# jaak-s/BayesianDataFusion.jl

Measured on AMD Instinct MI355X. Metric: Gibbs sweeps/sec (both entities) + test RMSE, MovieLens-1M D=32, higher is better.
Workload: dtype f64; 1 GPU; BPMF MovieLens-1M 6040x3952, 500209 training ratings (500000 held out), D=32, alpha=1.5, step = rows of both entities + hyperpriors + test prediction update (one native call); BEFORE the --warmup steps the engine's set-up runs 60 ms of full iterations whose results are discarded (device_warmup_ms); num_latent=32, burnin=5, psamples=1985, parallelism=1 GPU

## Files before the change

### bayesiandatafusion.jl_amd/_lib.py

```python
import ctypes as C
import os

_HERE = os.path.dirname(os.path.abspath(__file__))
LIB_PATH = os.environ.get("BDF_LIB_PATH") or os.path.join(_HERE, "csrc", "libbdf_hip.so")

BDF_MAX_MODES = 4
BDF_MAX_TERMS = 4
BDF_MAX_D = 64

P_ROW, P_BETA_E1, P_BETA_E2, P_NW_NORMAL, P_GAMMA_N, P_GAMMA_U, P_NW_MEAN, P_BETA_REL1, P_BETA_REL2 = 1, 2, 3, 4, 5, 6, 7, 8, 9
P_HMC_MOMENTUM, P_HMC_ACCEPT = 10, 11
P_PROBIT = 12
P_CENSORED = 13
P_INTERVAL = 14
P_ORDINAL = 15
P_ROBUST_N, P_ROBUST_U = 16, 17
P_PG = 18
P_NOISE_N, P_NOISE_U = 19, 20
P_SPIKE_N, P_SPIKE_U, P_SPIKE = 21, 22, 23


class ArgumentError(ValueError):
    """The reference's ArgumentError."""

# ... 93 lines not shown
    "bdf_ctx_time_next_hyper": (C.c_int, [C.c_void_p, C.c_void_p, C.c_void_p]),
    "bdf_ctx_set_item_size": (C.c_int, [C.c_void_p, C.c_int]),
    "bdf_dev_alloc": (C.c_int, [C.c_void_p, C.c_size_t, C.POINTER(C.c_void_p)]),
    "bdf_dev_free": (C.c_int, [C.c_void_p, C.c_void_p]),
    "bdf_h2d": (C.c_int, [C.c_void_p, C.c_void_p, C.c_void_p, C.c_size_t]),
    "bdf_d2h": (C.c_int, [C.c_void_p, C.c_void_p, C.c_void_p, C.c_size_t]),
    "bdf_index_build": (C.c_int, [C.c_int, c_i64p, C.c_int64, C.c_void_p, C.c_int, C.POINTER(c_i64p), C.POINTER(c_i64p)]),
    "bdf_relation_create": (C.c_int, [C.c_void_p, C.c_int, c_i64p, C.c_int64, C.c_void_p, C.c_int, c_dp, C.POINTER(C.c_void_p)]),
    "bdf_relation_destroy": (C.c_int, [C.c_void_p]),
    "bdf_relation_index": (C.c_int, [C.c_void_p, C.c_int, C.POINTER(c_i64p), C.POINTER(c_i64p)]),
    "bdf_relation_value_mean": (C.c_int, [C.c_void_p, c_dp]),
    "bdf_relation_order": (C.c_int, [C.c_void_p, C.c_int, c_i32p]),
    "bdf_sample_rows": (C.c_int, [C.c_void_p, C.c_int, C.c_int64, C.c_int, C.POINTER(Term), C.c_void_p, C.c_int, C.c_void_p,
                                  C.c_uint32, C.c_int, C.c_int, C.c_void_p, C.c_void_p]),
    "bdf_prior_pack_doubles": (C.c_int, [C.c_int]),
    "bdf_sample_block": (C.c_int, [C.c_void_p, C.c_int, C.c_int64, C.c_int64, C.c_void_p, C.c_void_p, C.c_void_p, C.c_double, C.c_void_p,
                                   C.c_void_p, C.c_uint32, C.c_void_p]),
    "bdf_row_system": (C.c_int, [C.c_void_p, C.c_int, C.c_int64, C.c_int, C.POINTER(Term), C.c_void_p, C.c_int, C.c_void_p,
                                 C.c_void_p, C.c_void_p]),
    "bdf_normals": (C.c_int, [C.c_void_p, C.c_uint32, C.c_uint32, C.c_int64, C.c_int64, C.c_int, C.c_void_p]),
    "bdf_philox": (C.c_int, [C.c_void_p, C.c_uint32, C.c_uint32, C.c_uint64, C.c_uint32, C.POINTER(C.c_uint32)]),
    "bdf_sample_rows_spike": (C.c_int, [C.c_void_p, C.c_int, C.c_int64, C.c_int, C.POINTER(Term), C.c_void_p, C.c_void_p, C.c_uint32, C.c_int,
                                        C.c_int, C.c_void_p]),
    "bdf_spike_hyper": (C.c_int, [C.c_void_p, C.c_int, C.c_int64, C.c_void_p, C.c_double, C.c_double, C.c_double, C.c_double, C.c_uint32,
                                  C.c_void_p]),
    "bdf_spike_accumulate": (C.c_int, [C.c_void_p, C.c_int, C.c_int64, C.c_void_p, C.c_void_p, C.c_void_p, C.c_void_p]),
    "bdf_hyper_sums": (C.c_int, [C.c_void_p, C.c_int, C.c_int64, C.c_void_p, C.c_void_p, C.c_void_p, C.c_void_p]),
    "bdf_hyper_sums_ranks": (C.c_int, [C.c_void_p, C.c_void_p, C.c_int, C.c_int64, C.c_int, C.c_void_p, C.c_void_p, C.c_void_p, C.c_void_p]),
    "bdf_hyper_sample": (C.c_int, [C.c_void_p, C.c_int, C.c_int64, C.c_void_p, C.c_void_p, C.c_void_p, C.c_double, C.c_void_p,
                                   C.c_double, C.c_uint32, C.c_void_p, C.c_void_p, C.c_void_p, C.c_void_p, C.c_void_p]),
    "bdf_hyper_draws": (C.c_int, [C.c_void_p, C.c_int, C.c_int64, C.c_double, C.c_uint32, C.c_void_p]),
    "bdf_pairs_sort": (C.c_int, [C.c_void_p, C.c_int]),
    "bdf_pairs_order": (C.c_int, [C.c_void_p, c_i64p]),
    "bdf_pairs_set_baseline": (C.c_int, [C.c_void_p, C.c_void_p]),
    "bdf_pairs_set_link": (C.c_int, [C.c_void_p, C.c_int]),
    "bdf_pairs_set_logistic_link": (C.c_int, [C.c_void_p]),
    "bdf_pairs_set_count_link": (C.c_int, [C.c_void_p, C.c_double]),
    "bdf_probit_draw": (C.c_int, [C.c_void_p, C.c_void_p, C.c_int, C.POINTER(C.c_void_p), C.c_double, C.c_uint32, C.c_void_p, C.c_void_p]),
    "bdf_censored_draw": (C.c_int, [C.c_void_p, C.c_void_p, C.c_void_p, C.c_int, C.POINTER(C.c_void_p), C.c_double, C.c_double, C.c_void_p,
                                    C.c_uint32, C.c_void_p, C.c_void_p]),
    "bdf_interval_draw": (C.c_int, [C.c_void_p, C.c_void_p, C.c_void_p, C.c_int, C.POINTER(C.c_void_p), C.c_double, C.c_double, C.c_void_p,
                                    C.c_uint32, C.c_void_p, C.c_void_p]),
    "bdf_robust_draw": (C.c_int, [C.c_void_p, C.c_void_p, C.c_int, C.POINTER(C.c_void_p), C.c_double, C.c_double, C.c_void_p, C.c_double,
                                  C.c_uint32, C.c_void_p, C.c_void_p]),
    "bdf_pg_draw": (C.c_int, [C.c_void_p, C.c_void_p, C.c_int, C.POINTER(C.c_void_p), C.c_double, C.c_int, C.c_double, C.c_uint32,
                              C.c_void_p, C.c_void_p]),
    "bdf_entity_noise_draw": (C.c_int, [C.c_void_p, C.c_void_p, C.c_int, C.c_void_p, C.c_int, C.POINTER(C.c_void_p), C.c_double, C.c_double,
                                        C.c_void_p, C.c_double, C.c_double, C.c_uint32, C.c_void_p, C.c_void_p, C.c_void_p]),
    "bdf_pairs_set_precision_scale": (C.c_int, [C.c_void_p, C.c_void_p, C.c_int]),
    "bdf_pairs_weighted_sse": (C.c_int, [C.c_void_p, C.c_void_p, C.c_int, C.POINTER(C.c_void_p), C.c_double, C.c_void_p, C.c_void_p]),
    "bdf_background_prior": (C.c_int, [C.c_void_p, C.c_int, C.c_int64, C.c_int, C.POINTER(BackgroundTerm), C.c_void_p, C.c_int, C.c_void_p,
                                       C.c_void_p, C.c_void_p, C.c_void_p, C.c_void_p]),
    "bdf_background_sse": (C.c_int, [C.c_void_p, C.c_void_p, C.c_int, C.POINTER(C.c_void_p), C.c_double, C.c_void_p, C.c_double, C.c_double,
                                     C.c_void_p, C.c_void_p, C.c_void_p, C.c_void_p, C.c_int64, C.c_int64, C.c_void_p]),
    "bdf_scores_create": (C.c_int, [C.c_void_p, C.c_int64, C.c_int64, C.c_int, C.c_int, C.c_void_p, C.POINTER(C.c_void_p)]),
    "bdf_scores_destroy": (C.c_int, [C.c_void_p]),
    "bdf_scores_push": (C.c_int, [C.c_void_p, C.c_void_p, C.c_void_p]),
    "bdf_scores_flush": (C.c_int, [C.c_void_p]),
    "bdf_scores_topk": (C.c_int, [C.c_void_p, C.c_void_p, C.c_int, C.c_double, C.c_void_p, C.c_void_p]),
    "bdf_scores_metrics": (C.c_int, [C.c_void_p, C.c_void_p, C.c_int, C.c_void_p, C.c_double, C.c_void_p]),
    "bdf_scores_copy": (C.c_int, [C.c_void_p, C.c_void_p, C.c_int64, C.c_int64, C.c_int]),
    "bdf_scores_set_draws": (C.c_int, [C.c_void_p, C.c_double]),
    "bdf_ordinal_create": (C.c_int, [C.c_void_p, C.c_int, C.c_double, C.c_int64, C.POINTER(C.c_void_p)]),
    "bdf_ordinal_destroy": (C.c_int, [C.c_void_p]),
    "bdf_ordinal_set_adapt": (C.c_int, [C.c_void_p, C.c_int64]),
    "bdf_ordinal_step": (C.c_int, [C.c_void_p, C.c_void_p, C.c_void_p, C.c_void_p, C.c_int, C.POINTER(C.c_void_p), C.c_double, C.c_double,
                                   C.c_void_p, C.c_uint32, C.c_int, C.c_void_p]),
    "bdf_ordinal_bounds": (C.c_int, [C.c_void_p, C.c_void_p, C.c_void_p, C.c_int64, C.c_void_p]),
    "bdf_ordinal_read": (C.c_int, [C.c_void_p, c_dp, c_dp, c_i64p, c_i64p, c_dp, c_dp, C.c_int64]),
    "bdf_ordinal_proposal": (C.c_int, [C.c_void_p, c_dp, c_dp, C.POINTER(C.c_int), c_dp]),
    "bdf_feat_linear": (C.c_int, [C.c_void_p, C.c_void_p, C.c_void_p, C.c_double, C.c_void_p]),
    "bdf_predict_sse": (C.c_int, [C.c_void_p, C.c_void_p, C.c_int, C.POINTER(C.c_void_p), C.c_double, C.c_void_p, C.c_void_p]),
    "bdf_sample_alpha": (C.c_int, [C.c_void_p, C.c_double, C.c_double, C.c_int64, C.c_void_p, C.c_uint32, C.c_void_p]),
    "bdf_sample_beta_rel": (C.c_int, [C.c_void_p, C.c_void_p, C.c_void_p, C.c_int, C.POINTER(C.c_void_p), C.c_double, C.c_double,
                                      C.c_double, C.c_uint32, C.c_void_p, C.c_void_p, C.c_void_p]),
    "bdf_sample_beta_rel_ranks": (C.c_int, [C.c_void_p, C.c_void_p, C.c_void_p, C.c_void_p, C.c_int64, C.c_int, C.POINTER(C.c_void_p),
                                            C.c_double, C.c_double, C.c_double, C.c_uint32, C.c_void_p, C.c_void_p, C.c_void_p]),
    "bdf_sum_ranks": (C.c_int, [C.c_void_p, C.c_void_p, C.c_void_p, C.c_int64]),
    "bdf_gibbs_recorded": (C.c_int, [C.c_void_p, C.c_int, C.POINTER(C.c_int), C.POINTER(C.c_int)]),
    "bdf_gibbs_set_recorded": (C.c_int, [C.c_void_p, C.c_int, C.c_int, C.c_int]),
    "bdf_ctx_set_small_rows": (C.c_int, [C.c_void_p, C.c_int, C.c_int64]),
    "bdf_ctx_set_lowrank": (C.c_int, [C.c_void_p, C.c_int, C.c_int64]),
    "bdf_ctx_set_col_rows": (C.c_int, [C.c_void_p, C.c_int]),
    "bdf_ctx_rows_dispatch": (C.c_int, [C.c_void_p, C.c_uint32, C.POINTER(C.c_int64)]),
    "bdf_pairs_create": (C.c_int, [C.c_void_p, C.c_int, C.c_int64, C.c_void_p, C.c_int, c_dp, C.POINTER(C.c_void_p)]),
    "bdf_pairs_destroy": (C.c_int, [C.c_void_p]),
    "bdf_predict": (C.c_int, [C.c_void_p, C.c_void_p, C.c_int, C.POINTER(C.c_void_p), C.c_double, C.c_void_p]),
    "bdf_predict_all": (C.c_int, [C.c_void_p, C.c_int, C.POINTER(C.c_int64), C.c_int, C.POINTER(C.c_void_p), C.c_double, C.c_void_p]),
    "bdf_predict_update": (C.c_int, [C.c_void_p, C.c_void_p, C.c_int, C.POINTER(C.c_void_p), C.c_double, C.c_int, C.c_double,
                                     C.c_double, C.c_double, C.c_void_p]),
    "bdf_pairs_state": (C.c_int, [C.c_void_p, C.POINTER(C.c_void_p), C.POINTER(C.c_void_p), c_i64p]),
    "bdf_pairs_lpd_update": (C.c_int, [C.c_void_p, C.c_void_p, C.c_void_p, C.c_int, C.POINTER(C.c_void_p), C.c_double, C.c_double, C.c_void_p,
                                       C.c_int, C.c_void_p]),
    "bdf_pairs_lpd": (C.c_int, [C.c_void_p, C.c_void_p, C.c_void_p]),
    "bdf_pairs_waic_update": (C.c_int, [C.c_void_p, C.c_void_p, C.c_void_p, C.c_int, C.POINTER(C.c_void_p), C.c_double, C.c_double, C.c_void_p,
                                        C.c_int, C.c_void_p]),
    "bdf_pairs_waic": (C.c_int, [C.c_void_p, C.c_void_p, C.c_void_p, C.c_void_p]),
    "bdf_newrows_quad": (C.c_int, [C.c_void_p, C.c_int, C.c_int64, C.c_void_p, C.c_void_p, C.c_void_p]),
    "bdf_newrows_update": (C.c_int, [C.c_void_p, C.c_void_p, C.c_int, C.c_void_p, C.c_void_p, C.c_void_p, C.c_double, C.c_double, C.c_void_p,
                                     C.c_int, C.c_double, C.c_double, C.c_double, C.c_int, C.c_void_p]),
    "bdf_newrows_result": (C.c_int, [C.c_void_p, C.c_void_p, C.c_void_p]),
    "bdf_newrows_state": (C.c_int, [C.c_void_p, C.POINTER(C.c_void_p), c_dp]),
    "bdf_feat_create_dense": (C.c_int, [C.c_void_p, C.c_int64, C.c_int64, c_dp, C.POINTER(C.c_void_p)]),
    "bdf_feat_create_csr": (C.c_int, [C.c_void_p, C.c_int64, C.c_int64, C.c_int64, c_i32p, c_i32p, c_dp, C.POINTER(C.c_void_p)]),
    "bdf_feat_create_bin": (C.c_int, [C.c_void_p, C.c_int64, C.c_int64, C.c_int64, c_i32p, c_i32p, C.POINTER(C.c_void_p)]),
    "bdf_feat_destroy": (C.c_int, [C.c_void_p]),
    "bdf_feat_set_row_ids": (C.c_int, [C.c_void_p, c_i32p]),
    "bdf_feat_size": (C.c_int, [C.c_void_p, c_i64p, c_i64p, c_i64p]),
    "bdf_feat_mul": (C.c_int, [C.c_void_p, C.c_void_p, C.c_void_p, C.c_int, C.c_void_p, C.c_int]),
    "bdf_feat_AtA_mul": (C.c_int, [C.c_void_p, C.c_void_p, C.c_void_p, C.c_int, C.c_double, C.c_void_p]),
    "bdf_uhat": (C.c_int, [C.c_void_p, C.c_void_p, C.c_int, C.c_void_p, C.c_void_p, C.c_void_p, C.c_void_p]),
    "bdf_hyper_feature_terms": (C.c_int, [C.c_void_p, C.c_int, C.c_int64, C.c_void_p, C.c_void_p, C.c_void_p, C.c_void_p]),
    "bdf_sample_beta": (C.c_int, [C.c_void_p, C.c_void_p, C.c_int, C.c_void_p, C.c_void_p, C.c_void_p, C.c_void_p, C.c_int,
                                  C.c_double, C.c_int, C.c_int, C.c_double, C.c_double, C.c_uint32, C.c_void_p, C.c_void_p,
                                  C.c_void_p]),
    "bdf_sample_beta_ranks": (C.c_int, [C.c_void_p, C.c_void_p, C.c_void_p, C.c_int, C.c_void_p, C.c_void_p, C.c_void_p, C.c_void_p, C.c_int,
                                        C.c_double, C.c_int, C.c_int, C.c_double, C.c_double, C.c_uint32, C.c_void_p, C.c_void_p,
                                        C.c_void_p]),
    "bdf_allgather_block": (C.c_int, [C.c_void_p, C.c_void_p, C.c_void_p, C.c_size_t]),
    "bdf_ctx_create_side": (C.c_int, [C.c_void_p, C.POINTER(C.c_void_p), C.c_int, C.c_int, C.POINTER(C.c_void_p)]),
    "bdf_ctx_create_rows": (C.c_int, [C.c_int, C.c_uint64, C.c_int, C.POINTER(C.c_void_p)]),
    "bdf_ctx_stream": (C.c_int, [C.c_void_p, C.POINTER(C.c_void_p)]),
    "bdf_layout_build": (C.c_int, [C.c_int64, c_i64p, C.c_int, C.c_int, c_i32p, c_i64p]),
    "bdf_relation_create_sharded": (C.c_int, [C.c_void_p, C.c_int, c_i64p, C.c_int64, C.c_void_p, C.c_int, c_dp, C.POINTER(c_i32p),
                                              c_i64p, C.c_int, C.c_int, C.c_int, C.POINTER(C.c_void_p)]),
    "bdf_comm_unique_id": (C.c_int, [C.c_void_p]),
    "bdf_comm_create": (C.c_int, [C.c_void_p, C.c_int, C.c_int, C.c_char_p, C.POINTER(C.c_void_p)]),
    "bdf_comm_create_host": (C.c_int, [C.c_void_p, C.c_int, C.c_int, EXCHANGE_FN, C.c_void_p, C.POINTER(C.c_void_p)]),
    "bdf_comm_enable_peer": (C.c_int, [C.c_void_p, EXCHANGE_FN, C.c_void_p, C.c_size_t]),
    "bdf_comm_disable_peer": (C.c_int, [C.c_void_p]),
    "bdf_comm_peer_selftest": (C.c_int, [C.c_void_p, C.c_void_p, C.c_void_p, C.c_size_t]),
    "bdf_comm_peer_stats": (C.c_int, [C.c_void_p, C.POINTER(C.c_int64), C.POINTER(C.c_int64)]),
    "bdf_comm_destroy": (C.c_int, [C.c_void_p]),
    "bdf_comm_size": (C.c_int, [C.c_void_p, C.POINTER(C.c_int), C.POINTER(C.c_int)]),
    "bdf_allgather_rows": (C.c_int, [C.c_void_p, C.c_void_p, C.c_int, C.c_int64, C.c_void_p, C.c_int, C.c_int]),
    "bdf_allgather_join": (C.c_int, [C.c_void_p, C.c_void_p]),
    "bdf_gibbs_create": (C.c_int, [C.c_void_p, C.c_int, C.c_int, C.POINTER(GibbsEntity), C.POINTER(C.c_void_p)]),
    "bdf_gibbs_destroy": (C.c_int, [C.c_void_p]),
    "bdf_gibbs_contexts": (C.c_int, [C.c_void_p, C.POINTER(C.c_void_p), C.POINTER(C.c_void_p)]),
    "bdf_gibbs_set_test": (C.c_int, [C.c_void_p, C.c_void_p, C.POINTER(C.c_int32), C.c_double, C.c_double, C.c_double, C.c_double,
                                     C.c_void_p]),
    "bdf_gibbs_set_comm": (C.c_int, [C.c_void_p, C.c_void_p]),
    "bdf_gibbs_set_relations": (C.c_int, [C.c_void_p, C.c_int, C.c_void_p]),
    "bdf_gibbs_sweep": (C.c_int, [C.c_void_p, C.c_uint32, C.c_int]),
    "bdf_gibbs_current": (C.c_int, [C.c_void_p, C.c_int, C.POINTER(C.c_int)]),
    "bdf_gibbs_time_rows": (C.c_int, [C.c_void_p, C.c_int, C.c_void_p, C.c_void_p]),
    "bdf_gibbs_span_rows": (C.c_int, [C.c_void_p, C.c_int, C.c_void_p]),
    "bdf_ctx_span_next_rows": (C.c_int, [C.c_void_p, C.c_void_p]),
    "bdf_gibbs_sync": (C.c_int, [C.c_void_p]),
    "bdf_gibbs_rows_only": (C.c_int, [C.c_void_p, C.c_int, C.c_uint32]),
    "bdf_gibbs_warm_device": (C.c_int, [C.c_void_p, C.c_double]),
    "bdf_synth_ratings": (C.c_int, [C.c_uint64, C.c_int64, C.c_int64, C.c_int64, C.c_int64, C.c_double, C.c_double, c_i32p, c_i32p,
                                    c_dp, C.c_void_p]),
    "bdf_vb_create": (C.c_int, [C.c_void_p, C.c_int, c_i64p, C.c_int64, C.c_void_p, C.c_int, c_dp, C.c_double, c_dp, c_dp,
                                C.POINTER(C.c_void_p)]),
    "bdf_vb_destroy": (C.c_int, [C.c_void_p]),
    "bdf_vb_set_test": (C.c_int, [C.c_void_p, C.c_void_p, C.c_double, C.c_double]),
    "bdf_vb_iterate": (C.c_int, [C.c_void_p, C.c_int]),
    "bdf_vb_stats": (C.c_int, [C.c_void_p, c_dp]),
    "bdf_vb_model": (C.c_int, [C.c_void_p, C.c_int, c_dp, c_dp, c_dp]),
    "bdf_hmc_create": (C.c_int, [C.c_void_p, C.c_int, c_i64p, C.c_int64, C.c_void_p, C.c_int, c_dp, C.c_double,
                                 C.POINTER(C.c_void_p)]),
    "bdf_hmc_destroy": (C.c_int, [C.c_void_p]),
    "bdf_hmc_set_test": (C.c_int, [C.c_void_p, C.c_void_p, C.c_double, C.c_double]),
    "bdf_hmc_set_params": (C.c_int, [C.c_void_p, C.c_int, C.c_int, C.c_int, C.c_double, C.c_int]),
    "bdf_hmc_iterate": (C.c_int, [C.c_void_p, C.c_int]),
# ... 53 lines not shown
```

### bayesiandatafusion.jl_amd/csrc/bdf_api.hip

```cpp
#include <chrono>
#include "rows.h"
#include <cstdlib>
#include <cstring>
#include <algorithm>
#include <cmath>
#include <numeric>
#include <atomic>

static thread_local char g_err[512] = "";

void bdf_set_error(const char *fmt, ...)
{
    va_list ap;
    va_start(ap, fmt);
    vsnprintf(g_err, sizeof(g_err), fmt, ap);
    va_end(ap);
}

extern "C" const char *bdf_last_error(void) { return g_err; }
extern "C" int bdf_version(void) { return 100; }

extern "C" int bdf_ctx_create(int device, void *stream, uint64_t seed, bdf_ctx **out)
{
    BDF_REQUIRE(out != nullptr, BDF_ERR_ARG, "bdf_ctx_create: out is NULL");
    int ndev = 0;
    if (hipGetDeviceCount(&ndev) != hipSuccess || ndev <= 0) {
        bdf_set_error("bdf_ctx_create: no HIP device visible (this library has no CPU path)");
        return BDF_ERR_NOGPU;
    }
    BDF_REQUIRE(device >= 0 && device < ndev, BDF_ERR_ARG, "bdf_ctx_create: device %d out of range (0..%d)", device, ndev - 1);
    BDF_HIP(hipSetDevice(device));
    hipDeviceProp_t prop;
    BDF_HIP(hipGetDeviceProperties(&prop, device));
    if (strncmp(prop.gcnArchName, "gfx950", 6) != 0) {
        bdf_set_error("bdf_ctx_create: device %d is %s; this library is built for gfx950 only", device, prop.gcnArchName);
        return BDF_ERR_NOGPU;
    }
    bdf_ctx *c = new bdf_ctx();
    c->sweep_dev = nullptr; c->flag_dev = nullptr; c->flag_host = nullptr; c->scratch = nullptr; c->scratch2 = nullptr; c->cg_status = nullptr; c->cg_part = nullptr;
    c->hyper_fuse = false; c->hyper_partial = nullptr; c->hyper_nblocks = 0; c->hyper_sumU = c->hyper_UUt = nullptr;
    c->hyper_chain = false; c->hyper_count = nullptr; c->hyper_chain_draws = nullptr;
    c->own_stream = false; c->stream = nullptr; c->rows = nullptr;
    struct Guard { bdf_ctx *c; ~Guard() { if (c) bdf_ctx_destroy(c); } } guard{c};
    c->device = device;
    c->n_cus = prop.multiProcessorCount;
    c->seed = seed;
    c->own_stream = false;
    c->stream = (hipStream_t)stream;
    BDF_HIP(hipMalloc((void **)&c->sweep_dev, sizeof(uint32_t)));
    BDF_HIP(hipHostMalloc((void **)&c->flag_host, 16 * sizeof(int), hipHostMallocMapped | hipHostMallocCoherent));
    memset(c->flag_host, 0, 16 * sizeof(int));
    BDF_HIP(hipHostGetDevicePointer((void **)&c->flag_dev, c->flag_host, 0));
    BDF_HIP(hipMemsetAsync(c->sweep_dev, 0, sizeof(uint32_t), c->stream));
    c->time_start = c->time_stop = nullptr;
    c->time_h_start = c->time_h_stop = nullptr;
    c->sweep_host = 0;
    c->rows_span = nullptr;
    c->rows_ready = nullptr; c->rows_ready_want = 0; c->hyper_ready = nullptr; c->hyper_ready_value = 0;
    c->rows_done = nullptr; c->rows_done_added = -1; c->hyper_wait = nullptr; c->hyper_wait_target = 0;
    c->warnings = 0;
    c->reserve_cus = 0;
    c->on_reserved = 0;
    c->skip_flag = nullptr;
    c->cg_status = nullptr; c->cg_part = nullptr;
    c->hyper_fuse = false; c->hyper_partial = nullptr; c->hyper_nblocks = 0; c->hyper_sumU = c->hyper_UUt = nullptr;
    c->hyper_chain = false; c->hyper_count = nullptr; c->hyper_chain_draws = nullptr;
    c->cg_gen = 0;
    c->cg_bar = nullptr;
    c->rows = bdf_rows_state_create();
    c->norm_part = nullptr;
    c->newrows_W = nullptr;
    c->scratch = nullptr;
    c->scratch2 = nullptr;
    c->scratch2_bytes = 0;
    c->scratch_bytes = 0;
    c->item_size = 192;
    c->piece_size = 128;
    c->item_auto = true;
    c->small_max = getenv("BDF_K1_SMALL") ? atoi(getenv("BDF_K1_SMALL")) : 48;
    c->small_min_rows = getenv("BDF_K1_SMALL_MIN_ROWS") ? atoll(getenv("BDF_K1_SMALL_MIN_ROWS")) : 8192;
    c->lr_max = getenv("BDF_LOWRANK") ? atoi(getenv("BDF_LOWRANK")) : -1;
    c->lr_min_rows = getenv("BDF_LOWRANK_MIN_ROWS") ? atoll(getenv("BDF_LOWRANK_MIN_ROWS")) : 8192;
    c->col_piece = getenv("BDF_K1_COL") ? atoi(getenv("BDF_K1_COL")) : 128;
    if (c->col_piece == 1) c->col_piece = 128;
    if (c->col_piece != 0) c->col_piece = std::min(4096, std::max(8, c->col_piece));
    c->col_explicit = false;
    c->lr_T = nullptr; c->lr_vt = nullptr; c->lr_vt_bytes = 0; c->lr_mrows = nullptr; c->lr_mrows_bytes = 0;
    {
        const char *force = getenv("BDF_GATHER");
        c->gather_mode = force && !strcmp(force, "general") ? 1 : (force && !strcmp(force, "wide") ? 2 : 0);
    }
    guard.c = nullptr;
    *out = c;
    return BDF_OK;
}

extern "C" int bdf_ctx_destroy(bdf_ctx *ctx)
{
    if (!ctx) return BDF_OK;
    hipSetDevice(ctx->device);
    hipStreamSynchronize(ctx->stream);
    bdf_rows_state_destroy(ctx);
    if (ctx->scratch) hipFree(ctx->scratch);
    if (ctx->sweep_dev) hipFree(ctx->sweep_dev);
    if (ctx->flag_host) hipHostFree(ctx->flag_host);
    if (ctx->scratch2) hipFree(ctx->scratch2);
    if (ctx->cg_status) hipHostFree((void *)ctx->cg_status);
    if (ctx->cg_part) hipFree(ctx->cg_part);
    if (ctx->cg_bar) hipFree(ctx->cg_bar);
    if (ctx->hyper_count) hipFree(ctx->hyper_count);
    if (ctx->lr_T) hipFree(ctx->lr_T);
    if (ctx->lr_vt) hipFree(ctx->lr_vt);
    if (ctx->lr_mrows) hipFree(ctx->lr_mrows);
    if (ctx->norm_part) hipFree(ctx->norm_part);
    if (ctx->newrows_W) hipFree(ctx->newrows_W);
    if (ctx->own_stream) hipStreamDestroy(ctx->stream);
    delete ctx;
    return BDF_OK;
}

int bdf_scratch(bdf_ctx *ctx, size_t bytes, void **out)
{
    if (bytes > ctx->scratch_bytes) {
        BDF_HIP(hipStreamSynchronize(ctx->stream));
        if (ctx->scratch) BDF_HIP(hipFree(ctx->scratch));
        size_t nb = std::max(bytes, ctx->scratch_bytes * 2);
        nb = (nb + 255) & ~(size_t)255;
        BDF_HIP(hipMalloc(&ctx->scratch, nb));
        ctx->scratch_bytes = nb;
    }
    *out = ctx->scratch;
    return BDF_OK;
}

int bdf_scratch2(bdf_ctx *ctx, size_t bytes, void **out)
{
    if (bytes > ctx->scratch2_bytes) {
        BDF_HIP(hipStreamSynchronize(ctx->stream));
        if (ctx->scratch2) BDF_HIP(hipFree(ctx->scratch2));
        size_t nb = std::max(bytes, ctx->scratch2_bytes * 2);
        nb = (nb + 255) & ~(size_t)255;
        BDF_HIP(hipMalloc(&ctx->scratch2, nb));
        ctx->scratch2_bytes = nb;
    }
    *out = ctx->scratch2;
    return BDF_OK;
}

__global__ void k_set_u32(uint32_t *p, uint32_t v) { *p = v; }
__global__ void k_inc_u32(uint32_t *p) { *p = *p + 1; }

extern "C" int bdf_ctx_set_sweep(bdf_ctx *ctx, uint32_t sweep)
{
    BDF_REQUIRE(ctx, BDF_ERR_ARG, "bdf_ctx_set_sweep: ctx is NULL");
    ctx->sweep_host = sweep;
    return BDF_OK;
}

extern "C" int bdf_ctx_advance_sweep(bdf_ctx *ctx)
{
    BDF_REQUIRE(ctx, BDF_ERR_ARG, "bdf_ctx_advance_sweep: ctx is NULL");
    ctx->sweep_host++;
    return BDF_OK;
}

extern "C" int bdf_ctx_set_item_size(bdf_ctx *ctx, int observations)
{
    BDF_REQUIRE(ctx && (observations == 0 || (observations >= 8 && observations <= (1 << 20))), BDF_ERR_ARG, "bdf_ctx_set_item_size: 0 (automatic) or 8..2^20 observations");
    if (observations == 0) {
        ctx->item_size = 192; ctx->piece_size = 128; ctx->item_auto = true;
        return BDF_OK;
    }
    ctx->item_size = observations;
    ctx->piece_size = std::max(8, observations * 2 / 3);
    ctx->item_auto = false;
    return BDF_OK;
}

extern "C" int bdf_ctx_set_gather(bdf_ctx *ctx, int mode)
{
    BDF_REQUIRE(ctx && mode >= 0 && mode <= 2, BDF_ERR_ARG, "bdf_ctx_set_gather: mode must be 0 (auto), 1 (general) or 2 (64-bit offsets)");
    ctx->gather_mode = mode;
    return BDF_OK;
}

extern "C" int bdf_ctx_set_small_rows(bdf_ctx *ctx, int max_observations, int64_t min_rows)
{
    BDF_REQUIRE(ctx && max_observations >= 0 && min_rows >= 0, BDF_ERR_ARG, "bdf_ctx_set_small_rows: bad argument");
    ctx->small_max = max_observations;
    ctx->small_min_rows = min_rows;
    return BDF_OK;
}

extern "C" int bdf_ctx_set_lowrank(bdf_ctx *ctx, int max_observations, int64_t min_rows)
{
    BDF_REQUIRE(ctx && max_observations >= -1 && max_observations <= 32 && min_rows >= 0, BDF_ERR_ARG,
                "bdf_ctx_set_lowrank: max_observations must be -1 (default), 0 (off) or 1..32");
    ctx->lr_max = max_observations;
    ctx->lr_min_rows = min_rows;
    return BDF_OK;
}

extern "C" int bdf_ctx_span_next_rows(bdf_ctx *ctx, void *slot_dev)
{
    BDF_REQUIRE(ctx, BDF_ERR_ARG, "bdf_ctx_span_next_rows: NULL context");
    ctx->rows_span = (unsigned long long *)slot_dev;
    return BDF_OK;
}

extern "C" int bdf_ctx_rows_dispatch(const bdf_ctx *ctx, uint32_t entity_tag, int64_t out[6])
{
    BDF_REQUIRE(ctx && out, BDF_ERR_ARG, "bdf_ctx_rows_dispatch: NULL argument");
    const std::array<int64_t, 7> *r = bdf_rows_dispatch_counts(ctx, entity_tag);
    BDF_REQUIRE(r, BDF_ERR_ARG, "bdf_ctx_rows_dispatch: no row launch under entity_tag %u on this context", entity_tag);
    for (int k = 0; k < 6; k++) out[k] = (*r)[(size_t)k + 1];
    return BDF_OK;
}

extern "C" int bdf_ctx_set_col_rows(bdf_ctx *ctx, int max_piece)
{
    BDF_REQUIRE(ctx && (max_piece == 0 || max_piece == -1 || (max_piece >= 8 && max_piece <= 4096)), BDF_ERR_ARG,
                "bdf_ctx_set_col_rows: -1 (default), 0 (off) or 8..4096 observations per piece");
    if (max_piece == -1) {
        ctx->col_piece = getenv("BDF_K1_COL") ? atoi(getenv("BDF_K1_COL")) : 128;
        if (ctx->col_piece == 1) ctx->col_piece = 128;
        if (ctx->col_piece != 0) ctx->col_piece = std::min(4096, std::max(8, ctx->col_piece));
        ctx->col_explicit = false;
        return BDF_OK;
    }
    ctx->col_piece = max_piece;
    ctx->col_explicit = true;
    return BDF_OK;
}

extern "C" int bdf_ctx_set_piece_size(bdf_ctx *ctx, int observations)
{
    BDF_REQUIRE(ctx && observations >= 8 && observations <= ctx->item_size, BDF_ERR_ARG,
                "bdf_ctx_set_piece_size: 8..item size (%d) observations", ctx ? ctx->item_size : 0);
    ctx->piece_size = observations;
    ctx->item_auto = false;
    return BDF_OK;
}

extern "C" int bdf_ctx_sync(bdf_ctx *ctx)
{
    BDF_REQUIRE(ctx, BDF_ERR_ARG, "bdf_ctx_sync: ctx is NULL");
    hipError_t st = hipErrorNotReady;
    const auto t_spin = std::chrono::steady_clock::now();
    while ((st = hipStreamQuery(ctx->stream)) == hipErrorNotReady &&
           std::chrono::duration<double, std::micro>(std::chrono::steady_clock::now() - t_spin).count() < 300.0) { }
    if (st == hipErrorNotReady) st = hipStreamSynchronize(ctx->stream);
    BDF_HIP(st);
    int flag = __atomic_load_n(ctx->flag_host, __ATOMIC_ACQUIRE);
    if (flag) {
        __atomic_store_n(ctx->flag_host, 0, __ATOMIC_RELEASE);
        ctx->warnings |= (uint32_t)flag & BDF_WARN_CG_MAXITER;
        flag &= ~(int)BDF_WARN_CG_MAXITER;
    }
    if (flag) {
        if (flag & 16) {
            bdf_set_error("row sampler: a split row's pieces did not all arrive in time (flag %d)", flag);
            return BDF_ERR_HIP;
        }
        if (flag & 32) {
            bdf_set_error("macau_hmc: an energy of the Hamiltonian was not finite (flag %d)", flag);
            return BDF_ERR_NOTPD;
        }
        bdf_set_error("a matrix that must be positive definite was not (flag %d: %s%s%s%s)", flag, flag & 1 ? "row system " : "",
                      flag & 2 ? "hyperprior " : "", flag & 4 ? "noise precision " : "", flag & 8 ? "FF + lambda I" : "");
        return BDF_ERR_NOTPD;
    }
    return BDF_OK;
}

extern "C" int bdf_ctx_warnings(bdf_ctx *ctx, uint32_t *bits_out)
{
    BDF_REQUIRE(ctx && bits_out, BDF_ERR_ARG, "bdf_ctx_warnings: NULL argument");
    *bits_out = ctx->warnings;
    ctx->warnings = 0;
    return BDF_OK;
}

extern "C" int bdf_event_create(void **ev)
{
    BDF_REQUIRE(ev, BDF_ERR_ARG, "bdf_event_create: NULL argument");
    hipEvent_t e;
    BDF_HIP(hipEventCreate(&e));
    *ev = (void *)e;
    return BDF_OK;
}

extern "C" int bdf_event_destroy(void *ev)
{
    if (ev) BDF_HIP(hipEventDestroy((hipEvent_t)ev));
    return BDF_OK;
}

extern "C" int bdf_event_elapsed_us(void *start, void *stop, double *us)
{
    BDF_REQUIRE(start && stop && us, BDF_ERR_ARG, "bdf_event_elapsed_us: NULL argument");
    BDF_HIP(hipEventSynchronize((hipEvent_t)stop));
    float ms = 0.f;
    BDF_HIP(hipEventElapsedTime(&ms, (hipEvent_t)start, (hipEvent_t)stop));
    *us = 1e3 * (double)ms;
    return BDF_OK;
}

extern "C" int bdf_ctx_time_next_rows(bdf_ctx *ctx, void *start, void *stop)
{
    BDF_REQUIRE(ctx, BDF_ERR_ARG, "bdf_ctx_time_next_rows: ctx is NULL");
    ctx->time_start = (hipEvent_t)start;
    ctx->time_stop = (hipEvent_t)stop;
    return BDF_OK;
}
// ... 536 lines not shown
```

### bayesiandatafusion.jl_amd/csrc/bdf_common.h

```cpp
#pragma once
#include <map>
#include <array>
#include <algorithm>
#include <numeric>
#include <hip/hip_runtime.h>
#include <hip/hip_ext.h>
#include <cstdint>
#include <cstdio>
#include <cstdarg>
#include <cstring>
#include <vector>
#include "../../include/bdf.h"

void bdf_set_error(const char *fmt, ...);

#define BDF_HIP(expr)                                                                      \
    do {                                                                                   \
        hipError_t e__ = (expr);                                                           \
        if (e__ != hipSuccess) {                                                           \
            bdf_set_error("%s failed: %s (%s:%d)", #expr, hipGetErrorString(e__), __FILE__, __LINE__); \
            return BDF_ERR_HIP;                                                            \
        }                                                                                  \
    } while (0)

#define BDF_REQUIRE(cond, code, ...)                                                       \
    do {                                                                                   \
        if (!(cond)) { bdf_set_error(__VA_ARGS__); return (code); }                        \
    } while (0)

template <typename T>
int bdf_upload(T **dst, const std::vector<T> &src)
{
    BDF_HIP(hipMalloc((void **)dst, std::max<size_t>(src.size() * sizeof(T), 16)));
    if (!src.empty()) BDF_HIP(hipMemcpy(*dst, src.data(), src.size() * sizeof(T), hipMemcpyHostToDevice));
    return BDF_OK;
}

template <typename Degree>
std::vector<int32_t> rows_by_degree(int64_t N, Degree degree)
{
    std::vector<int32_t> ord((size_t)N);
    std::iota(ord.begin(), ord.end(), 0);
    std::stable_sort(ord.begin(), ord.end(), [&](int32_t x, int32_t y) { return degree(x) > degree(y); });
    return ord;
}

struct bdf_rows_state;
struct bdf_ctx {
    int device;
    int n_cus;
    hipStream_t stream;
    bool own_stream;
    uint64_t seed;
    uint32_t *sweep_dev;
    uint32_t sweep_host;
    void *scratch;
    size_t scratch_bytes;
    void *scratch2;
    size_t scratch2_bytes;
    int small_max;
    int64_t small_min_rows;
    int lr_max;
    int64_t lr_min_rows;
    int col_piece;
    bool col_explicit;
    double *lr_T;
    double *lr_mrows;
    size_t lr_mrows_bytes;
    double *lr_vt;
    size_t lr_vt_bytes;
    int *flag_dev;
    int *flag_host;
    uint32_t warnings;
    int item_size;
    int piece_size;
    bool item_auto;
    int gather_mode;
    hipEvent_t time_start, time_stop;
    unsigned long long *rows_span;
    const uint32_t *rows_ready;
    uint32_t rows_ready_want;
    uint32_t *rows_done;
    int64_t rows_done_added;
    const uint32_t *hyper_wait;
    uint32_t hyper_wait_target;
    uint32_t *hyper_ready;
    uint32_t hyper_ready_value;
    hipEvent_t time_h_start, time_h_stop;
    int reserve_cus;
    int on_reserved;
    const int *skip_flag;
    volatile uint64_t *cg_status;
    bool hyper_fuse;
    const double *hyper_partial; int hyper_nblocks; double *hyper_sumU, *hyper_UUt;
    bool hyper_chain;
    int hyper_chain_D; int64_t hyper_chain_N, hyper_chain_rpb; const double *hyper_chain_sample, *hyper_chain_uhat;
    unsigned *hyper_count;
    double *hyper_chain_draws;
    double *cg_part;
    uint32_t cg_gen;
    unsigned *cg_bar;
    bdf_rows_state *rows;
    double *norm_part;
    double *newrows_W;
};

int bdf_scratch(bdf_ctx *ctx, size_t bytes, void **out);
int bdf_scratch2(bdf_ctx *ctx, size_t bytes, void **out);
int bdf_sum_ranks_into(bdf_ctx *ctx, bdf_comm *comm, double *x, int64_t n, double *gather);
int bdf_sample_beta_rel_impl(bdf_ctx *ctx, bdf_comm *comm, const bdf_feat *fc, const bdf_pairs *train, int64_t first_obs, int D,
                             const double *const *factors, double mean_value, double alpha, const double *alpha_dev, double lambda_beta,
                             uint32_t rel_tag, double *beta_out, double *linear_out, double *rhs_out);
#define BDF_DRAWS_BATCH 8
int bdf_hyper_draws_batch(bdf_ctx *ctx, int D, int n, const int64_t *N, const double *nu, const uint32_t *entity_tag, double *const *draws_out);

struct bdf_mode_index {
    std::vector<int64_t> rowptr;
    std::vector<int64_t> rowids;
    std::vector<int32_t> order;
    int64_t *rowptr_dev;
    int32_t *colidx_dev;
    double  *vals_dev;
    int32_t *perm_dev;
    uint32_t *packed_dev;
    int32_t *order_dev;
    std::vector<int32_t> own_orig;
    std::vector<int32_t> own_pos;
    std::vector<int64_t> own_q;
    std::vector<int64_t> chunk_begin;
    int64_t own_nnz;
};

struct bdf_rel {
    bdf_ctx *ctx;
    uint64_t serial;
    int n_modes;
    int64_t dims[BDF_MAX_MODES];
    int64_t nnz;
    double value_mean;
    bdf_mode_index idx[BDF_MAX_MODES];
    int sharded;
    int rank, world, chunks;
    int64_t nint[BDF_MAX_MODES];
    int n_codes;
    double *table_dev;
};

struct bdf_pairs {
// ... 224 lines not shown
```

### bayesiandatafusion.jl_amd/csrc/bdf_gibbs.hip

```cpp
#include "bdf_common.h"
#include <algorithm>
#include <chrono>
#include <cmath>
#include <cstdio>
#include <cstdlib>
#include <map>
#include <mutex>
#include <tuple>

struct bdf_gibbs {
    bdf_ctx *rows, *hyper, *pred;
    bdf_ctx *gate = nullptr;
    int D;
    struct Ent {
        bdf_gibbs_entity d;
        int cur;
        hipEvent_t ev_rows = nullptr, ev_hyper = nullptr;
        hipEvent_t ev_beta = nullptr;
        bool beta_recorded = false;
        bool hyper_recorded = false;
        uint32_t epoch = 0;
        uint32_t *done_dev = nullptr;
        uint32_t done_target = 0;
        hipEvent_t t_start = nullptr, t_stop = nullptr;
        unsigned long long *span = nullptr;
    };
    std::vector<Ent> ent;
    bdf_pairs *test;
    int32_t test_entity[BDF_MAX_MODES];
    double test_mean, clamp_lo, clamp_hi, class_cut;
    double *stats_dev;
    hipEvent_t ev_pred[3] = {nullptr, nullptr, nullptr};
    uint64_t pred_at[3] = {0, 0, 0};
    uint64_t n_pred;
    uint64_t n_iter = 0;
    bdf_comm *comm;
    std::vector<bdf_gibbs_relation> rels;
    double *rel_sse = nullptr;
    uint32_t *ready_dev;
    bool polling;
    bool debug;
    double host_wait_us, host_enqueue_us;
    uint64_t n_sweeps;
};

namespace {

__global__ void k_spin(long long ticks)
{
    const long long t0 = wall_clock64();
    while (wall_clock64() - t0 < ticks) __builtin_amdgcn_s_sleep(8);
}

__global__ void k_wait_flag(const uint32_t *flag, long long max_ticks, uint32_t *timed_out)
{
    const long long t0 = wall_clock64();
    while (__hip_atomic_load(flag, __ATOMIC_RELAXED, __HIP_MEMORY_SCOPE_AGENT) == 0) {
        __builtin_amdgcn_s_sleep(8);
        if (wall_clock64() - t0 > max_ticks) { *timed_out = 1; break; }
    }
}
__global__ void k_set_flag(uint32_t *flag) { __hip_atomic_store(flag, 1u, __ATOMIC_RELEASE, __HIP_MEMORY_SCOPE_AGENT); }

__global__ __launch_bounds__(64) void k_rows_gate(const uint32_t *done, uint32_t target, int *flag)
{
    int spins = 0;
    for (;;) {
        uint32_t v = __hip_atomic_load(done + BDF_DONE_STRIDE * threadIdx.x, __ATOMIC_RELAXED, __HIP_MEMORY_SCOPE_AGENT);
#pragma unroll
        for (int off = 32; off >= 1; off >>= 1) v += __shfl_xor(v, off);
        if ((int32_t)(v - target) >= 0) break;
        __builtin_amdgcn_s_sleep(8);
        if (++spins > (1 << 22)) { if (threadIdx.x == 0) atomicOr_system(flag, 16); break; }
    }
}

int streams_concurrent(hipStream_t a, hipStream_t b, bool *yes)
{
    uint32_t *d;
    BDF_HIP(hipMalloc((void **)&d, 2 * sizeof(uint32_t)));
    struct Free { uint32_t *p; ~Free() { (void)hipFree(p); } } guard{d};
    BDF_HIP(hipMemsetAsync(d, 0, 2 * sizeof(uint32_t), a));
    BDF_HIP(hipStreamSynchronize(a)); BDF_HIP(hipStreamSynchronize(b));
    hipLaunchKernelGGL(k_wait_flag, dim3(1), dim3(1), 0, a, (const uint32_t *)d, 2000000LL, d + 1);
    hipLaunchKernelGGL(k_set_flag, dim3(1), dim3(1), 0, b, d);
    BDF_HIP(hipStreamSynchronize(a)); BDF_HIP(hipStreamSynchronize(b));
    uint32_t h[2] = {0, 0};
    BDF_HIP(hipMemcpy(h, d, sizeof(h), hipMemcpyDeviceToHost));
    *yes = h[1] == 0;
    return BDF_OK;
}

int streams_overlap(hipStream_t a, hipStream_t b, bool *yes)
{
    hipEvent_t e0, e1, e2;
    BDF_HIP(hipEventCreate(&e0)); BDF_HIP(hipEventCreate(&e1)); BDF_HIP(hipEventCreate(&e2));
    BDF_HIP(hipStreamSynchronize(a)); BDF_HIP(hipStreamSynchronize(b));
    float best = 1e9f;
    for (int rep = 0; rep < 3; rep++) {
        BDF_HIP(hipEventRecord(e0, a));
        BDF_HIP(hipStreamWaitEvent(b, e0, 0));
        hipLaunchKernelGGL(k_spin, dim3(1), dim3(64), 0, a, 6000LL);
        hipLaunchKernelGGL(k_spin, dim3(1), dim3(64), 0, b, 6000LL);
        BDF_HIP(hipEventRecord(e1, b));
        BDF_HIP(hipStreamWaitEvent(a, e1, 0));
        BDF_HIP(hipEventRecord(e2, a));
        BDF_HIP(hipEventSynchronize(e2));
        float ms = 0.f;
        BDF_HIP(hipEventElapsedTime(&ms, e0, e2));
        best = std::min(best, ms);
    }
    (void)hipEventDestroy(e0); (void)hipEventDestroy(e1); (void)hipEventDestroy(e2);
    *yes = best < 0.100f;
    return BDF_OK;
}

int pooled_stream(int device, int reserve, bool reserved, int slot, hipStream_t *out)
{
    static std::mutex mu;
    static std::map<std::tuple<int, int, int, int>, hipStream_t> pool;
    std::lock_guard<std::mutex> lock(mu);
    const auto key = std::make_tuple(device, reserve, reserved ? 1 : 0, slot);
    auto it = pool.find(key);
    if (it != pool.end()) { *out = it->second; return BDF_OK; }
    hipStream_t st;
    if (reserve <= 0) {
        BDF_HIP(hipStreamCreateWithFlags(&st, hipStreamNonBlocking));
    } else {
        hipDeviceProp_t prop;
        BDF_HIP(hipGetDeviceProperties(&prop, device));
        const int ncu = prop.multiProcessorCount, words = (ncu + 31) / 32;
        std::vector<uint32_t> mask((size_t)words, 0u);
        for (int i = 0; i < ncu; i++)
            if ((i < reserve) == reserved) mask[(size_t)(i / 32)] |= 1u << (i % 32);
        BDF_HIP(hipExtStreamCreateWithCUMask(&st, (uint32_t)words, mask.data()));
    }
    pool[key] = st;
    *out = st;
    return BDF_OK;
}

int make_side_ctx(bdf_ctx *main, const std::vector<bdf_ctx *> &apart, bool reserved, bdf_ctx **out)
{
    bdf_ctx *fallback = nullptr;
    for (int attempt = 0; attempt < 8; attempt++) {
        hipStream_t st;
        int rc = pooled_stream(main->device, main->reserve_cus, reserved, attempt + 1, &st);
        if (rc) return rc;
        if (st == main->stream) continue;
        bool taken = false;
        for (bdf_ctx *o : apart) taken = taken || o->stream == st;
        if (taken) continue;
        bdf_ctx *c;
        rc = bdf_ctx_create(main->device, (void *)st, main->seed, &c);
        if (rc) return rc;
        c->reserve_cus = main->reserve_cus;
        c->on_reserved = (reserved && main->reserve_cus > 0) ? 1 : 0;
        bool ok = true;
        if ((rc = streams_overlap(st, main->stream, &ok))) return rc;
// ... 11 lines not shown
}

}

extern "C" int bdf_ctx_create_rows(int device, uint64_t seed, int reserve_cus, bdf_ctx **out)
{
    BDF_REQUIRE(out && reserve_cus >= 0 && reserve_cus % 8 == 0 && reserve_cus <= 64, BDF_ERR_ARG,
                "bdf_ctx_create_rows: reserve_cus must be 0, 8, 16, ... 64 (whole CUs per XCD)");
    int ndev = 0;
    if (hipGetDeviceCount(&ndev) != hipSuccess || ndev <= 0) {
        bdf_set_error("bdf_ctx_create_rows: no HIP device visible (this library has no CPU path)");
        return BDF_ERR_NOGPU;
    }
    BDF_REQUIRE(device >= 0 && device < ndev, BDF_ERR_ARG, "bdf_ctx_create_rows: device %d out of range", device);
    BDF_HIP(hipSetDevice(device));
    hipStream_t st;
    int rc = pooled_stream(device, reserve_cus, false, 0, &st);
    if (rc) return rc;
    bdf_ctx *c;
    if ((rc = bdf_ctx_create(device, (void *)st, seed, &c))) return rc;
    c->reserve_cus = reserve_cus;
    *out = c;
    return BDF_OK;
}

extern "C" int bdf_ctx_create_side(bdf_ctx *main_ctx, bdf_ctx *const *apart, int n_apart, int reserved, bdf_ctx **out)
{
    BDF_REQUIRE(main_ctx && out && n_apart >= 0 && (n_apart == 0 || apart), BDF_ERR_ARG, "bdf_ctx_create_side: bad argument");
    std::vector<bdf_ctx *> ap(apart, apart + n_apart);
    return make_side_ctx(main_ctx, ap, reserved != 0, out);
}

extern "C" int bdf_gibbs_create(bdf_ctx *rows_ctx, int D, int n_entities, const bdf_gibbs_entity *ents, bdf_gibbs **out)
{
    BDF_REQUIRE(rows_ctx && ents && out, BDF_ERR_ARG, "bdf_gibbs_create: NULL argument");
    BDF_REQUIRE(D >= 1 && D <= BDF_MAX_D, BDF_ERR_ARG, "bdf_gibbs_create: num_latent=%d must be in 1..%d", D, BDF_MAX_D);
    BDF_REQUIRE(n_entities >= 1 && n_entities <= 64, BDF_ERR_ARG, "bdf_gibbs_create: 1..64 entities");
    for (int j = 0; j < n_entities; j++) {
        const bdf_gibbs_entity &e = ents[j];
        BDF_REQUIRE(e.n_terms >= 1 && e.n_terms <= BDF_MAX_TERMS, BDF_ERR_ARG, "bdf_gibbs_create: entity %d takes part in %d relations (1..%d)", j, e.n_terms, BDF_MAX_TERMS);
        BDF_REQUIRE(e.sample[0] && e.sample[1] && e.sample[2] && e.mu && e.Lambda && e.mu0 && e.WI && e.sumU && e.UUt && e.prior_pack && e.draws,
                    BDF_ERR_ARG, "bdf_gibbs_create: entity %d has a NULL buffer", j);
        BDF_REQUIRE(!e.feat || (e.beta && e.uhat && e.mu_matrix && e.Tinv && e.lambda_beta), BDF_ERR_ARG,
                    "bdf_gibbs_create: entity %d has side information but a NULL beta / uhat / mu_matrix / Tinv / lambda_beta", j);
        BDF_REQUIRE(!e.spike || (e.spike_state && !e.feat && !e.bg_Lambda), BDF_ERR_ARG,
                    "bdf_gibbs_create: entity %d has the spike-and-slab prior: spike_state must be set, side information and a background are not taken", j);
        BDF_REQUIRE(!e.feat || e.feat->m == e.N, BDF_ERR_ARG, "bdf_gibbs_create: entity %d has %lld rows but its feature matrix %lld", j,
                    (long long)e.N, e.feat ? (long long)e.feat->m : 0LL);
        for (int t = 0; t < e.n_terms; t++) {
            BDF_REQUIRE(e.terms[t].rel, BDF_ERR_ARG, "bdf_gibbs_create: entity %d term %d has no relation", j, t);
            for (int k = 0; k < e.terms[t].rel->n_modes; k++)
                BDF_REQUIRE(e.terms[t].entity_of_mode[k] >= 0 && e.terms[t].entity_of_mode[k] < n_entities, BDF_ERR_ARG,
                            "bdf_gibbs_create: entity %d term %d mode %d names entity %d", j, t, k, e.terms[t].entity_of_mode[k]);
        }
    }
    BDF_HIP(hipSetDevice(rows_ctx->device));
    bdf_gibbs *g = new bdf_gibbs();
    g->rows = rows_ctx; g->hyper = g->pred = nullptr; g->D = D; g->test = nullptr; g->stats_dev = nullptr;
    g->n_pred = 0; g->comm = nullptr; g->ready_dev = nullptr; g->polling = false;
    g->debug = false; g->host_wait_us = g->host_enqueue_us = 0.0; g->n_sweeps = 0;
    int rc;
    if ((rc = make_side_ctx(rows_ctx, {}, true, &g->hyper)) || (rc = make_side_ctx(rows_ctx, {g->hyper}, false, &g->pred))) { bdf_gibbs_destroy(g); return rc; }
    g->ready_dev = nullptr;
    g->polling = rows_ctx->reserve_cus > 0 && g->hyper->on_reserved && !getenv("BDF_NO_POLL");
    if (g->polling) {
        bool conc = false;
        if ((rc = streams_concurrent(rows_ctx->stream, g->hyper->stream, &conc))) { bdf_gibbs_destroy(g); return rc; }
        g->polling = conc;
    }
    if (g->polling && (rc = make_side_ctx(rows_ctx, {g->hyper, g->pred}, true, &g->gate))) { bdf_gibbs_destroy(g); return rc; }
    if (g->polling && !g->gate) g->polling = false;
    g->debug = getenv("BDF_DEBUG") != nullptr;
    if (g->debug)
        fprintf(stderr, "[bdf_gibbs] reserve_cus=%d hyperprior stream on reserved CUs=%d polling=%d\n", rows_ctx->reserve_cus,
                g->hyper->on_reserved, (int)g->polling);
    struct Guard { bdf_gibbs *g; ~Guard() { if (g) bdf_gibbs_destroy(g); } } guard{g};
    BDF_HIP(hipMalloc((void **)&g->ready_dev, (size_t)n_entities * sizeof(uint32_t)));
    BDF_HIP(hipMemsetAsync(g->ready_dev, 0, (size_t)n_entities * sizeof(uint32_t), rows_ctx->stream));
    BDF_HIP(hipStreamSynchronize(rows_ctx->stream));
    g->ent.resize((size_t)n_entities);
    for (int j = 0; j < n_entities; j++) {
        auto &E = g->ent[(size_t)j];
        E.d = ents[j]; E.cur = 0;
        BDF_HIP(hipEventCreate(&E.ev_rows));
        BDF_HIP(hipEventCreate(&E.ev_hyper));
        if (E.d.feat) BDF_HIP(hipEventCreateWithFlags(&E.ev_beta, hipEventDisableTiming));
    }
    for (int k = 0; k < 3; k++) BDF_HIP(hipEventCreateWithFlags(&g->ev_pred[k], hipEventDisableTiming));
    if (g->polling) {
        const size_t bytes = (size_t)BDF_DONE_SHARDS * BDF_DONE_STRIDE * sizeof(uint32_t);
        for (int j = 0; j < n_entities; j++) {
            BDF_HIP(hipMalloc((void **)&g->ent[(size_t)j].done_dev, bytes));
            BDF_HIP(hipMemsetAsync(g->ent[(size_t)j].done_dev, 0, bytes, rows_ctx->stream));
        }
        BDF_HIP(hipStreamSynchronize(rows_ctx->stream));
    }
    guard.g = nullptr;
    *out = g;
    return BDF_OK;
}

extern "C" int bdf_gibbs_destroy(bdf_gibbs *g)
{
    if (!g) return BDF_OK;
    if (g->rows) (void)hipStreamSynchronize(g->rows->stream);
    if (g->debug && g->n_sweeps)
        fprintf(stderr, "[bdf_gibbs] %llu sweeps: host enqueue %.1f us per sweep, host wait for the device %.1f us per sweep\n",
                (unsigned long long)g->n_sweeps, g->host_enqueue_us / (double)g->n_sweeps, g->host_wait_us / (double)g->n_sweeps);
    for (auto &E : g->ent) {
        if (E.ev_rows) (void)hipEventDestroy(E.ev_rows);
        if (E.ev_hyper) (void)hipEventDestroy(E.ev_hyper);
        if (E.ev_beta) (void)hipEventDestroy(E.ev_beta);
        if (E.done_dev) (void)hipFree(E.done_dev);
    }
    for (int k = 0; k < 3; k++)
        if (g->ev_pred[k]) (void)hipEventDestroy(g->ev_pred[k]);
    if (g->ready_dev) (void)hipFree(g->ready_dev);
    if (g->rel_sse) (void)hipFree(g->rel_sse);
    if (g->gate) { (void)hipStreamSynchronize(g->gate->stream); bdf_ctx_destroy(g->gate); }
    if (g->pred) bdf_ctx_destroy(g->pred);
    if (g->hyper) bdf_ctx_destroy(g->hyper);
    delete g;
    return BDF_OK;
}

extern "C" int bdf_gibbs_contexts(bdf_gibbs *g, bdf_ctx **hyper, bdf_ctx **pred)
{
    BDF_REQUIRE(g, BDF_ERR_ARG, "bdf_gibbs_contexts: NULL argument");
    if (hyper) *hyper = g->hyper;
    if (pred) *pred = g->pred;
    return BDF_OK;
}

extern "C" int bdf_ctx_stream(const bdf_ctx *ctx, void **stream)
{
    BDF_REQUIRE(ctx && stream, BDF_ERR_ARG, "bdf_ctx_stream: NULL argument");
    *stream = (void *)ctx->stream;
    return BDF_OK;
}

extern "C" int bdf_gibbs_set_test(bdf_gibbs *g, bdf_pairs *pairs, const int32_t *entity_of_mode, double mean_value,
                                  double clamp_lo, double clamp_hi, double class_cut, double *stats_dev)
{
    BDF_REQUIRE(g && pairs && entity_of_mode && stats_dev, BDF_ERR_ARG, "bdf_gibbs_set_test: NULL argument");
    for (int k = 0; k < pairs->n_modes; k++) {
        BDF_REQUIRE(entity_of_mode[k] >= 0 && entity_of_mode[k] < (int)g->ent.size(), BDF_ERR_ARG, "bdf_gibbs_set_test: mode %d names entity %d", k, entity_of_mode[k]);
        g->test_entity[k] = entity_of_mode[k];
    }
    g->test = pairs; g->test_mean = mean_value; g->clamp_lo = clamp_lo; g->clamp_hi = clamp_hi; g->class_cut = class_cut;
    g->stats_dev = stats_dev;
    return BDF_OK;
}

extern "C" int bdf_gibbs_set_relations(bdf_gibbs *g, int n_relations, const bdf_gibbs_relation *rels)
{
    BDF_REQUIRE(g && n_relations >= 0 && (n_relations == 0 || rels), BDF_ERR_ARG, "bdf_gibbs_set_relations: bad argument");
    for (int k = 0; k < n_relations; k++) {
        const bdf_gibbs_relation &r = rels[k];
        BDF_REQUIRE(r.rel && (r.alpha_dev || r.probit), BDF_ERR_ARG, "bdf_gibbs_set_relations: relation %d has no handle or no alpha_dev", k);
        BDF_REQUIRE(!(r.alpha_sample || r.feat) || r.train, BDF_ERR_ARG, "bdf_gibbs_set_relations: relation %d needs its observations as pairs (train)", k);
        BDF_REQUIRE(!r.feat || (r.beta && r.linear), BDF_ERR_ARG, "bdf_gibbs_set_relations: relation %d has features but no beta / linear buffer", k);
        BDF_REQUIRE(!r.feat_test || r.test_baseline, BDF_ERR_ARG, "bdf_gibbs_set_relations: relation %d has test features but no baseline buffer", k);
        BDF_REQUIRE(!r.probit || (!r.feat && !r.alpha_sample), BDF_ERR_ARG, "bdf_gibbs_set_relations: relation %d: the probit model takes neither relation features nor a sampled alpha", k);
        BDF_REQUIRE(!r.probit || (r.train && r.linear), BDF_ERR_ARG, "bdf_gibbs_set_relations: relation %d: the probit model needs its observations as pairs (train) and a linear buffer", k);
        BDF_REQUIRE(!r.censor || (!r.probit && !r.feat), BDF_ERR_ARG, "bdf_gibbs_set_relations: relation %d: the censored model takes neither the probit model nor relation features", k);
        BDF_REQUIRE(!r.censor || (r.train && r.linear), BDF_ERR_ARG, "bdf_gibbs_set_relations: relation %d: the censored model needs its observations as pairs (train) and a linear buffer", k);
// ... 105 lines not shown
    int n_bg = 0;
    for (int t = 0; t < e.n_terms; t++) {
        terms[t].rel = e.terms[t].rel; terms[t].mode = e.terms[t].mode; terms[t]._pad = 0;
        terms[t].alpha = e.terms[t].alpha; terms[t].mean_value = e.terms[t].mean_value; terms[t].linear_values = nullptr;
        terms[t].alpha_dev = nullptr; terms[t].obs_precision = nullptr;
        if (const bdf_gibbs_relation *gr = relation_of(g, e.terms[t].rel)) {
            terms[t].alpha_dev = gr->probit ? nullptr : gr->alpha_dev;
            terms[t].linear_values = (gr->feat || draws_latent(*gr)) ? gr->linear : nullptr;
            if (gr->probit) terms[t].alpha = 1.0;
            terms[t].obs_precision = gr->obs_precision;
            if (gr->bg_weight > 0.0) {
                if (gr->obs_precision) terms[t].linear_values = gr->linear;
                else terms[t].alpha_dev = e.bg_alpha_rows + n_bg;
                n_bg++;
            }
        }
        for (int k = 0; k < BDF_MAX_MODES; k++) terms[t].factors[k] = nullptr;
        current_factors(g, e.terms[t].entity_of_mode, e.terms[t].rel->n_modes, terms[t].factors);
    }
}

int update_relations(bdf_gibbs *g)
{
    bdf_ctx *R = g->rows;
    const int D = g->D;
    int rc;
    for (const auto &r : g->rels) {
        if (!has_model(r)) continue;
        const double *fac[BDF_MAX_MODES];
        current_factors(g, r.entity_of_mode, r.rel->n_modes, fac);
        if (r.robust_nu > 0.0 && (rc = bdf_robust_draw(R, r.train, D, fac, r.mean_value, 0.0, r.alpha_dev, r.robust_nu, r.rel_tag, r.obs_precision,
                                                      r.alpha_sample ? g->rel_sse + 1 : nullptr)))
            return rc;
        if (r.noise_mode != 0 && (rc = bdf_entity_noise_draw(R, r.rel, r.noise_mode - 1, r.train, D, fac, r.mean_value, 0.0, r.alpha_dev, r.noise_shape,
                                                             r.noise_rate, r.rel_tag, r.noise_tau, r.obs_precision, r.alpha_sample ? g->rel_sse + 1 : nullptr)))
            return rc;
        if (r.alpha_sample) {
            int64_t n = r.nnz;
            if (r.bg_weight > 0.0) {
                const size_t pk = (size_t)D + (size_t)D * D;
                for (int m = 0; m < 2; m++)
                    if ((rc = bdf_hyper_sums(R, D, g->ent[(size_t)r.entity_of_mode[m]].d.N, fac[m], nullptr, r.bg_sums + m * pk, r.bg_sums + m * pk + D))) return rc;
                rc = bdf_background_sse(R, r.train, D, fac, r.mean_value, r.bg_weights, r.bg_value, r.bg_weight, r.bg_sums, r.bg_sums + D, r.bg_sums + pk,
                                        r.bg_sums + pk + D, r.rel->dims[0], r.rel->dims[1], g->rel_sse + 1);
                n = r.rel->dims[0] * r.rel->dims[1];
            } else if (r.obs_precision) rc = (r.robust_nu > 0.0 || r.noise_mode != 0) ? BDF_OK : bdf_pairs_weighted_sse(R, r.train, D, fac, r.mean_value, r.obs_precision, g->rel_sse + 1);
            else rc = bdf_predict_sse(R, r.train, D, fac, r.mean_value, nullptr, g->rel_sse);
            if (rc) return rc;
            if (g->comm && (rc = bdf_sum_ranks(R, g->comm, g->rel_sse + 1, 1))) return rc;
            if ((rc = bdf_sample_alpha(R, r.alpha_lambda0, r.alpha_nu0, n, g->rel_sse + 1, r.rel_tag, r.alpha_dev))) return rc;
        }
        if (r.probit && (rc = bdf_probit_draw(R, r.train, D, fac, r.mean_value, r.rel_tag, r.linear + r.first_obs, nullptr))) return rc;
        if (r.pg_model && (rc = bdf_pg_draw(R, r.train, D, fac, r.mean_value, r.pg_model, r.pg_r, r.rel_tag, r.obs_precision, r.linear + r.first_obs)))
            return rc;
        if (r.censor && (rc = bdf_censored_draw(R, r.train, r.censor, D, fac, r.mean_value, 0.0, r.alpha_dev, r.rel_tag, r.linear + r.first_obs, nullptr)))
            return rc;
        if (r.ordinal && (rc = bdf_ordinal_step(R, r.ordinal, r.train, r.ordinal_codes, D, fac, r.mean_value, 0.0, r.alpha_dev, r.rel_tag, -1,
                                                const_cast<double *>(r.interval))))
            return rc;
        if (r.interval && (rc = bdf_interval_draw(R, r.train, r.interval, D, fac, r.mean_value, 0.0, r.alpha_dev, r.rel_tag, r.linear + r.first_obs, nullptr)))
            return rc;
        if (r.feat) {
            if ((rc = bdf_sample_beta_rel_impl(R, g->comm, r.feat, r.train, r.first_obs, D, fac, r.mean_value, 1.0, r.alpha_dev, r.lambda_beta,
                                               r.rel_tag, r.beta, r.linear + r.first_obs, nullptr)))
                return rc;
            if (g->comm) {
                if ((rc = bdf_allgather_block(R, g->comm, r.linear, sizeof(double) * (size_t)r.obs_block)) || (rc = bdf_allgather_join(R, g->comm))) return rc;
            }
            if (r.feat_test) {
                for (int k = 0; k < 3; k++)
                    if (g->n_pred > (uint64_t)k) BDF_HIP(hipStreamWaitEvent(R->stream, g->ev_pred[(g->n_pred - 1 - (uint64_t)k) % 3], 0));
                if ((rc = bdf_feat_linear(R, r.feat_test, r.beta, r.mean_value, r.test_baseline))) return rc;
            }
        }
    }
    return BDF_OK;
}
}

extern "C" int bdf_gibbs_set_comm(bdf_gibbs *g, bdf_comm *comm)
{
    BDF_REQUIRE(g, BDF_ERR_ARG, "bdf_gibbs_set_comm: NULL argument");
    g->comm = comm;
    return BDF_OK;
}

namespace {
double hyper_nu(const bdf_gibbs_entity &e) { return e.nu0 + ((e.feat && e.full_lambda_u) ? (double)e.feat->n : 0.0); }
}

extern "C" int bdf_gibbs_rows_only(bdf_gibbs *g, int entity, uint32_t sweep)
{
    BDF_REQUIRE(g && entity >= 0 && entity < (int)g->ent.size(), BDF_ERR_ARG, "bdf_gibbs_rows_only: bad argument");
    bdf_ctx *R = g->rows;
    auto &E = g->ent[(size_t)entity];
    const bdf_gibbs_entity &e = E.d;
    R->sweep_host = sweep;
    int rc;
    bdf_term terms[BDF_MAX_TERMS];
    fill_terms(g, e, terms);
    const int nxt = (E.cur + 1) % 3;
    if (e.spike) {
        if ((rc = bdf_sample_rows_spike(R, g->D, e.N, e.n_terms, terms, e.spike_state, e.sample[E.cur], e.tag, 0, 1, e.sample[nxt]))) return rc;
        E.cur = nxt;
        return BDF_OK;
    }
    const double *mu, *Lambda, *pack;
    if ((rc = row_prior(g, E, &mu, &Lambda, &pack))) return rc;
    const int nch = e.terms[0].rel->chunks;
    for (int c = 0; c < nch; c++)
        if ((rc = bdf_sample_rows(R, g->D, e.N, e.n_terms, terms, mu, e.feat ? 1 : 0, Lambda, e.tag, c, nch, e.sample[nxt], pack))) return rc;
    E.cur = nxt;
    return BDF_OK;
}

extern "C" int bdf_gibbs_warm_device(bdf_gibbs *g, double milliseconds)
{
    BDF_REQUIRE(g && milliseconds >= 0.0 && milliseconds <= 10000.0, BDF_ERR_ARG, "bdf_gibbs_warm_device: bad argument");
    if (milliseconds <= 0.0) return BDF_OK;
    bdf_ctx *R = g->rows;
    const int D = g->D, n = (int)g->ent.size();
    int rc;
    if ((rc = bdf_gibbs_sync(g))) return rc;
    struct Piece { void *p; size_t bytes; bool sample; int ent; };
    std::vector<Piece> pieces;
    std::vector<char> flags;
    const size_t DD = (size_t)D * D * sizeof(double), Dv = (size_t)D * sizeof(double);
    for (int j = 0; j < n; j++) {
        auto &E = g->ent[(size_t)j];
        const bdf_gibbs_entity &e = E.d;
        pieces.push_back({e.sample[E.cur], (size_t)e.N * Dv, true, j});
        pieces.push_back({e.mu, Dv, false, j}); pieces.push_back({e.Lambda, DD, false, j});
        pieces.push_back({e.sumU, Dv, false, j}); pieces.push_back({e.UUt, DD, false, j});
        if (e.params) pieces.push_back({e.params, Dv + DD, false, j});
        pieces.push_back({e.prior_pack, (size_t)bdf_prior_pack_doubles(D) * sizeof(double), false, j});
        pieces.push_back({e.draws, DD + Dv, false, j});
        if (e.spike) pieces.push_back({e.spike_state, 4 * Dv, false, j});
        if (e.feat) {
            pieces.push_back({e.beta, (size_t)e.feat->n * Dv, false, j});
            pieces.push_back({e.uhat, (size_t)e.N * Dv, false, j});
            pieces.push_back({e.mu_matrix, (size_t)e.N * Dv, false, j});
            pieces.push_back({e.Tinv, DD, false, j});
            pieces.push_back({e.lambda_beta, sizeof(double), false, j});
            if (e.cg_iters) pieces.push_back({e.cg_iters, (size_t)D * sizeof(int32_t), false, j});
        }
        flags.push_back(E.hyper_recorded ? 1 : 0); flags.push_back(E.beta_recorded ? 1 : 0);
    }
    if (g->stats_dev) pieces.push_back({g->stats_dev, 4 * sizeof(double), false, 0});
    for (const auto &r : g->rels) {
        if (r.alpha_dev) pieces.push_back({r.alpha_dev, sizeof(double), false, 0});
        if (r.feat) {
            int world = 1, rk = 0;
            if (g->comm) (void)bdf_comm_size(g->comm, &rk, &world);
            pieces.push_back({r.beta, (size_t)r.feat->n * sizeof(double), false, 0});
            pieces.push_back({r.linear, (size_t)r.obs_block * (size_t)world * sizeof(double), false, 0});
            if (r.feat_test) pieces.push_back({r.test_baseline, (size_t)r.feat_test->m * sizeof(double), false, 0});
        }
        if (draws_latent(r)) pieces.push_back({r.linear + r.first_obs, (size_t)r.train->n * sizeof(double), false, 0});
        if (r.robust_nu > 0.0 || r.pg_model || r.noise_mode != 0) pieces.push_back({r.obs_precision, (size_t)r.train->n * sizeof(double), false, 0});
        if (r.noise_mode != 0) pieces.push_back({r.noise_tau, (size_t)r.rel->dims[r.noise_mode - 1] * sizeof(double), false, 0});
        if (r.ordinal) {
            pieces.push_back({r.ordinal->state_dev, r.ordinal->state_doubles * sizeof(double), false, 0});
            pieces.push_back({const_cast<double *>(r.interval), (size_t)r.train->n * 2 * sizeof(double), false, 0});
        }
    }
    size_t total = 0;
    for (auto &pc : pieces) total += (pc.bytes + 255) & ~(size_t)255;
    char *snap = nullptr;
    BDF_HIP(hipMalloc((void **)&snap, std::max<size_t>(total, 256)));
    struct Free { char *p; ~Free() { if (p) (void)hipFree(p); } } guard{snap};
    size_t off = 0;
    for (auto &pc : pieces) {
        BDF_HIP(hipMemcpyAsync(snap + off, pc.p, pc.bytes, hipMemcpyDeviceToDevice, R->stream));
        off += (pc.bytes + 255) & ~(size_t)255;
    }
    BDF_HIP(hipStreamSynchronize(R->stream));
    const uint32_t keep = R->sweep_host;
    int64_t fixed = 0;
    const auto t0 = std::chrono::steady_clock::now();
    int64_t k = 0;
    rc = BDF_OK;
    while (!rc) {
        for (int b = 0; b < 8 && !rc; b++, k++) rc = bdf_gibbs_sweep(g, 0xfffe0000u + (uint32_t)(k & 0xffff), g->test ? 3 : -1);
        if (rc) break;
        if (g->comm && fixed == 0) {
            if ((rc = bdf_gibbs_sync(g))) break;
            const double per_iter = std::chrono::duration<double, std::milli>(std::chrono::steady_clock::now() - t0).count() / 8.0;
            const double mine = std::max(8.0, std::min(20000.0, milliseconds / std::max(per_iter, 1e-3)));
            int rank = 0, world = 1;
            if ((rc = bdf_comm_size(g->comm, &rank, &world))) break;
            void *sv;
            if ((rc = bdf_scratch(R, ((size_t)world + 1) * sizeof(double), &sv))) break;
            double *cnt = (double *)sv;
            BDF_HIP(hipMemcpyAsync(cnt, &mine, sizeof(double), hipMemcpyHostToDevice, R->stream));
            if ((rc = bdf_sum_ranks_into(R, g->comm, cnt, 1, cnt + 1))) break;
            double sum = 0.0;
            BDF_HIP(hipMemcpyAsync(&sum, cnt, sizeof(double), hipMemcpyDeviceToHost, R->stream));
            BDF_HIP(hipStreamSynchronize(R->stream));
            fixed = std::max<int64_t>(8, (int64_t)(sum / (double)world + 0.5));
        }
        if (fixed ? k >= fixed : std::chrono::duration<double, std::milli>(std::chrono::steady_clock::now() - t0).count() >= milliseconds) break;
    }
    const int rc_sync = bdf_gibbs_sync(g);
    if (!rc) rc = rc_sync;
    off = 0;
    for (auto &pc : pieces) {
        void *dst = pc.sample ? (void *)g->ent[(size_t)pc.ent].d.sample[g->ent[(size_t)pc.ent].cur] : pc.p;
        BDF_HIP(hipMemcpyAsync(dst, snap + off, pc.bytes, hipMemcpyDeviceToDevice, R->stream));
        off += (pc.bytes + 255) & ~(size_t)255;
    }
    for (int j = 0; j < n; j++) {
        g->ent[(size_t)j].hyper_recorded = flags[(size_t)2 * j] != 0;
        g->ent[(size_t)j].beta_recorded = flags[(size_t)2 * j + 1] != 0;
    }
    BDF_HIP(hipStreamSynchronize(R->stream));
    R->sweep_host = g->hyper->sweep_host = g->pred->sweep_host = keep;
    return rc;
}

extern "C" int bdf_gibbs_recorded(const bdf_gibbs *g, int entity, int *hyper, int *beta)
{
    BDF_REQUIRE(g && entity >= 0 && entity < (int)g->ent.size() && hyper && beta, BDF_ERR_ARG, "bdf_gibbs_recorded: bad argument");
    *hyper = g->ent[(size_t)entity].hyper_recorded ? 1 : 0;
    *beta = g->ent[(size_t)entity].beta_recorded ? 1 : 0;
    return BDF_OK;
}

extern "C" int bdf_gibbs_set_recorded(bdf_gibbs *g, int entity, int hyper, int beta)
{
    BDF_REQUIRE(g && entity >= 0 && entity < (int)g->ent.size(), BDF_ERR_ARG, "bdf_gibbs_set_recorded: bad argument");
    g->ent[(size_t)entity].hyper_recorded = hyper != 0;
    g->ent[(size_t)entity].beta_recorded = beta != 0;
    return BDF_OK;
}

extern "C" int bdf_gibbs_time_rows(bdf_gibbs *g, int entity, void *start, void *stop)
{
    BDF_REQUIRE(g && entity >= 0 && entity < (int)g->ent.size(), BDF_ERR_ARG, "bdf_gibbs_time_rows: bad entity");
    g->ent[(size_t)entity].t_start = (hipEvent_t)start;
    g->ent[(size_t)entity].t_stop = (hipEvent_t)stop;
    return BDF_OK;
}

extern "C" int bdf_gibbs_span_rows(bdf_gibbs *g, int entity, void *slot_dev)
{
    BDF_REQUIRE(g && entity >= 0 && entity < (int)g->ent.size(), BDF_ERR_ARG, "bdf_gibbs_span_rows: bad entity");
    g->ent[(size_t)entity].span = (unsigned long long *)slot_dev;
    return BDF_OK;
}

extern "C" int bdf_gibbs_current(const bdf_gibbs *g, int entity, int *buffer)
{
    BDF_REQUIRE(g && buffer && entity >= 0 && entity < (int)g->ent.size(), BDF_ERR_ARG, "bdf_gibbs_current: bad argument");
    *buffer = g->ent[(size_t)entity].cur;
    return BDF_OK;
}

extern "C" int bdf_gibbs_sweep(bdf_gibbs *g, uint32_t sweep, int predict_phase)
{
    BDF_REQUIRE(g, BDF_ERR_ARG, "bdf_gibbs_sweep: NULL argument");
    bdf_ctx *R = g->rows, *H = g->hyper, *P = g->pred;
    const int D = g->D, n = (int)g->ent.size();
    int rc;
    R->sweep_host = H->sweep_host = P->sweep_host = sweep;
    constexpr uint64_t pred_lag = 3;
    const auto t_in = std::chrono::steady_clock::now();
    for (uint64_t back = 1; back <= std::min<uint64_t>(g->n_pred, 3); back++) {
        const uint64_t k = (g->n_pred - back) % 3;
        if (g->pred_at[k] + pred_lag <= g->n_iter) {
            hipError_t st = hipErrorNotReady;
            const auto t_spin = std::chrono::steady_clock::now();
            while ((st = hipEventQuery(g->ev_pred[k])) == hipErrorNotReady &&
                   std::chrono::duration<double, std::micro>(std::chrono::steady_clock::now() - t_spin).count() < 400.0) { }
            if (st == hipErrorNotReady) st = hipEventSynchronize(g->ev_pred[k]);
            BDF_HIP(st);
            break;
        }
    }
    const auto t_go = std::chrono::steady_clock::now();
    bool draws_in_chain = !g->comm;
    for (int j = 0; j < n; j++) draws_in_chain = draws_in_chain && g->ent[(size_t)j].d.N <= 16384;
    if (!draws_in_chain && n <= BDF_DRAWS_BATCH) {
        int64_t Ns[BDF_DRAWS_BATCH]; double nus[BDF_DRAWS_BATCH]; uint32_t tags[BDF_DRAWS_BATCH]; double *outs[BDF_DRAWS_BATCH];
        int nb = 0;
        for (int j = 0; j < n; j++) {
            const bdf_gibbs_entity &e = g->ent[(size_t)j].d;
            if (e.spike) continue;
            Ns[nb] = e.n_real; nus[nb] = hyper_nu(e); tags[nb] = e.tag; outs[nb] = e.draws; nb++;
        }
        if (nb > 0 && (rc = bdf_hyper_draws_batch(H, D, nb, Ns, nus, tags, outs))) return rc;
    }
    if (!g->rels.empty() && (rc = update_relations(g))) return rc;
    for (int j = 0; j < n; j++) {
        auto &E = g->ent[(size_t)j];
        const bdf_gibbs_entity &e = E.d;
        static const bool poll_with_comm = getenv("BDF_POLL_WITH_COMM") != nullptr;
        bool bg = false;
        for (int t = 0; t < e.n_terms; t++) bg = bg || background_of(g, e, t) != nullptr;
        const bool poll = g->polling && (!g->comm || poll_with_comm) && E.hyper_recorded && !e.feat && !bg && !e.spike;
        if (E.hyper_recorded && !poll) BDF_HIP(hipStreamWaitEvent(R->stream, E.ev_hyper, 0));
        if (e.feat && (rc = bdf_uhat(R, e.feat, D, e.beta, e.mu, e.uhat, e.mu_matrix))) return rc;
        if (!draws_in_chain && n > BDF_DRAWS_BATCH && !e.spike && (rc = bdf_hyper_draws(H, D, e.n_real, hyper_nu(e), e.tag, e.draws))) return rc;
        const double *mu_rows = nullptr, *Lambda_rows = nullptr, *pack_rows = nullptr;
        if (!e.spike && (rc = row_prior(g, E, &mu_rows, &Lambda_rows, &pack_rows))) return rc;
        bdf_term terms[BDF_MAX_TERMS];
        fill_terms(g, e, terms);
        const int nxt = (E.cur + 1) % 3;
        hipEvent_t done = E.t_stop ? E.t_stop : E.ev_rows;
        const int nch = e.terms[0].rel->chunks;
        const bool counter = E.done_dev && draws_in_chain && g->polling && !g->comm && !e.feat && !bg && !e.spike && nch == 1 && !E.t_stop;
        const bool pred_waits = j == n - 1 && g->test && predict_phase >= 0;
        bool by_counter = false;
        for (int c = 0; c < nch; c++) {
            R->time_start = (c == 0) ? E.t_start : nullptr;
            R->rows_span = E.span;
            R->time_stop = (c == nch - 1 && !g->comm && !counter) ? done : nullptr;
            if (poll) { R->rows_ready = g->ready_dev + j; R->rows_ready_want = E.epoch; }
            if (counter) R->rows_done = E.done_dev;
            if ((rc = e.spike ? bdf_sample_rows_spike(R, D, e.N, e.n_terms, terms, e.spike_state, e.sample[E.cur], e.tag, c, nch, e.sample[nxt])
                              : bdf_sample_rows(R, D, e.N, e.n_terms, terms, mu_rows, e.feat ? 1 : 0, Lambda_rows, e.tag, c, nch, e.sample[nxt], pack_rows)))
                return rc;
            if (counter && R->rows_done_added >= 0) { by_counter = true; E.done_target += (uint32_t)R->rows_done_added; }
            if (g->comm && (rc = bdf_allgather_rows(R, g->comm, D, e.N, e.sample[nxt], c, nch))) return rc;
        }
        if (g->comm) {
            if ((rc = bdf_allgather_join(R, g->comm))) return rc;
            BDF_HIP(hipEventRecord(done, R->stream));
        } else if (counter && !by_counter) {
            BDF_HIP(hipEventRecord(done, R->stream));
        }
        E.t_start = E.t_stop = nullptr;
        E.span = nullptr;
        E.cur = nxt;
        if (by_counter) { H->hyper_wait = E.done_dev; H->hyper_wait_target = E.done_target; }
        else BDF_HIP(hipStreamWaitEvent(H->stream, done, 0));
        if (e.spike) {
            if ((rc = bdf_spike_hyper(H, D, e.n_real, e.sample[E.cur], e.spike_a, e.spike_b, e.spike_shape, e.spike_rate, e.tag, e.spike_state)))
                return rc;
            BDF_HIP(hipEventRecord(E.ev_hyper, H->stream));
            E.hyper_recorded = true;
            if (pred_waits) BDF_HIP(hipStreamWaitEvent(P->stream, done, 0));
            continue;
        }
        H->hyper_fuse = true;
        const double *Tinv = e.WI;
        if (e.feat && e.full_lambda_u) {
            if (E.beta_recorded) BDF_HIP(hipStreamWaitEvent(H->stream, E.ev_beta, 0));
            if ((rc = bdf_hyper_feature_terms(H, D, e.feat->n, e.beta, e.WI, e.lambda_beta, e.Tinv))) return rc;
            Tinv = e.Tinv;
        }
        if ((rc = g->comm ? bdf_hyper_sums_ranks(H, g->comm, D, e.N, nch, e.sample[E.cur], e.feat ? e.uhat : nullptr, e.sumU, e.UUt)
                          : bdf_hyper_sums(H, D, e.N, e.sample[E.cur], e.feat ? e.uhat : nullptr, e.sumU, e.UUt)))
            return rc;
        H->hyper_chain_draws = draws_in_chain ? e.draws : nullptr;
        H->time_h_stop = E.ev_hyper;
        H->hyper_ready = g->ready_dev + j;
        H->hyper_ready_value = ++E.epoch;
        if ((rc = bdf_hyper_sample(H, D, e.n_real, e.sumU, e.UUt, e.mu0, e.b0, Tinv, hyper_nu(e), e.tag, e.mu, e.Lambda, e.params, e.prior_pack, e.draws)))
            return rc;
        E.hyper_recorded = true;
        if (pred_waits && by_counter) {
            hipExtLaunchKernelGGL(k_rows_gate, dim3(1), dim3(64), 0, g->gate->stream, nullptr, E.ev_rows, 0, (const uint32_t *)E.done_dev,
                                  E.done_target, H->flag_dev);
            BDF_HIP(hipGetLastError());
            BDF_HIP(hipStreamWaitEvent(P->stream, E.ev_rows, 0));
        } else if (pred_waits) BDF_HIP(hipStreamWaitEvent(P->stream, done, 0));
    }
    for (int j = 0; j < n; j++) {
        auto &E = g->ent[(size_t)j];
        const bdf_gibbs_entity &e = E.d;
        if (!e.feat) continue;
        BDF_HIP(hipStreamWaitEvent(R->stream, E.ev_hyper, 0));
        if ((rc = bdf_sample_beta_ranks(R, g->comm, e.feat, D, e.sample[E.cur], e.mu, e.Lambda, e.lambda_beta, e.use_ff, e.tol, 0,
                                        e.sample_lambda_beta, e.lb_nu, e.lb_mu, e.tag, e.beta, nullptr, e.cg_iters)))
            return rc;
        BDF_HIP(hipEventRecord(E.ev_beta, R->stream));
        E.beta_recorded = true;
    }
    if (g->test && predict_phase >= 0) {
        const double *fac[BDF_MAX_MODES];
        current_factors(g, g->test_entity, g->test->n_modes, fac);
        if ((rc = predict_phase == 3 ? bdf_predict_sse(P, g->test, D, fac, g->test_mean, nullptr, g->stats_dev)
                                     : bdf_predict_update(P, g->test, D, fac, g->test_mean, predict_phase, g->clamp_lo, g->clamp_hi, g->class_cut, g->stats_dev)))
            return rc;
        BDF_HIP(hipEventRecord(g->ev_pred[g->n_pred % 3], P->stream));
        g->pred_at[g->n_pred % 3] = g->n_iter;
        g->n_pred++;
    }
    g->n_iter++;
    if (g->debug) {
        g->host_wait_us += std::chrono::duration<double, std::micro>(t_go - t_in).count();
        g->host_enqueue_us += std::chrono::duration<double, std::micro>(std::chrono::steady_clock::now() - t_go).count();
        g->n_sweeps++;
    }
    return BDF_OK;
}

extern "C" int bdf_gibbs_sync(bdf_gibbs *g)
{
    BDF_REQUIRE(g, BDF_ERR_ARG, "bdf_gibbs_sync: NULL argument");
    int rc;
// ... 4 lines not shown
```

### bayesiandatafusion.jl_amd/csrc/dpp_rows32.h

```cpp
#pragma once
#include "dpp_rows16.h"

namespace {

template <int S, int I>
__device__ __forceinline__ int sys_off(int j)
{
    constexpr int IB = I / 16, ii = I % 16;
    if constexpr (IB >= S) {
        constexpr int blk = IB * (IB + 1) / 2 + S;
        return (blk * 4 + (ii >> 2)) * 64 + 16 * (ii & 3) + j;
    } else {
        return (1 * 4 + (j >> 2)) * 64 + 16 * (j & 3) + ii;
    }
}

template <int DR, int I>
__device__ __forceinline__ void col_rank1(double (&A0)[33], double (&A1)[33], double v0, double v1)
{
    if constexpr (I < 16) {
        if constexpr (I == 0) fm1<0>(A0[0], v0, v0); else fm1_run<I>(A0[I], v0, v0);
        if constexpr (16 + I < DR) {
            fm1_run<I>(A0[16 + I], v1, v0);
            fm1_run<I>(A1[16 + I], v1, v1);
        }
        col_rank1<DR, I + 1>(A0, A1, v0, v1);
    }
}
template <int B0, int K0, int N, int I = 0>
__device__ __forceinline__ void col_star(double (&A)[33], double s, double m)
{
    if constexpr (I < N) {
        fm1_run<K0 + I>(A[B0 + I], s, m);
        col_star<B0, K0, N, I + 1>(A, s, m);
    }
}
__device__ __forceinline__ double col_own_y(double v0, double v1, uint64_t hmask)
{
    int lo, hi;
    asm("s_mov_b64 vcc, %6\n\t"
        "v_cndmask_b32_dpp %0, %2, %4, vcc row_ror:8 row_mask:0xf bank_mask:0xf\n\t"
        "v_cndmask_b32_dpp %1, %3, %5, vcc row_ror:8 row_mask:0xf bank_mask:0xf"
        : "=&v"(lo), "=v"(hi) : "v"(__double2loint(v0)), "v"(__double2hiint(v0)), "v"(__double2loint(v1)), "v"(__double2hiint(v1)), "s"(hmask) : "vcc");
    return __hiloint2double(hi, lo);
}
template <int DR>
__device__ __forceinline__ void col_rank1u(double (&A0)[33], double (&A1)[33], double v0, double v1, bool h, uint64_t hmask)
{
    fm1<0>(A0[0], v0, v0);
    col_star<1, 1, 7>(A0, v0, v0);
    col_star<0, 0, 8>(A1, v0, v1);
    col_star<16, 0, (DR - 16 < 8 ? DR - 16 : 8)>(A1, v1, v1);
    const double x = h ? v0 : v1;
    col_star<8, 8, 8>(A0, v0, x);
    if constexpr (DR > 24) {
        const double y = col_own_y(v0, v1, hmask);
        col_star<24, 8, DR - 24>(A1, v1, y);
    }
}
template <int DR, int S, int K, int I, bool FIRST>
__device__ __forceinline__ void fin_elim(double (&A0)[33], double (&A1)[33], double nm0, double nm1)
{
    if constexpr (I <= 32) {
        if constexpr (S == 0) {
            if constexpr (DR > 16) {
                if constexpr (FIRST) fm1<K>(A1[I], A0[I], nm1); else fm1_run<K>(A1[I], A0[I], nm1);
                fm1_self_run<K>(A0[I], nm0);
            } else {
                if constexpr (FIRST) fm1_self<K>(A0[I], nm0); else fm1_self_run<K>(A0[I], nm0);
            }
        } else {
            if constexpr (FIRST) fm1_self<K>(A1[I], nm1); else fm1_self_run<K>(A1[I], nm1);
        }
        fin_elim<DR, S, K, (I + 1 < DR || I == 32) ? I + 1 : 32, false>(A0, A1, nm0, nm1);
    }
}

template <int DR, int k>
__device__ __forceinline__ void fin_factor(double (&A0)[33], double (&A1)[33], double &d0, double &d1, int j)
{
    if constexpr (k < DR) {
        constexpr int S = k / 16, K = k % 16;
        const double dk = row_bcast_f64<K>(S ? A1[k] : A0[k]);
        const double rinv = fast_rcp(dk);
        double nm0 = 0.0, nm1;
        if constexpr (S == 0) {
            d0 = (j == K) ? dk : d0;
            nm0 = (j > K) ? -(A0[k] * rinv) : 0.0;
            nm1 = -(A1[k] * rinv);
        } else {
            d1 = (j == K) ? dk : d1;
            nm1 = (j > K) ? -(A1[k] * rinv) : 0.0;
        }
        fin_elim<DR, S, K, (k + 1 < DR) ? k + 1 : 32, true>(A0, A1, nm0, nm1);
        fin_factor<DR, k + 1>(A0, A1, d0, d1, j);
    }
}

template <int C>
__device__ __forceinline__ void fin_backward(const double (&A0)[33], const double (&A1)[33], double &y0, double &y1, double rd0,
                                             double rd1, int j)
{
    if constexpr (C >= 1) {
        constexpr int S = C / 16, K = C % 16;
        if constexpr (S == 1) {
            fm1<K>(y0, y1, -(A0[C] * rd0));
            if constexpr (K > 0) fm1_self_run<K>(y1, (j < K) ? -(A1[C] * rd1) : 0.0);
        } else {
            fm1_self<K>(y0, (j < K) ? -(A0[C] * rd0) : 0.0);
        }
        fin_backward<C - 1>(A0, A1, y0, y1, rd0, rd1, j);
    }
}

}
```

### bayesiandatafusion.jl_amd/csrc/k_rows_col.hip

```cpp
#include "rows.h"
#include "dpp_rows32.h"
#include <algorithm>

#ifndef BDF_COL_WAVES
#define BDF_COL_WAVES 2
#endif
#define COL_VGPR_HALF 104
#define COL_PSZ 672
#define COL_NE 42
#define COL_TL 304

#ifdef BDF_K1_STAMPS
#define CSTAMP_DECL unsigned long long st_t = __builtin_amdgcn_s_memtime(), st_acc = 0, st_mid = 0, st_prior = 0, st_fin = 0, st_rng = 0, st_lay = 0, st_steps = 0, st_rounds = 0, st_parts = 0, st_fins = 0, st_folds = 0; const unsigned long long st_begin = st_t
#define CSTAMP(x) do { const unsigned long long now_ = __builtin_amdgcn_s_memtime(); x += now_ - st_t; st_t = now_; } while (0)
#else
#define CSTAMP_DECL do { } while (0)
#define CSTAMP(x) do { } while (0)
#endif

namespace {

struct ColCoef { static __device__ __forceinline__ double c(double x) { asm volatile("" : "+s"(x)); return x; } };

template <int DR, int K>
__device__ __forceinline__ void col_obs(double (&A0)[33], double (&A1)[33], double v0, double v1, double r, bool h, uint64_t hmask)
{
    col_rank1u<DR>(A0, A1, v0, v1, h, hmask);
    fm1_run<K>(A0[32], r, v0);
    fm1_run<K>(A1[32], r, v1);
}

__device__ __forceinline__ double col_ld(__amdgpu_buffer_rsrc_t rs, uint32_t off)
{
    typedef unsigned u2v __attribute__((ext_vector_type(2)));
    const u2v x = __builtin_amdgcn_raw_buffer_load_b64(rs, (int)off, 0, 0);
    return __hiloint2double((int)x.y, (int)x.x);
}

template <bool FULL, int K0>
__device__ __forceinline__ void col_gather4(double (&b)[4][2], __amdgpu_buffer_rsrc_t rs, uint32_t idw, uint32_t rowb, uint32_t eo, bool ok1)
{
#pragma unroll
    for (int q = 0; q < 4; q++) {
        uint32_t id;
        if (q == 0) id = row_bcast_u32<K0>(idw); else if (q == 1) id = row_bcast_u32<K0 + 1>(idw);
        else if (q == 2) id = row_bcast_u32<K0 + 2>(idw); else id = row_bcast_u32<K0 + 3>(idw);
        if constexpr (FULL) {
            const uint32_t base = id + eo;
            b[q][1] = col_ld(rs, base);
            b[q][0] = col_ld(rs, base + 128u);
        } else {
            const uint32_t base = id + eo;
            b[q][0] = col_ld(rs, base);
            b[q][1] = col_ld(rs, ok1 ? base - 128u : 0xffffffffu);
        }
    }
}
template <int DR, int K0>
__device__ __forceinline__ void col_compute4(double (&A0)[33], double (&A1)[33], const double (&b)[4][2], double r, bool h, uint64_t hmask)
{
    col_obs<DR, K0>(A0, A1, b[0][0], b[0][1], r, h, hmask);
    col_obs<DR, K0 + 1>(A0, A1, b[1][0], b[1][1], r, h, hmask);
    col_obs<DR, K0 + 2>(A0, A1, b[2][0], b[2][1], r, h, hmask);
    col_obs<DR, K0 + 3>(A0, A1, b[3][0], b[3][1], r, h, hmask);
}

__device__ __forceinline__ double &col_entry(double (&A0)[33], double (&A1)[33], int e)
{
    return e < 16 ? A0[e] : e == 16 ? A0[32] : e < 25 ? A1[e - 17] : A1[e - 9];
}
template <int X>
__device__ __forceinline__ void col_fold(double (&A0)[33], double (&A1)[33], double m)
{
#pragma unroll
    for (int e = 0; e < COL_NE; e++) { double &d = col_entry(A0, A1, e); d = fma(__shfl_xor(d, X), m, d); }
}

template <int E0, int E1, bool ADD>
__device__ __forceinline__ void col_slot_load(double (&A0)[33], double (&A1)[33], const double *src, double m)
{
#pragma unroll
    for (int e = E0; e < E1; e++) {
        const double v = src[e * 16];
        double &d = col_entry(A0, A1, e);
        if (ADD) d = fma(v, m, d); else d = v * m;
    }
}

__device__ __forceinline__ void col_prior_dma(const double *image, unsigned lds_dst, int lane)
{
    const void *sbase = (const void *)(((uint64_t)(uint32_t)__builtin_amdgcn_readfirstlane((int)((uint64_t)image >> 32)) << 32) |
                                       (uint32_t)__builtin_amdgcn_readfirstlane((int)(uint32_t)(uint64_t)image));
#pragma unroll
    for (int k = 0; k < 6; k++) {
        const unsigned voff = (unsigned)k * 1024u + (unsigned)lane * 16u;
        unsigned keep;
        asm volatile("s_mov_b32 %0, m0\n\ts_mov_b32 m0, %2\n\ts_nop 0\n\tglobal_load_lds_dwordx4 %1, %3 sc1\n\ts_mov_b32 m0, %0"
                     : "=&s"(keep) : "v"(voff), "s"(lds_dst + (unsigned)k * 1024u), "s"(sbase) : "memory");
    }
}
template <int S, int I, int DR>
__device__ __forceinline__ void col_prior_lds(double (&A)[33], const double *img, double alpha, int j)
{
    if constexpr (I < DR) {
        A[I] = fma(alpha, A[I], img[sys_off<S, I>(j)]);
        col_prior_lds<S, I + 1, DR>(A, img, alpha, j);
    }
}

template <int DR, bool FULL>
__global__ __launch_bounds__(64, BDF_COL_WAVES) __attribute__((amdgpu_num_vgpr(COL_VGPR_HALF))) void k_rows_col(SampleArgs a_in, ColPlanDev p_in, uint32_t fac_bytes)
{
    __shared__ __attribute__((aligned(16))) double lds[4 * COL_TL + 768];
    const int w = blockIdx.x;
    if (w >= p_in.n_waves) return;
    const int r_end = p_in.wave_round[w + 1];
    if (a_in.span && threadIdx.x == 0) atomicMin(a_in.span + 2 * (w & 63), (unsigned long long)__builtin_amdgcn_s_memrealtime());
    CSTAMP_DECL;
#pragma nounroll
    for (int rd = p_in.wave_round[w]; rd < r_end; rd++) {
    int zero = 0, lane = threadIdx.x;
    asm volatile("" : "+s"(zero), "+v"(lane));
    const SampleArgs &a = (&a_in)[zero];
    const ColPlanDev &p = (&p_in)[zero];
    const int j = lane & 15, g = lane >> 4;
    const bool hh = (j & 8) != 0;
    const uint64_t hmask = 0xff00ff00ff00ff00ull;
    const TermDev &T = a.t[0];
    const int D = FULL ? 32 : a.D;
    const int ec0 = D - 1 - j, ec1 = D - 17 - j;
    const int n0 = ec0, n1 = ec1 >= 0 ? ec1 : 0;
    const bool ok1 = ec1 >= 0;
    const uint32_t rowb = (uint32_t)D * 8u;
    const uint32_t eo = FULL ? (uint32_t)ec1 * 8u : (uint32_t)ec0 * 8u;
    const __amdgpu_buffer_rsrc_t rs = __builtin_amdgcn_make_buffer_rsrc((void *)T.fac[0], 0, (int)fac_bytes, 0x00020000);
    const bool coded = T.packed != nullptr;
    const double mean = T.mean;
    {
        const ColJob jb = p.jobs[(int64_t)rd * 4 + g];
        const bool live = jb.row >= 0;
        const int n = live ? jb.count : 0;
        const unsigned lds_img = (unsigned)__builtin_amdgcn_readfirstlane((int)(unsigned)(size_t)(__attribute__((address_space(3))) double *)(lds + 4 * COL_TL));
        bool have_prior = true;
        if (a.ready) have_prior = __builtin_amdgcn_readfirstlane((int)((int32_t)(__hip_atomic_load(a.ready, __ATOMIC_RELAXED, __HIP_MEMORY_SCOPE_AGENT) - a.ready_want) >= 0)) != 0;
        if (have_prior) col_prior_dma(a.prior_c, lds_img, lane);
        double A0[33], A1[33];
#pragma unroll
        for (int i = 0; i < 33; i++) { A0[i] = 0.0; A1[i] = 0.0; }
        int nmax = n;
        nmax = max(nmax, __shfl_xor(nmax, 16));
        nmax = max(nmax, __shfl_xor(nmax, 32));
        nmax = __builtin_amdgcn_readfirstlane(nmax);
        if (nmax > 0) {
            const uint32_t *packed = coded ? T.packed + jb.q_begin : nullptr;
            const int32_t *colidx = T.colidx + jb.q_begin;
            const double *vals = T.vals + jb.q_begin;
            const double *table = T.table;
#define COL_CHUNK(c0, IDW, R)                                                                     \
            {                                                                                     \
                const int o_ = (c0) + j;                                                          \
                IDW = 0xffffffu; R = 0.0;                                                         \
                if (o_ < n) {                                                                     \
                    if (coded) { const uint32_t pw_ = packed[o_]; IDW = pw_; R = table[pw_ >> 24] - mean; } \
                    else { IDW = (uint32_t)colidx[o_]; R = vals[o_] - mean; }                     \
                }                                                                                 \
                IDW = __umul24(IDW, rowb);       \
            }
            uint32_t idw_c, idw_n;
            double r_c, r_n;
            COL_CHUNK(0, idw_c, r_c)
            double ba[4][2], bb[4][2];
            col_gather4<FULL, 0>(ba, rs, idw_c, rowb, eo, ok1);
            for (int c0 = 0;; c0 += 16) {
                COL_CHUNK(c0 + 16, idw_n, r_n)
                col_gather4<FULL, 4>(bb, rs, idw_c, rowb, eo, ok1);
                __builtin_amdgcn_sched_barrier(0);
                col_compute4<DR, 0>(A0, A1, ba, r_c, hh, hmask);
                if (c0 + 4 >= nmax) break;
                col_gather4<FULL, 8>(ba, rs, idw_c, rowb, eo, ok1);
                __builtin_amdgcn_sched_barrier(0);
                col_compute4<DR, 4>(A0, A1, bb, r_c, hh, hmask);
                if (c0 + 8 >= nmax) break;
                col_gather4<FULL, 12>(bb, rs, idw_c, rowb, eo, ok1);
                __builtin_amdgcn_sched_barrier(0);
                col_compute4<DR, 8>(A0, A1, ba, r_c, hh, hmask);
                if (c0 + 12 >= nmax) break;
                col_gather4<FULL, 0>(ba, rs, idw_n, rowb, eo, ok1);
                __builtin_amdgcn_sched_barrier(0);
                col_compute4<DR, 12>(A0, A1, bb, r_c, hh, hmask);
                if (c0 + 16 >= nmax) break;
                idw_c = idw_n; r_c = r_n;
            }
#undef COL_CHUNK
        }
#ifdef BDF_K1_STAMPS
        asm volatile("s_nop 0" :: "v"(A0[0]), "v"(A0[32]), "v"(A1[31]));
        st_steps += (unsigned long long)nmax; st_rounds++;
#endif
        CSTAMP(st_acc);
        const unsigned fl = (unsigned)jb.flags;
        if (__builtin_amdgcn_readfirstlane((int)(__ballot((fl & COLF_PAIR) != 0) != 0ull))) {
#ifdef BDF_K1_STAMPS
            st_folds++;
#endif
            col_fold<16>(A0, A1, (fl & COLF_PAIR) ? 1.0 : 0.0);
            if (__builtin_amdgcn_readfirstlane((int)(__ballot((fl & COLF_QUAD) != 0) != 0ull)))
                col_fold<32>(A0, A1, (fl & COLF_QUAD) ? 1.0 : 0.0);
        }
        if (__builtin_amdgcn_readfirstlane((int)(fl & COLF_MULTI))) {
            const int srow = __builtin_amdgcn_readfirstlane(jb.srow);
            double *dst = p.partials + (int64_t)__builtin_amdgcn_readfirstlane(jb.slot) * COL_PSZ + j;
            if (g == 0) {
#pragma unroll
                for (int e = 0; e < COL_NE; e++) __hip_atomic_store(dst + e * 16, col_entry(A0, A1, e), __ATOMIC_RELAXED, __HIP_MEMORY_SCOPE_AGENT);
            }
            const ColSplit sr = p.rows[srow];
            asm volatile("s_waitcnt vmcnt(0)" ::: "memory");
            int old = 0;
            if (lane == 0) old = __hip_atomic_fetch_add(p.arrived + srow, 1, __ATOMIC_RELAXED, __HIP_MEMORY_SCOPE_AGENT);
            old = __builtin_amdgcn_readfirstlane(old);
#ifdef BDF_K1_STAMPS
            st_parts++;
            if (old == sr.n_slots - 1) st_fins++;
#endif
            if (old != sr.n_slots - 1) { CSTAMP(st_mid); continue; }
            __builtin_amdgcn_fence(__ATOMIC_ACQUIRE, "agent");
            asm volatile("s_waitcnt vmcnt(0)" ::: "memory");
            if (lane == 0) p.arrived[srow] = 0;
            const double *src = p.partials + (int64_t)sr.slot_begin * COL_PSZ + j;
            col_slot_load<0, COL_NE, false>(A0, A1, src + (int64_t)(g < sr.n_slots ? g : 0) * COL_PSZ, g < sr.n_slots ? 1.0 : 0.0);
            for (int s0 = 4; s0 < sr.n_slots; s0 += 4) {
                const bool on = s0 + g < sr.n_slots;
                const double *sp = src + (int64_t)(on ? s0 + g : 0) * COL_PSZ;
                const double m = on ? 1.0 : 0.0;
                col_slot_load<0, 14, true>(A0, A1, sp, m);
                asm volatile("" ::: "memory");
                col_slot_load<14, 28, true>(A0, A1, sp, m);
                asm volatile("" ::: "memory");
                col_slot_load<28, COL_NE, true>(A0, A1, sp, m);
                asm volatile("" ::: "memory");
            }
            col_fold<16>(A0, A1, 1.0);
            col_fold<32>(A0, A1, 1.0);
        }
        CSTAMP(st_mid);
        double z0 = 0.0, z1 = 0.0;
        {
            double ze = 0.0, zo = 0.0;
            if (live && 2 * j < D) bdf_normal_pair<ColCoef>(a.seed, a.sweep, BDF_P_ROW, a.entity_tag, (uint64_t)(uint32_t)jb.orig, (uint32_t)j, ze, zo);
            const int base = lane & 48;
            const double ze0 = __shfl(ze, base + (n0 >> 1)), zo0 = __shfl(zo, base + (n0 >> 1));
            const double ze1 = __shfl(ze, base + (n1 >> 1)), zo1 = __shfl(zo, base + (n1 >> 1));
            z0 = (n0 & 1) ? zo0 : ze0;
            z1 = ok1 ? ((n1 & 1) ? zo1 : ze1) : 0.0;
        }
        asm volatile("" : "+v"(z0), "+v"(z1) :: "memory");
        CSTAMP(st_rng);
        {
            double *tl = lds + g * COL_TL;
            const int jl = j & 7;
            if (!hh) {
#pragma unroll
                for (int i = 0; i < 8; i++) tl[jl * 9 + i] = A0[8 + i];
#pragma unroll
                for (int i = 0; i < 8; i++) tl[72 + i * 9 + jl] = A1[24 + i];
            }
            {
                double *w = tl + 144 + (hh ? 72 : 0) + jl * 9;
#pragma unroll
                for (int i = 0; i < 8; i++) w[i] = A1[i];
            }
            wave_sync();
            {
                const double *r2 = tl + (hh ? 72 : 0) + jl * 9;
                const double *r3 = tl + (hh ? 0 : 144) + jl;
                const double *r4 = tl + (hh ? 72 : 216) + jl;
#pragma unroll
                for (int i = 0; i < 8; i++) A1[8 + i] = r2[i];
#pragma unroll
                for (int i = 0; i < 8; i++) if (16 + i < DR) A0[16 + i] = r3[i * 9];
#pragma unroll
                for (int i = 0; i < 8; i++) if (24 + i < DR) A0[24 + i] = r4[i * 9];
            }
            wave_sync();
            if (hh) {
#pragma unroll
                for (int i = 0; i < 8; i++) tl[jl * 9 + i] = A0[i];
#pragma unroll
                for (int i = 0; i < 8; i++) tl[72 + jl * 9 + i] = A1[16 + i];
            }
            wave_sync();
            if (!hh) {
#pragma unroll
                for (int i = 0; i < 8; i++) A0[8 + i] = tl[i * 9 + jl];
#pragma unroll
                for (int i = 0; i < 8; i++) if (24 + i < DR) A1[24 + i] = tl[72 + i * 9 + jl];
            }
            wave_sync();
        }
#ifdef BDF_K1_STAMPS
        asm volatile("s_waitcnt lgkmcnt(0)\n\ts_nop 0" :: "v"(A0[8]), "v"(A0[31]), "v"(A1[8]), "v"(A1[31]));
#endif
        CSTAMP(st_lay);
        const double alpha = term_alpha(T);
        if (!have_prior) {
            int spins = 0;
            while ((int32_t)(__hip_atomic_load(a.ready, __ATOMIC_RELAXED, __HIP_MEMORY_SCOPE_AGENT) - a.ready_want) < 0) {
                __builtin_amdgcn_s_sleep(16);
                if (++spins > (1 << 22)) { if (lane == 0) atomicOr_system(a.flag, 16); break; }
            }
            col_prior_dma(a.prior_c, lds_img, lane);
        }
        {
            const double *pb = a.prior_b + (a.mu_is_matrix && live ? (int64_t)jb.row * D : 0);
            const double b0 = __hip_atomic_load(pb + n0, __ATOMIC_RELAXED, __HIP_MEMORY_SCOPE_AGENT);
            const double b1 = __hip_atomic_load(pb + n1, __ATOMIC_RELAXED, __HIP_MEMORY_SCOPE_AGENT);
            asm volatile("s_waitcnt vmcnt(0)" ::: "memory");
            wave_sync();
            const double *img = lds + 4 * COL_TL;
            col_prior_lds<0, 0, DR>(A0, img, alpha, j);
            col_prior_lds<1, 0, DR>(A1, img, alpha, j);
            A0[32] = fma(alpha, A0[32], b0);
            A1[32] = ok1 ? fma(alpha, A1[32], b1) : 0.0;
            wave_sync();
        }
#ifdef BDF_K1_STAMPS
        asm volatile("s_nop 0" :: "v"(A0[0]), "v"(A0[31]), "v"(A1[0]), "v"(A1[31]));
#endif
        CSTAMP(st_prior);
        double d0 = 1.0, d1 = 1.0;
        fin_factor<DR, 0>(A0, A1, d0, d1, j);
        const bool lead = live && (fl & COLF_LEADER);
        if (lead && (!(d0 > 0.0) || (ok1 && !(d1 > 0.0)))) atomicOr_system(a.flag, 1);
        const double rd0 = fast_rcp(d0), rd1 = fast_rcp(d1);
        double y0 = fma(z0, fast_rsqrt(d0), A0[32] * rd0), y1 = fma(z1, fast_rsqrt(d1), A1[32] * rd1);
        fin_backward<DR - 1>(A0, A1, y0, y1, rd0, rd1, j);
        if (lead) __hip_atomic_store(a.out + ((int64_t)jb.row * D + ec0), y0, __ATOMIC_RELAXED, __HIP_MEMORY_SCOPE_AGENT);
        if (lead && ok1) __hip_atomic_store(a.out + ((int64_t)jb.row * D + ec1), y1, __ATOMIC_RELAXED, __HIP_MEMORY_SCOPE_AGENT);
        CSTAMP(st_fin);
    }
    }
    if (a_in.done) {
        asm volatile("s_waitcnt vmcnt(0)" ::: "memory");
        if (threadIdx.x == 0) __hip_atomic_fetch_add(a_in.done + BDF_DONE_STRIDE * (w & (BDF_DONE_SHARDS - 1)), 1u, __ATOMIC_RELAXED, __HIP_MEMORY_SCOPE_AGENT);
    }
    if (a_in.span && threadIdx.x == 0) atomicMax(a_in.span + 2 * (w & 63) + 1, (unsigned long long)__builtin_amdgcn_s_memrealtime());
#ifdef BDF_K1_STAMPS
    if (threadIdx.x == 0 && a_in.b_dump && w < 65536) {
        unsigned long long *d = (unsigned long long *)a_in.b_dump + (size_t)w * 16;
        d[0] = st_begin; d[8] = st_t; d[6] = st_rounds; d[7] = st_steps;
        d[1] = st_parts; d[2] = st_fins; d[3] = st_folds; d[4] = st_lay;
        d[11] = st_rng; d[12] = st_acc; d[13] = st_mid; d[14] = st_prior; d[15] = st_fin;
        d[9] = __builtin_amdgcn_s_getreg((4 - 1) << 11 | 0 << 6 | 4) | ((unsigned long long)__builtin_amdgcn_s_getreg((32 - 1) << 11 | 0 << 6 | 4));
        d[10] = __builtin_amdgcn_s_getreg((4 - 1) << 11 | 0 << 6 | 20);
    }
#endif
}

#define COL_C_OBS 52.0
#define COL_C_FIN 1460.0
#define COL_C_FOLD 180.0
#define COL_C_PART 700.0

struct Round { ColJob job[4]; double cost; };

ColJob idle_job() { return ColJob{-1, 0, 0, 0, -1, 0, 0}; }

}

int bdf_col_plan_build(bdf_ctx *ctx, const std::vector<bdf_row_ref> &rows, int T, int64_t slots, bdf_col_plan &plan)
{
    std::vector<Round> rounds;
    std::vector<ColSplit> splits;
    struct Unit { int32_t row, orig; int64_t qb; int32_t n; };
    std::vector<Unit> singles, pairs;
    int32_t n_slots_total = 0;
    auto quad_round = [&](const bdf_row_ref &rr, int64_t b0, int64_t b1, int32_t srow, int32_t slot, double fin_share) {
        Round R;
        const int64_t m = b1 - b0;
        int32_t lmax = 0;
        for (int q = 0; q < 4; q++) {
            const int64_t p0 = b0 + m * q / 4, p1 = b0 + m * (q + 1) / 4;
            R.job[q] = ColJob{rr.out, rr.orig, rr.qb + p0, (int32_t)(p1 - p0), srow, slot,
                              (int32_t)(COLF_PAIR | COLF_QUAD | (q == 0 ? COLF_LEADER : 0) | (srow >= 0 ? COLF_MULTI : 0))};
            lmax = std::max(lmax, (int32_t)(p1 - p0));
        }
        constexpr double part_extra = 3000.0;
        R.cost = COL_C_OBS * lmax + 2 * COL_C_FOLD + (srow >= 0 ? COL_C_PART + fin_share + part_extra : COL_C_FIN);
        rounds.push_back(R);
    };
    for (const bdf_row_ref &rr : rows) {
        const int64_t n = rr.cnt;
        if (n <= T) singles.push_back(Unit{rr.out, rr.orig, rr.qb, (int32_t)n});
        else if (n <= 2 * (int64_t)T) pairs.push_back(Unit{rr.out, rr.orig, rr.qb, (int32_t)n});
        else if (n <= 4 * (int64_t)T) quad_round(rr, 0, n, -1, 0, 0.0);
        else {
            const int64_t W = (n + 4 * (int64_t)T - 1) / (4 * (int64_t)T);
            BDF_REQUIRE(W < (1 << 20), BDF_ERR_ARG, "bdf_sample_rows: a row of %lld observations", (long long)n);
            const int32_t srow = (int32_t)splits.size();
            splits.push_back(ColSplit{n_slots_total, (int32_t)W});
            const double share = (COL_C_FIN + 2 * COL_C_FOLD + 60.0 * (double)((W + 3) / 4)) / (double)W;
            for (int64_t q = 0; q < W; q++) quad_round(rr, n * q / W, n * (q + 1) / W, srow, n_slots_total + (int32_t)q, share);
            n_slots_total += (int32_t)W;
        }
    }
    auto by_len = [](const Unit &x, const Unit &y) { return x.n > y.n; };
    std::stable_sort(pairs.begin(), pairs.end(), by_len);
    std::stable_sort(singles.begin(), singles.end(), by_len);
    auto pair_jobs = [](const Unit &u, ColJob *dst) {
        const int32_t h = u.n / 2;
        dst[0] = ColJob{u.row, u.orig, u.qb, h, -1, 0, COLF_PAIR | COLF_LEADER};
        dst[1] = ColJob{u.row, u.orig, u.qb + h, u.n - h, -1, 0, COLF_PAIR};
    };
    size_t si = 0;
    for (size_t pi = 0; pi < pairs.size(); pi += 2) {
        Round R;
        pair_jobs(pairs[pi], R.job);
        int32_t lmax = pairs[pi].n - pairs[pi].n / 2;
        if (pi + 1 < pairs.size()) pair_jobs(pairs[pi + 1], R.job + 2);
        else {
            for (int q = 2; q < 4; q++) {
                if (si < singles.size()) {
                    const Unit &u = singles[si++];
                    R.job[q] = ColJob{u.row, u.orig, u.qb, u.n, -1, 0, COLF_LEADER};
                    lmax = std::max(lmax, u.n);
                } else R.job[q] = idle_job();
            }
        }
        R.cost = COL_C_OBS * lmax + COL_C_FOLD + COL_C_FIN;
        rounds.push_back(R);
    }
    for (; si < singles.size(); si += 4) {
        Round R;
        for (int q = 0; q < 4; q++) {
            if (si + q < singles.size()) {
                const Unit &u = singles[si + q];
                R.job[q] = ColJob{u.row, u.orig, u.qb, u.n, -1, 0, COLF_LEADER};
            } else R.job[q] = idle_job();
        }
        R.cost = COL_C_OBS * singles[si].n + COL_C_FIN;
        rounds.push_back(R);
    }
    plan.n_rounds = (int64_t)rounds.size();
    plan.n_waves = 0;
    plan.n_split_rows = (int32_t)splits.size();
    if (rounds.empty()) return BDF_OK;
    (void)slots;
    const int64_t nw = (int64_t)rounds.size();
    std::vector<int32_t> rank(rounds.size());
    for (size_t i = 0; i < rank.size(); i++) rank[i] = (int32_t)i;
    std::stable_sort(rank.begin(), rank.end(), [&](int32_t x, int32_t y) { return rounds[(size_t)x].cost > rounds[(size_t)y].cost; });
    constexpr int64_t S2 = 896;
    std::vector<int32_t> idx;
    idx.reserve(rounds.size());
    if (nw <= S2) idx = rank;
    else {
        const int64_t two = std::min<int64_t>(nw, 2 * S2);
        const int64_t P = two - S2, A = S2 - P;
        for (int64_t i = 0; i < P; i++) idx.push_back(rank[(size_t)(A + i)]);
        for (int64_t i = 0; i < A; i++) idx.push_back(rank[(size_t)i]);
        for (int64_t i = 0; i < P; i++) idx.push_back(rank[(size_t)(two - 1 - i)]);
        for (int64_t i = two; i < nw; i++) idx.push_back(rank[(size_t)i]);
    }
    std::vector<ColJob> jobs;
    std::vector<int32_t> wave_round;
    jobs.reserve(rounds.size() * 4);
    wave_round.push_back(0);
    for (int32_t i : idx) {
        for (int q = 0; q < 4; q++) jobs.push_back(rounds[(size_t)i].job[q]);
        wave_round.push_back((int32_t)(jobs.size() / 4));
    }
    plan.cost_max = rounds[(size_t)rank.front()].cost;
    plan.cost_min = rounds[(size_t)rank.back()].cost;
    plan.n_waves = (int32_t)nw;
    BDF_HIP(hipMalloc((void **)&plan.jobs_dev, jobs.size() * sizeof(ColJob)));
    BDF_HIP(hipMemcpy(plan.jobs_dev, jobs.data(), jobs.size() * sizeof(ColJob), hipMemcpyHostToDevice));
    BDF_HIP(hipMalloc((void **)&plan.wave_round_dev, wave_round.size() * sizeof(int32_t)));
    BDF_HIP(hipMemcpy(plan.wave_round_dev, wave_round.data(), wave_round.size() * sizeof(int32_t), hipMemcpyHostToDevice));
    BDF_HIP(hipMalloc((void **)&plan.rows_dev, std::max<size_t>(splits.size() * sizeof(ColSplit), 8)));
    if (!splits.empty()) BDF_HIP(hipMemcpy(plan.rows_dev, splits.data(), splits.size() * sizeof(ColSplit), hipMemcpyHostToDevice));
    BDF_HIP(hipMalloc((void **)&plan.partials_dev, std::max<size_t>((size_t)n_slots_total * COL_PSZ * sizeof(double), 8)));
    BDF_HIP(hipMalloc((void **)&plan.arrived_dev, std::max<size_t>(splits.size() * sizeof(int32_t), 8)));
    BDF_HIP(hipMemsetAsync(plan.arrived_dev, 0, std::max<size_t>(splits.size() * sizeof(int32_t), 8), ctx->stream));
    return BDF_OK;
}

void bdf_col_plan_free(bdf_col_plan &plan)
{
    if (plan.jobs_dev) (void)hipFree(plan.jobs_dev);
    if (plan.wave_round_dev) (void)hipFree(plan.wave_round_dev);
    if (plan.rows_dev) (void)hipFree(plan.rows_dev);
    if (plan.partials_dev) (void)hipFree(plan.partials_dev);
    if (plan.arrived_dev) (void)hipFree(plan.arrived_dev);
    plan = bdf_col_plan{};
}

int bdf_col_launch(bdf_ctx *ctx, const SampleArgs &a, const bdf_col_plan &plan, int64_t M_other, hipEvent_t e0, hipEvent_t e1)
{
    if (plan.n_waves <= 0) return BDF_OK;
    ColPlanDev p;
    p.jobs = plan.jobs_dev; p.wave_round = plan.wave_round_dev; p.n_waves = plan.n_waves; p._pad = 0;
    p.rows = plan.rows_dev; p.partials = plan.partials_dev; p.arrived = plan.arrived_dev;
    const int64_t bytes = M_other * (int64_t)a.D * 8;
    BDF_REQUIRE(bytes < ((int64_t)1 << 32), BDF_ERR_ARG, "bdf_sample_rows: the column kernel needs a factor matrix below 4 GiB");
    const uint32_t fb = (uint32_t)bytes;
    const dim3 grid((unsigned)plan.n_waves), block(64);
    const int DR = (a.D + 3) / 4 * 4;
#define COL_LAUNCH(DRV, FULLV) hipExtLaunchKernelGGL((k_rows_col<DRV, FULLV>), grid, block, 0, ctx->stream, e0, e1, 0, a, p, fb)
    if (a.D == 32) COL_LAUNCH(32, true);
    else if (DR <= 20) COL_LAUNCH(20, false);
    else if (DR <= 24) COL_LAUNCH(24, false);
    else if (DR <= 28) COL_LAUNCH(28, false);
    else COL_LAUNCH(32, false);
#undef COL_LAUNCH
    BDF_HIP(hipGetLastError());
    return BDF_OK;
}
```

### bayesiandatafusion.jl_amd/csrc/rows.h

```cpp
#pragma once
#include "bdf_common.h"

#define BDF_K1_CODES 32
struct TermDev {
    const int64_t *rowptr;
    const int32_t *colidx;
    const double *vals;
    const int32_t *perm;
    const double *linear;
    const double *fac[BDF_MAX_MODES - 1];
    int64_t nnz;
    int32_t n_other;
    int32_t lean;
    double alpha, mean;
    const uint32_t *packed;
    const double *table;
    int32_t n_codes, _padc;
    const double *alpha_dev;
    const double *weight;
};

__device__ __forceinline__ double term_alpha(const TermDev &T) { return T.alpha_dev ? *T.alpha_dev : T.alpha; }

struct SampleArgs {
    TermDev t[BDF_MAX_TERMS];
    int32_t n_terms, D;
    const double *mu;
    int32_t mu_is_matrix, _pad;
    const double *Lambda;
    uint32_t sweep, _pad3;
    uint64_t seed;
    uint32_t entity_tag, _pad2;
    double *out;
    const double *prior_b;
    const double *prior_c;
    double *P_dump, *b_dump;
    int *flag;
    const uint32_t *ready;
    uint32_t ready_want, _pad4;
    unsigned long long *span;
    uint32_t *done;
    const double *spike_state;
    const double *u_current;
};

inline int bdf_rows_dp(int D) { return D <= 16 ? 16 : (D <= 32 ? 32 : 64); }

int bdf_launch_sample_rows(bdf_ctx *ctx, const SampleArgs &a, const bdf_rel *const *rels, const int *modes, int shard,
                           int n_shards, bool dump);
bdf_rows_state *bdf_rows_state_create();
void bdf_rows_state_destroy(bdf_ctx *ctx);
void bdf_plans_release(bdf_ctx *ctx, uint64_t rel_serial);
const std::array<int64_t, 7> *bdf_rows_dispatch_counts(const bdf_ctx *ctx, uint32_t entity_tag);

struct RowItem {
    int32_t row;
    int32_t orig;
    int64_t q_begin;
    int32_t count, _pad;
};

int bdf_small_launch(bdf_ctx *ctx, const SampleArgs &a, const RowItem *items, int64_t n_items, hipEvent_t e0, hipEvent_t e1);
int bdf_lr_launch(bdf_ctx *ctx, const SampleArgs &a, int64_t M_other, int64_t n_rows_entity, const RowItem *items, int64_t n_items, int64_t n_padded, int64_t n32_padded,
                  const int32_t *rows_dev, bool transform, hipEvent_t e0, hipEvent_t e1);
int bdf_lr_max_observations();
int bdf_lr32_max_observations();

struct Item {
    int32_t row;
    int32_t term;
    int64_t q_begin;
    int32_t count;
    int32_t slot;
    int32_t srow;
    int32_t orig;
};

struct SplitRow {
    int32_t row;
    int32_t slot_begin, n_slots;
    int32_t _pad;
};

struct PlanDev {
    const Item *direct;   int32_t n_direct;
    const Item *split;    int32_t n_split;
    const SplitRow *rows; int32_t n_split_rows;
    double *partials;
    int32_t *arrived;
    const int32_t *order;
};

int bdf_k1_launch(bdf_ctx *ctx, const SampleArgs &a, const PlanDev &p, bool dump, hipEvent_t e0, hipEvent_t e1);
int bdf_ss_launch(bdf_ctx *ctx, const SampleArgs &a, const PlanDev &p, hipEvent_t e0, hipEvent_t e1);
int bdf_spike_lambda_launch(bdf_ctx *ctx, int D, const double *spike_state, double *Lambda_mu_out);
inline int bdf_prior_image_doubles(int D) { const int DB = bdf_rows_dp(D) / 16; return DB * (DB + 1) / 2 * 4 * 64; }
int bdf_prior_launch(bdf_ctx *ctx, int D, const double *Lambda, const double *mu, int64_t nrows, int mu_is_matrix, double *out_b, double *out_c);

struct ColJob {
    int32_t row;
    int32_t orig;
    int64_t q_begin;
    int32_t count;
    int32_t srow;
    int32_t slot;
    int32_t flags;
};
#define COLF_LEADER 1
#define COLF_PAIR 2
#define COLF_QUAD 4
#define COLF_MULTI 8
struct ColSplit { int32_t slot_begin, n_slots; };
struct ColPlanDev {
    const ColJob *jobs;
    const int32_t *wave_round;
    int32_t n_waves, _pad;
    const ColSplit *rows;
    double *partials;
    int32_t *arrived;
};
struct bdf_row_ref { int32_t out, orig; int64_t qb, cnt; };
struct bdf_col_plan {
    ColJob *jobs_dev = nullptr;
    int32_t *wave_round_dev = nullptr;
    ColSplit *rows_dev = nullptr;
    double *partials_dev = nullptr;
    int32_t *arrived_dev = nullptr;
    int32_t n_waves = 0, n_split_rows = 0;
    int64_t n_rounds = 0;
    double cost_max = 0.0, cost_min = 0.0;
};
int bdf_col_plan_build(bdf_ctx *ctx, const std::vector<bdf_row_ref> &rows, int T, int64_t slots, bdf_col_plan &plan);
void bdf_col_plan_free(bdf_col_plan &plan);
int bdf_col_launch(bdf_ctx *ctx, const SampleArgs &a, const bdf_col_plan &plan, int64_t M_other, hipEvent_t e0, hipEvent_t e1);
```

### bayesiandatafusion.jl_amd/csrc/rows_plan.hip

```cpp
#include "rows.h"
#include "c_layout_chol.h"
#include <cstdlib>
#include <mutex>

namespace {

struct PlanKey {
    uint64_t rel[BDF_MAX_TERMS];
    int mode[BDF_MAX_TERMS];
    int n_terms, DP, T, Tp;
    int shard, n_shards;
    int small;
    int lr;
    int lr32;
    int64_t lr_min, lr_other;
    int col;
    int col_slots;
    bool operator<(const PlanKey &o) const { return memcmp(this, &o, sizeof(PlanKey)) < 0; }
};

struct Plan {
    PlanDev dev{};
    RowItem *small_dev = nullptr;
    int64_t n_small = 0;
    RowItem *lr_dev = nullptr;
    int32_t *lr_rows_dev = nullptr;
    int64_t n_lr = 0, n_lr_padded = 0;
    int64_t n_lr32_padded = 0;
    bdf_col_plan col;
    int64_t rows_lr = 0, rows_small = 0, rows_col = 0, rows_k1 = 0;
};

void plan_free(Plan &p)
{
    for (void *q : {(void *)p.small_dev, (void *)p.lr_dev, (void *)p.lr_rows_dev, (void *)p.dev.direct, (void *)p.dev.split, (void *)p.dev.rows,
                    (void *)p.dev.order, (void *)p.dev.partials, (void *)p.dev.arrived})
        (void)hipFree(q);
    bdf_col_plan_free(p.col);
}

struct LrKey {
    const void *fac, *Lambda, *mu; uint32_t sweep, tag; int D; int64_t M;
    bool operator==(const LrKey &o) const { return fac == o.fac && Lambda == o.Lambda && mu == o.mu && sweep == o.sweep && tag == o.tag && D == o.D && M == o.M; }
};

std::mutex g_plans_mutex;

}

struct bdf_rows_state {
    std::map<PlanKey, Plan> plans;
    std::map<uint32_t, std::array<int64_t, 7>> dispatch;
    LrKey lr_key{nullptr, nullptr, nullptr, 0, 0, 0, 0};
};

namespace {

constexpr int64_t MAX_PIECES = 64;

struct RowRef {
    int32_t out, orig;
    int64_t qb[BDF_MAX_TERMS];
    int64_t cnt[BDF_MAX_TERMS];
};

enum class Route { LowRank, LowRank32, Small, Column, K1Direct, K1Split };

Route classify(const PlanKey &key, const RowRef &rr, bool lr_on, int &n_items)
{
    int nz = 0;
    int64_t n = 0;
    for (int r = 0; r < key.n_terms; r++) { nz += rr.cnt[r] > 0; n += rr.cnt[r]; }
    if (nz <= 1 && key.small > 0 && n <= key.small) return Route::Small;
    if (nz <= 1 && lr_on && n <= key.lr) return Route::LowRank;
    if (nz <= 1 && lr_on && n <= key.lr32) return Route::LowRank32;
    if (key.col > 0) return Route::Column;
    const int T = key.T;
    n_items = 0;
    for (int r = 0; r < key.n_terms; r++) n_items += (int)std::min<int64_t>((rr.cnt[r] + T - 1) / T, MAX_PIECES);
    if (n_items > 1 && key.Tp != T) {
        n_items = 0;
        for (int r = 0; r < key.n_terms; r++) n_items += (int)std::min<int64_t>((rr.cnt[r] + key.Tp - 1) / key.Tp, MAX_PIECES);
    }
    return n_items <= 1 ? Route::K1Direct : Route::K1Split;
}

int build_plan(bdf_ctx *ctx, const PlanKey &key, const std::vector<RowRef> &rows, bool lr_on, Plan &plan)
{
    const int Tp = key.Tp, DB = key.DP / 16;
    const int psz = DB * (DB + 1) / 2 * 4 * 64 + DB * 16;
    std::vector<Item> direct, split;
    std::vector<RowItem> small, lr, lr32;
    std::vector<SplitRow> srows;
    std::vector<bdf_row_ref> crows;
    for (const RowRef &rr : rows) {
        const int32_t row = rr.out;
        int n_items = 0;
        const Route route = classify(key, rr, lr_on, n_items);
        if (route == Route::Column) { crows.push_back(bdf_row_ref{rr.out, rr.orig, rr.qb[0], rr.cnt[0]}); continue; }
        if (route == Route::K1Split) {
            SplitRow sr{row, (int32_t)split.size(), n_items, 0};
            for (int r = 0; r < key.n_terms; r++) {
                const int64_t beg = rr.qb[r], n = rr.cnt[r];
                const int pieces = (int)std::min<int64_t>((n + Tp - 1) / Tp, MAX_PIECES);
                for (int s = 0; s < pieces; s++) {
                    const int64_t b0 = beg + n * s / pieces, b1 = beg + n * (s + 1) / pieces;
                    split.push_back(Item{row, r, b0, (int32_t)(b1 - b0), (int32_t)split.size(), (int32_t)srows.size(), rr.orig});
                }
            }
            srows.push_back(sr);
            continue;
        }
        Item it{row, 0, 0, 0, -1, -1, rr.orig};
        for (int r = 0; r < key.n_terms; r++)
            if (rr.cnt[r] > 0) { it.term = r; it.q_begin = rr.qb[r]; it.count = (int32_t)rr.cnt[r]; }
        if (route == Route::K1Direct) { direct.push_back(it); continue; }
        (route == Route::Small ? small : (route == Route::LowRank ? lr : lr32)).push_back(RowItem{row, rr.orig, it.q_begin, it.count, 0});
    }
    const int64_t total = (int64_t)split.size() + (int64_t)direct.size();
    std::vector<int32_t> order((size_t)total);
    {
        auto gcd = [](int64_t x, int64_t y) { while (y) { int64_t t = x % y; x = y; y = t; } return x; };
        int64_t stride = 1;
        if (total > 2) {
            stride = (int64_t)(0.6180339887 * (double)total) | 1;
            while (gcd(stride, total) != 1) stride += 2;
        }
        for (int64_t i = 0; i < total; i++) order[(size_t)i] = (int32_t)((i * stride) % total);
    }
    int rc;
    if (key.col > 0 && (rc = bdf_col_plan_build(ctx, crows, key.col, key.col_slots, plan.col))) return rc;
    plan.rows_lr = (int64_t)lr.size() + (int64_t)lr32.size(); plan.rows_small = (int64_t)small.size(); plan.rows_col = (int64_t)crows.size();
    plan.rows_k1 = (int64_t)direct.size() + (int64_t)srows.size();
    while (small.size() % 4) small.push_back(RowItem{-1, 0, 0, 0, 0});
    plan.n_small = (int64_t)small.size();
    if (!small.empty() && (rc = bdf_upload(&plan.small_dev, small))) return rc;
// ... 34 lines not shown
{
    const int DP = bdf_rows_dp(a.D);
    memset(&key, 0, sizeof(key));
    for (int r = 0; r < a.n_terms; r++) { key.rel[r] = rels[r]->serial; key.mode[r] = modes[r]; }
    key.n_terms = a.n_terms; key.DP = DP; key.T = ctx->item_size; key.Tp = std::min(ctx->piece_size, ctx->item_size); key.shard = shard; key.n_shards = n_shards;
    if (ctx->item_auto) {
        int64_t nnz_launch = 0;
        for (int r = 0; r < a.n_terms; r++) nnz_launch += rels[r]->idx[modes[r]].own_nnz;
        const int64_t slots = (int64_t)256 * 4 * (DP == 64 ? 2 : (DP == 32 ? BDF_K1_WAVES32C : 8));
        const int64_t t = std::min<int64_t>(2048, (nnz_launch / (slots * 16) + 63) / 64 * 64);
        if (t > key.T) { key.T = (int)t; key.Tp = (int)(t * 2 / 3); }
    }
    if (a.spike_state != nullptr) return;
    const int64_t n_rows_all = rels[0]->sharded ? (int64_t)rels[0]->idx[modes[0]].own_orig.size() : (int64_t)rels[0]->idx[modes[0]].order.size();
    if (DP == 16 && !dump && ctx->small_max > 0 && a.n_terms == 1 && a.t[0].lean == 1 && a.t[0].n_other == 1 && a.t[0].linear == nullptr &&
        a.t[0].weight == nullptr && n_rows_all >= ctx->small_min_rows)
        key.small = std::min(ctx->small_max, ctx->item_size);

    if (DP > 16 && !dump && ctx->lr_max != 0 && a.n_terms == 1 && a.t[0].n_other == 1 && a.t[0].linear == nullptr && a.t[0].weight == nullptr) {
        const int other = 1 - modes[0];
        M_other = rels[0]->nint[other];
        const int lr_want = ctx->lr_max < 0 ? a.D / 2 : ctx->lr_max;
        key.lr = std::min(std::min(lr_want, bdf_lr_max_observations()), ctx->item_size);
        key.lr32 = DP == 64 ? std::min(std::min(lr_want, bdf_lr32_max_observations()), ctx->item_size) : 0;
        key.lr_min = std::max<int64_t>(ctx->lr_min_rows, 1);
        key.lr_other = ctx->lr_min_rows > 0 ? rels[0]->dims[other] : 0;
    }

    static const bool no_col = getenv("BDF_K1_GENERAL_KERNEL") != nullptr;
    if (DP == 32 && a.D > 16 && !dump && ctx->col_piece > 0 && (ctx->col_explicit || ctx->item_auto) && a.n_terms == 1 && a.t[0].n_other == 1 &&
        a.t[0].lean == 1 && a.t[0].linear == nullptr && a.t[0].weight == nullptr && !no_col) {
        key.col = ctx->col_piece;
        if (!ctx->col_explicit) {
            const int64_t nnz_entity = (int64_t)rels[0]->idx[modes[0]].rowptr.back();
            const int64_t t = std::min<int64_t>(2048, (nnz_entity / (2048 * 8) + 63) / 64 * 64);
            if (t > key.col) key.col = (int)t;
        }
        key.col_slots = std::max(1, ctx->n_cus - ctx->reserve_cus) * 4 * 2;
        M_other = rels[0]->nint[1 - modes[0]];
    }
}

bool collect_rows(const PlanKey &key, const bdf_rel *const *rels, const int *modes, std::vector<RowRef> &rows)
{
    if (rels[0]->sharded) {
        const bdf_mode_index &ix0 = rels[0]->idx[modes[0]];
        for (int64_t o = ix0.chunk_begin[(size_t)key.shard]; o < ix0.chunk_begin[(size_t)key.shard + 1]; o++) {
            RowRef rr;
            rr.out = ix0.own_pos[(size_t)o]; rr.orig = ix0.own_orig[(size_t)o];
            for (int r = 0; r < key.n_terms; r++) {
                const bdf_mode_index &ix = rels[r]->idx[modes[r]];
                rr.qb[r] = ix.own_q[(size_t)o]; rr.cnt[r] = ix.own_q[(size_t)o + 1] - ix.own_q[(size_t)o];
            }
            rows.push_back(rr);
        }
    } else {
        const std::vector<int32_t> &order = rels[0]->idx[modes[0]].order;
        for (size_t pos = (size_t)key.shard; pos < order.size(); pos += (size_t)key.n_shards) {
            RowRef rr;
            rr.out = rr.orig = order[pos];
            for (int r = 0; r < key.n_terms; r++) {
                const auto &rp = rels[r]->idx[modes[r]].rowptr;
                rr.qb[r] = rp[(size_t)rr.orig]; rr.cnt[r] = rp[(size_t)rr.orig + 1] - rp[(size_t)rr.orig];
            }
            rows.push_back(rr);
        }
    }
    if (key.lr <= 0) return false;
    const std::vector<int64_t> &rp = rels[0]->idx[modes[0]].rowptr;
    int64_t cnt = 0;
    for (size_t i = 0; i + 1 < rp.size(); i++) cnt += rp[i + 1] - rp[i] <= key.lr;
    return cnt >= key.lr_min && 2 * cnt >= key.lr_other;
}

int launch_lowrank(bdf_ctx *ctx, const SampleArgs &a, const Plan &plan, int64_t M_other, int64_t n_rows_entity, int shard, hipEvent_t e0, hipEvent_t e1)
{
    const LrKey now{a.t[0].fac[0], a.Lambda, a.mu, a.sweep, a.entity_tag, a.D, M_other};
    const bool same = shard > 0 && now == ctx->rows->lr_key;
    int rc = bdf_lr_launch(ctx, a, M_other, n_rows_entity, plan.lr_dev, plan.n_lr, plan.n_lr_padded, plan.n_lr32_padded, plan.lr_rows_dev, !same, e0, e1);
    if (!rc) ctx->rows->lr_key = now;
    return rc;
}

int launch_column(bdf_ctx *ctx, const SampleArgs &a, const Plan &plan, int64_t M_other, bool more, hipEvent_t e0, hipEvent_t e1)
{
    static const bool no_coded = getenv("BDF_K1_NO_CODED") != nullptr;
    SampleArgs ac = a;
    if (no_coded) ac.t[0].packed = nullptr;
    if (more || plan.n_lr > 0 || plan.n_small > 0) ac.done = nullptr;
    if (ac.done) ctx->rows_done_added = plan.col.n_waves;
    return bdf_col_launch(ctx, ac, plan.col, M_other, e0, e1);
}

}

bdf_rows_state *bdf_rows_state_create() { return new bdf_rows_state(); }

void bdf_rows_state_destroy(bdf_ctx *ctx)
{
    if (!ctx->rows) return;
    bdf_plans_release(ctx, 0);
    delete ctx->rows;
    ctx->rows = nullptr;
}

const std::array<int64_t, 7> *bdf_rows_dispatch_counts(const bdf_ctx *ctx, uint32_t entity_tag)
{
    auto it = ctx->rows->dispatch.find(entity_tag);
    return it == ctx->rows->dispatch.end() ? nullptr : &it->second;
}

extern "C" int bdf_rows_unfinished(bdf_ctx *ctx, int64_t *count)
{
    BDF_REQUIRE(ctx && count, BDF_ERR_ARG, "bdf_rows_unfinished: NULL argument");
    BDF_HIP(hipStreamSynchronize(ctx->stream));
    *count = 0;
    std::lock_guard<std::mutex> lock(g_plans_mutex);
    for (auto &kv : ctx->rows->plans) {
        if (kv.second.col.n_split_rows > 0) {
            std::vector<int32_t> hc((size_t)kv.second.col.n_split_rows);
            BDF_HIP(hipMemcpy(hc.data(), kv.second.col.arrived_dev, hc.size() * sizeof(int32_t), hipMemcpyDeviceToHost));
            for (int32_t v : hc) *count += v != 0;
        }
        const int n = kv.second.dev.n_split_rows;
        if (n <= 0) continue;
        std::vector<int32_t> h((size_t)n);
        BDF_HIP(hipMemcpy(h.data(), kv.second.dev.arrived, (size_t)n * sizeof(int32_t), hipMemcpyDeviceToHost));
        for (int32_t v : h) *count += v != 0;
        static const bool dbg = getenv("BDF_DEBUG_UNFINISHED") != nullptr;
        if (dbg)
            for (int i = 0; i < n; i++)
                if (h[(size_t)i] != 0)
                    fprintf(stderr, "[bdf] unfinished: plan DP=%d T=%d Tp=%d shard %d/%d terms %d, split row %d of %d: counter %d (array %p)\n",
                            kv.first.DP, kv.first.T, kv.first.Tp, kv.first.shard, kv.first.n_shards, kv.first.n_terms, i, n, h[(size_t)i],
                            (void *)kv.second.dev.arrived);
    }
    return BDF_OK;
}

void bdf_plans_release(bdf_ctx *ctx, uint64_t rel_serial)
{
    std::lock_guard<std::mutex> lock(g_plans_mutex);
    auto &plans = ctx->rows->plans;
    for (auto kv = plans.begin(); kv != plans.end();) {
        bool hit = rel_serial == 0;
        for (int r = 0; r < kv->first.n_terms; r++) hit = hit || kv->first.rel[r] == rel_serial;
        if (!hit) { ++kv; continue; }
        plan_free(kv->second);
        kv = plans.erase(kv);
    }
}

int bdf_launch_sample_rows(bdf_ctx *ctx, const SampleArgs &a_in, const bdf_rel *const *rels, const int *modes, int shard,
                           int n_shards, bool dump)
{
    SampleArgs a = a_in;
    int rc;
    const bool spike = a.spike_state != nullptr;
    if (spike) {
        const size_t nlm = (size_t)a.D * a.D + a.D, npk = (size_t)a.D + (size_t)bdf_prior_image_doubles(a.D);
        void *pb;
        if ((rc = bdf_scratch(ctx, (nlm + npk) * sizeof(double), &pb))) return rc;
        double *lm = (double *)pb, *pk = lm + nlm;
        if ((rc = bdf_spike_lambda_launch(ctx, a.D, a.spike_state, lm))) return rc;
        if ((rc = bdf_prior_launch(ctx, a.D, lm, lm + (size_t)a.D * a.D, 1, 0, pk, pk + a.D))) return rc;
        a.Lambda = lm; a.mu = lm + (size_t)a.D * a.D; a.mu_is_matrix = 0;
        a.prior_b = pk; a.prior_c = pk + a.D;
    }
    if (a.prior_b == nullptr) {
        const int64_t nr = a.mu_is_matrix ? rels[0]->nint[modes[0]] : 1;
        void *pb;
        if ((rc = bdf_scratch(ctx, ((size_t)nr * a.D + (size_t)bdf_prior_image_doubles(a.D)) * sizeof(double), &pb))) return rc;
        if ((rc = bdf_prior_launch(ctx, a.D, a.Lambda, a.mu, nr, a.mu_is_matrix, (double *)pb, (double *)pb + nr * a.D))) return rc;
        a.prior_b = (const double *)pb;
        a.prior_c = (const double *)pb + nr * a.D;
    }
    PlanKey key;
    int64_t M_other = 0;
    route_key(ctx, a, rels, modes, shard, n_shards, dump, key, M_other);
    const Plan *plan;
    {
        std::lock_guard<std::mutex> lock(g_plans_mutex);
        auto &plans = ctx->rows->plans;
        auto it = plans.find(key);
        if (it == plans.end()) {
            std::vector<RowRef> rows;
            const bool lr_on = collect_rows(key, rels, modes, rows);
            Plan np;
            if ((rc = build_plan(ctx, key, rows, lr_on, np))) return rc;
            it = plans.emplace(key, np).first;
        }
        plan = &it->second;
    }
    const int64_t work[4] = {plan->n_lr, plan->n_small, plan->col.n_waves, (int64_t)plan->dev.n_split + plan->dev.n_direct};
    std::array<int64_t, 7> &rdsp = ctx->rows->dispatch[a.entity_tag];
    if (rdsp[0] != (int64_t)a.sweep + 1) rdsp = {(int64_t)a.sweep + 1, 0, 0, 0, 0, 0, 0};
    rdsp[1] += plan->rows_lr; rdsp[2] += plan->rows_small; rdsp[3] += plan->rows_col; rdsp[4] += plan->rows_k1;
    rdsp[5] += work[3]; rdsp[6] += work[2];
    for (int s = 0; s < 4; s++) {
        if (work[s] <= 0) continue;
        const bool more = std::any_of(work + s + 1, work + 4, [](int64_t w) { return w > 0; });
        const hipEvent_t e0 = dump ? nullptr : ctx->time_start, e1 = (dump || more) ? nullptr : ctx->time_stop;
        if (s == 0) rc = launch_lowrank(ctx, a, *plan, M_other, rels[0]->nint[modes[0]], shard, e0, e1);
        else if (s == 1) rc = bdf_small_launch(ctx, a, plan->small_dev, plan->n_small, e0, e1);
        else if (s == 2) rc = launch_column(ctx, a, *plan, M_other, more, e0, e1);
        else rc = spike ? bdf_ss_launch(ctx, a, plan->dev, e0, e1) : bdf_k1_launch(ctx, a, plan->dev, dump, e0, e1);
        if (rc) return rc;
        if (!dump) { ctx->time_start = nullptr; if (!more) ctx->time_stop = nullptr; }
    }
    return BDF_OK;
}
```

### bayesiandatafusion.jl_amd/engine.py

```python
import ctypes as C
import os
import sys
import weakref

import numpy as np
import torch

from . import _lib
from . import features as feat
from ._lib import ArgumentError, BackgroundTerm, GibbsEntity, Term, check, lib
from .relation_data import background_mean, check_model, noise_kind


def _ptr(t):
    return C.c_void_p(t.data_ptr()) if t is not None else C.c_void_p(0)


def _facs(factors):
    fp = (C.c_void_p * len(factors))(*[f.data_ptr() for f in factors])
    return fp


class Layout:

# ... 28 lines not shown

    def elapsed_us(self):
        us = C.c_double(0.0)
        check(lib().bdf_event_elapsed_us(self.start, self.stop, C.byref(us)))
        return us.value

    def __del__(self):
        try:
            lib().bdf_event_destroy(self.start)
            lib().bdf_event_destroy(self.stop)
        except Exception:
            pass


class Context:

    def __init__(self, device=None, seed=0, stream=None):
        if not torch.cuda.is_available():
            raise _lib.NoGpuError("no GPU visible: bayesiandatafusion.jl_amd has no CPU path (the reference is the CPU path)")
        self.device = torch.device("cuda", torch.cuda.current_device() if device is None else int(device))
        torch.cuda.set_device(self.device)
        self.stream = stream if stream is not None else torch.cuda.current_stream(self.device)
        self.handle = C.c_void_p()
        check(lib().bdf_ctx_create(self.device.index, C.c_void_p(self.stream.cuda_stream), C.c_uint64(int(seed) & (2 ** 64 - 1)),
                                   C.byref(self.handle)))
        self.seed = int(seed)
        self._children = weakref.WeakSet()

    @classmethod
    def wrap(cls, handle, device, seed, owned=False):
        self = cls.__new__(cls)
        self.device = device
        self.handle = C.c_void_p(handle) if not isinstance(handle, C.c_void_p) else handle
        st = C.c_void_p()
        check(lib().bdf_ctx_stream(self.handle, C.byref(st)))
        self.stream = torch.cuda.ExternalStream(st.value or 0, device=device)
        self.seed = int(seed)
        self._children = weakref.WeakSet()
        self._owned = owned
        return self

    @classmethod
    def rows(cls, device, seed, reserve_cus=0):
        if not torch.cuda.is_available():
            raise _lib.NoGpuError("no GPU visible: bayesiandatafusion.jl_amd has no CPU path (the reference is the CPU path)")
        dev = torch.device("cuda", torch.cuda.current_device() if device is None else int(device))
        torch.cuda.set_device(dev)
        h = C.c_void_p()
        check(lib().bdf_ctx_create_rows(dev.index, C.c_uint64(int(seed) & (2 ** 64 - 1)), int(reserve_cus), C.byref(h)))
        return cls.wrap(h, dev, seed, owned=True)

    @classmethod
    def side(cls, main, apart=(), reserved=False):
        h = C.c_void_p()
        arr = (C.c_void_p * max(len(apart), 1))(*[a.handle for a in apart])
        check(lib().bdf_ctx_create_side(main.handle, arr, len(apart), int(reserved), C.byref(h)))
        return cls.wrap(h, main.device, main.seed, owned=True)

    def adopt(self, child):
        self._children.add(child)

    def set_item_size(self, observations):
        check(lib().bdf_ctx_set_item_size(self.handle, int(observations)))

    def rows_unfinished(self):
        n = C.c_int64(0)
        check(lib().bdf_rows_unfinished(self.handle, C.byref(n)))
        return n.value

    def set_small_rows(self, max_observations, min_rows):
        check(lib().bdf_ctx_set_small_rows(self.handle, int(max_observations), int(min_rows)))

    def set_lowrank(self, max_observations=-1, min_rows=8192):
        check(lib().bdf_ctx_set_lowrank(self.handle, int(max_observations), int(min_rows)))

    def set_col_rows(self, max_piece=-1):
        check(lib().bdf_ctx_set_col_rows(self.handle, int(max_piece)))

    def rows_dispatch(self, entity_tag):
        out = (C.c_int64 * 6)()
        if lib().bdf_ctx_rows_dispatch(self.handle, int(entity_tag), out) != 0:
            return None
        return dict(zip(("lowrank", "small", "col", "k1", "k1_items", "col_waves"), (int(x) for x in out)))

    def set_piece_size(self, observations):
        check(lib().bdf_ctx_set_piece_size(self.handle, int(observations)))

    def set_gather(self, mode):
        check(lib().bdf_ctx_set_gather(self.handle, int(mode)))

    def set_sweep(self, i):
        check(lib().bdf_ctx_set_sweep(self.handle, C.c_uint32(int(i))))

    def advance_sweep(self):
        check(lib().bdf_ctx_advance_sweep(self.handle))

    def sync(self):
        check(lib().bdf_ctx_sync(self.handle))
        bits = C.c_uint32(0)
        check(lib().bdf_ctx_warnings(self.handle, C.byref(bits)))
        if bits.value & 64:
            import warnings
            warnings.warn("beta update: a conjugate-gradient column was still above its tolerance after maxiter iterations",
                          RuntimeWarning, stacklevel=2)

    def zeros(self, *shape, dtype=torch.float64):
        with torch.cuda.stream(self.stream):
            return torch.zeros(*shape, dtype=dtype, device=self.device)

    def tensor(self, a, dtype=torch.float64):
        with torch.cuda.stream(self.stream):
            return torch.as_tensor(np.ascontiguousarray(a), dtype=dtype).to(self.device)

    def close(self):
        if self.handle:
            for ch in list(self._children):
                ch.close()
            if getattr(self, "_owned", True):
                lib().bdf_ctx_destroy(self.handle)
            self.handle = C.c_void_p()

    def __del__(self):
        try:
            self.close()
        except Exception:
            pass


class DeviceRelation:

    def __init__(self, ctx, idf, layouts=None, rank=0, values=None):
        self.ctx = ctx
        self.handle = C.c_void_p()
        dims = np.asarray(idf.dims, dtype=np.int64)
        vals = np.ascontiguousarray(idf.values if values is None else values, dtype=np.float64)
        ids = idf.ids
        if layouts is None or all(l.pos is None for l in layouts):
            check(lib().bdf_relation_create(ctx.handle, len(idf.dims), dims.ctypes.data_as(_lib.c_i64p), idf.nnz(),
                                            ids.ctypes.data_as(C.c_void_p), ids.dtype.itemsize, vals.ctypes.data_as(_lib.c_dp),
                                            C.byref(self.handle)))
        else:
            pos = (_lib.c_i32p * len(layouts))(*[l.pos.ctypes.data_as(_lib.c_i32p) for l in layouts])
            cmax = np.asarray([l.cmax for l in layouts], dtype=np.int64)
            check(lib().bdf_relation_create_sharded(ctx.handle, len(idf.dims), dims.ctypes.data_as(_lib.c_i64p), idf.nnz(),
                                                    ids.ctypes.data_as(C.c_void_p), ids.dtype.itemsize, vals.ctypes.data_as(_lib.c_dp),
                                                    pos, cmax.ctypes.data_as(_lib.c_i64p), rank, layouts[0].world,
                                                    layouts[0].chunks, C.byref(self.handle)))
        self.dims = list(idf.dims)
        self.nnz = idf.nnz()
        self.kind, self.alpha_sample, self.alpha_dev = "gauss", False, None
        self.F = self.beta = self.F_test = self.test_baseline = None
        self.train = None
        self.linear = None
        self.censor = self.interval = self.ordinal = self.ord_codes = None
        self.omega = self.wsse = self.omega_sum = None
        self.robust_nu, self.pg_model, self.pg_r = 0.0, 0, 0.0
        self.noise = self.tau = self.tau_sum = None
        self.bg = self.bg_sums = self.bg_weights = None
        ctx.adopt(self)

    @property
    def has_model(self):
        return self.alpha_sample or self.F is not None or self.kind != "gauss" or self.bg is not None

    def index(self, mode0):
        rp, ri = _lib.c_i64p(), _lib.c_i64p()
# ... 815 lines not shown
                g.feat, g.lambda_beta = dr.F.handle, r.model.lambda_beta
                if ri == 0 and dr.F_test is not None:
                    g.feat_test, g.test_baseline = dr.F_test.handle, dr.test_baseline.data_ptr()
        self._gibbs_relations = arr
        check(lib().bdf_gibbs_set_relations(self.gibbs, len(rows), C.cast(arr, C.c_void_p)))

    def begin_scores(self):
        if self.scores is not None:
            self.scores.close()
            self.scores = None
        rec = self.data.relations[0].model.recommend if self.data.relations else None
        if rec is not None:
            r0, rows = self.data.relations[0], rec["rows"]
            self.scores = DeviceScores(self.ctx, int(r0.data.dims[0]) if rows is None else len(rows), int(r0.data.dims[1]), self.D, rec["batch"],
                                       None if rows is None else np.asarray(rows, dtype=np.int64) - 1)

    def robust_accumulate(self, ri=0):
        dr = self.rel[ri]
        with torch.cuda.stream(self.ctx.stream):
            if dr.omega_sum is None:
                dr.omega_sum = torch.zeros_like(dr.omega)
            dr.omega_sum += dr.omega

    def robust_mean(self, ri=0):
        with torch.cuda.stream(self.ctx.stream):
            return self.rel[ri].omega.mean()

    def spike_accumulate(self):
        if self.ctx_h is not self.ctx:
            self.ctx.stream.wait_stream(self.ctx_h.stream)
        for st in self.ent:
            if st.spike is not None:
                st.spike_accumulate()

    def entity_noise_accumulate(self, ri=0):
        dr = self.rel[ri]
        with torch.cuda.stream(self.ctx.stream):
            if dr.tau_sum is None:
                dr.tau_sum = torch.zeros_like(dr.tau)
            dr.tau_sum += dr.tau

    def entity_noise_mean(self, ri=0):
        with torch.cuda.stream(self.ctx.stream):
            return self.rel[ri].tau.mean()

    def ordinal_begin(self, burnin, psamples, ri=0):
        r, dr = self.data.relations[ri], self.rel[ri]
        if dr.ordinal is None:
            return None
        if dr.ordinal.read()["proposals"] != 0:
            raise ArgumentError(f"Relation {r.name} is ordinal: its edges' trace and burn-in cover one run; build a new engine (reset_model = true)")
        dr.ordinal.close()
        dr.ordinal = DeviceOrdinal(self.ctx, r.model.ordinal["K"], r.model.ordinal["step"], int(burnin) + int(psamples))
        dr.ordinal.set_adapt(burnin)
        self._register_relations()
        return dr.ordinal

    def warm_device(self, milliseconds=50.0):
        if self.gibbs and milliseconds > 0:
            check(lib().bdf_gibbs_warm_device(self.gibbs, float(milliseconds)))
            for j, st in enumerate(self.ent):
                cur = C.c_int(0)
                check(lib().bdf_gibbs_current(self.gibbs, j, C.byref(cur)))
                st.cur = cur.value

    def set_alpha(self):
        if self.gibbs:
            raise ArgumentError("change the precision before the engine is built")

    def k1_algorithmic_bytes(self, j):
        en, st, D = self.data.entities[j], self.ent[j], self.D
        b = st.n_real * (8 * D + 8) + 8 * D * D + 8 * D + (st.n_real * 8 * D if st.F is not None else 0)
        for r in en.relations:
            b += r.data.nnz() * ((4 + 8 * D) * (len(r.entities) - 1) + 8)
        return b

    def k1_algorithmic_flops(self, j):
        en, st, D = self.data.entities[j], self.ent[j], self.D
        f = st.n_real * (D ** 3 / 3.0 + 3 * D * D)
        for r in en.relations:
            f += r.data.nnz() * (D * (D + 1) + 2 * D + D * max(len(r.entities) - 2, 0))
        return f

    def rows_dispatch(self, j):
        return self.ctx.rows_dispatch(self.ent[j].tag)

    def lowrank_rows(self, j):
        got = self.rows_dispatch(j)
        if got is not None:
            return got["lowrank"]
        en, st, D = self.data.entities[j], self.ent[j], self.D
        lr = int(os.environ.get("BDF_LOWRANK", "-1"))
        cap = 32 if D > 32 else 16
        lr = min(cap, D // 2) if lr < 0 else min(lr, cap)
        if D <= 16 or lr == 0 or len(en.relations) != 1 or len(en.relations[0].entities) != 2:
            return 0
        r = en.relations[0]
        dr = self.rel[self._relation_index(r)]
        if dr.F is not None or dr.omega is not None:
            return 0
        m = [e is en for e in r.entities].index(True)
        deg = np.bincount(np.asarray(r.data.ids[:, m], dtype=np.int64) - 1, minlength=en.count)
        cnt = int((deg <= lr).sum())
        min_rows = int(os.environ.get("BDF_LOWRANK_MIN_ROWS", "8192"))
        return cnt if (cnt >= max(min_rows, 1) and 2 * cnt >= r.data.dims[1 - m]) else 0

    def _entity_index(self, en):
        return [e is en for e in self.data.entities].index(True)

    def _relation_index(self, r):
        return [x is r for x in self.data.relations].index(True)

    def _terms(self, j):
        en = self.data.entities[j]
        terms = (Term * len(en.relations))()
        n_bg = 0
        for t, r in enumerate(en.relations):
            dr, term = self.rel[self._relation_index(r)], terms[t]
            term.rel, term.mode, term.mean_value = dr.handle, en.modes[t] - 1, r.model.mean_value
            term.alpha = 1.0 if dr.kind == "probit" else r.model.alpha
            term.linear_values = dr.linear.data_ptr() if dr.linear is not None else None
            term.alpha_dev = dr.alpha_dev.data_ptr() if (self.native and r.model.alpha_sample) else None
            term.obs_precision = dr.omega.data_ptr() if dr.omega is not None else None
            if dr.bg is not None:
                if dr.omega is None:
                    term.alpha = r.model.alpha * (1.0 - dr.bg["weight"])
                    if self.native and r.model.alpha_sample:
                        term.alpha_dev = self.ent[j].bg_alpha_rows.data_ptr() + 8 * n_bg
                n_bg += 1
            for k, e2 in enumerate(r.entities):
                term.factors[k] = self.ent[self._entity_index(e2)].sample.data_ptr()
        return terms

    def update_relations(self):
        L, R, D = lib(), self.ctx.handle, self.D
        comm = self.comm.handle if (self.world > 1 and self.comm is not None) else None
        for ri, (r, dr) in enumerate(zip(self.data.relations, self.rel)):
            if not dr.has_model:
                continue
            m, tag, train = r.model, ri + 1, (dr.train.handle if dr.train is not None else None)
            fac = _facs(self.factors_of(r))
            wsse = _ptr(dr.wsse) if (dr.omega is not None and m.alpha_sample) else None
            if dr.robust_nu > 0.0:
                check(L.bdf_robust_draw(R, train, D, fac, m.mean_value, m.alpha, _ptr(dr.alpha_dev), dr.robust_nu, tag, _ptr(dr.omega), wsse))
            if dr.noise is not None:
                check(L.bdf_entity_noise_draw(R, dr.handle, dr.noise["mode"] - 1, train, D, fac, m.mean_value, m.alpha, _ptr(dr.alpha_dev),
                                              dr.noise["shape"], dr.noise["rate"], tag, _ptr(dr.tau), _ptr(dr.omega), wsse))
            if m.alpha_sample:
                sse = wsse if dr.omega is not None else C.c_void_p(dr.train.stats.data_ptr() + 8)
                n = r.data.nnz()
                if dr.bg is not None:
                    sse = _ptr(dr.wsse)
                    for k, f in enumerate(self.factors_of(r)):
                        check(L.bdf_hyper_sums(R, D, f.shape[0], _ptr(f), None, _ptr(dr.bg_sums[k, :D]), _ptr(dr.bg_sums[k, D:])))
                    check(L.bdf_background_sse(R, train, D, fac, m.mean_value, _ptr(dr.bg_weights) if dr.bg_weights is not None else None,
                                               dr.bg["value"], dr.bg["weight"], _ptr(dr.bg_sums[0, :D]), _ptr(dr.bg_sums[0, D:]),
                                               _ptr(dr.bg_sums[1, :D]), _ptr(dr.bg_sums[1, D:]), r.data.dims[0], r.data.dims[1], sse))
                    n = int(r.data.dims[0]) * int(r.data.dims[1])
                elif dr.omega is None:
                    check(L.bdf_predict_sse(R, train, D, fac, m.mean_value, None, _ptr(dr.train.stats)))
                elif dr.robust_nu == 0.0 and dr.noise is None:
                    check(L.bdf_pairs_weighted_sse(R, train, D, fac, m.mean_value, _ptr(dr.omega), wsse))
                if comm is not None:
                    check(L.bdf_sum_ranks(R, comm, sse, 1))
                check(L.bdf_sample_alpha(R, m.alpha_lambda0, m.alpha_nu0, n, sse, tag, _ptr(dr.alpha_dev)))
                self.ctx.sync()
# ... 461 lines not shown
```

### include/bdf.h

```cpp
#ifndef BDF_H
#define BDF_H
#include <stddef.h>
#include <stdint.h>
#ifdef __cplusplus
extern "C" {
#endif

#define BDF_OK           0
#define BDF_ERR_ARG     (-1)
#define BDF_ERR_BOUNDS  (-2)
#define BDF_ERR_HIP     (-3)
#define BDF_ERR_NOTPD   (-4)
#define BDF_ERR_NOGPU   (-5)

#define BDF_MAX_MODES 4
#define BDF_MAX_TERMS 4
#define BDF_MAX_D     64

#define BDF_P_ROW       1
#define BDF_P_BETA_E1   2
#define BDF_P_BETA_E2   3
#define BDF_P_NW_NORMAL 4
#define BDF_P_GAMMA_N   5
#define BDF_P_GAMMA_U   6
#define BDF_P_NW_MEAN   7
#define BDF_P_BETA_REL1 8
#define BDF_P_BETA_REL2 9
#define BDF_P_HMC_MOMENTUM 10
#define BDF_P_HMC_ACCEPT   11
#define BDF_P_PROBIT       12
#define BDF_P_CENSORED     13
#define BDF_P_INTERVAL     14
#define BDF_P_ORDINAL      15
#define BDF_P_ROBUST_N 16
#define BDF_P_ROBUST_U 17
#define BDF_P_PG 18
#define BDF_P_NOISE_N 19
#define BDF_P_NOISE_U 20
#define BDF_P_SPIKE_N 21
#define BDF_P_SPIKE_U 22
#define BDF_P_SPIKE 23

typedef struct bdf_ctx   bdf_ctx;
typedef struct bdf_rel   bdf_rel;
typedef struct bdf_pairs bdf_pairs;
typedef struct bdf_feat  bdf_feat;
typedef struct bdf_comm  bdf_comm;
typedef struct bdf_gibbs bdf_gibbs;
typedef struct bdf_ordinal bdf_ordinal;

const char *bdf_last_error(void);
int bdf_version(void);

int bdf_ctx_create(int device, void *stream, uint64_t seed, bdf_ctx **out);
int bdf_ctx_destroy(bdf_ctx *ctx);
int bdf_ctx_set_sweep(bdf_ctx *ctx, uint32_t sweep);
int bdf_ctx_advance_sweep(bdf_ctx *ctx);
int bdf_ctx_create_side(bdf_ctx *main_ctx, bdf_ctx *const *apart, int n_apart, int reserved, bdf_ctx **out);
int bdf_ctx_create_rows(int device, uint64_t seed, int reserve_cus, bdf_ctx **out);
int bdf_event_create(void **ev);
int bdf_event_destroy(void *ev);
int bdf_event_elapsed_us(void *start, void *stop, double *us);
int bdf_ctx_time_next_rows(bdf_ctx *ctx, void *start, void *stop);
int bdf_ctx_time_next_hyper(bdf_ctx *ctx, void *start, void *stop);
int bdf_ctx_sync(bdf_ctx *ctx);
#define BDF_WARN_CG_MAXITER 64u
int bdf_ctx_warnings(bdf_ctx *ctx, uint32_t *bits_out);
int bdf_ctx_set_item_size(bdf_ctx *ctx, int observations);
int bdf_ctx_set_piece_size(bdf_ctx *ctx, int observations);
int bdf_ctx_set_small_rows(bdf_ctx *ctx, int max_observations, int64_t min_rows);
int bdf_ctx_set_lowrank(bdf_ctx *ctx, int max_observations, int64_t min_rows);
int bdf_ctx_set_col_rows(bdf_ctx *ctx, int max_piece);
int bdf_ctx_rows_dispatch(const bdf_ctx *ctx, uint32_t entity_tag, int64_t out[6]);
int bdf_ctx_span_next_rows(bdf_ctx *ctx, void *slot_dev);
int bdf_ctx_set_gather(bdf_ctx *ctx, int mode);
int bdf_dev_alloc(bdf_ctx *ctx, size_t bytes, void **dptr);
int bdf_dev_free(bdf_ctx *ctx, void *dptr);
int bdf_h2d(bdf_ctx *ctx, void *dst_dev, const void *src_host, size_t bytes);
int bdf_d2h(bdf_ctx *ctx, void *dst_host, const void *src_dev, size_t bytes);

int bdf_index_build(int n_modes, const int64_t *dims, int64_t nnz, const void *ids, int id_bytes,
                    int64_t *const *rowptr, int64_t *const *rowids);
int bdf_relation_create(bdf_ctx *ctx, int n_modes, const int64_t *dims, int64_t nnz,
                        const void *ids, int id_bytes, const double *values, bdf_rel **out);
int bdf_relation_destroy(bdf_rel *rel);
int bdf_relation_index(const bdf_rel *rel, int mode, const int64_t **rowptr, const int64_t **rowids);
int bdf_relation_value_mean(const bdf_rel *rel, double *mean);
int bdf_relation_order(const bdf_rel *rel, int mode, int32_t *order_host);

typedef struct {
    const bdf_rel *rel;
    int32_t mode;
    int32_t _pad;
    double alpha;
    double mean_value;
    const double *linear_values;
    const double *factors[BDF_MAX_MODES];
    const double *alpha_dev;
    const double *obs_precision;
} bdf_term;

int bdf_sample_rows(bdf_ctx *ctx, int D, int64_t N, int n_terms, const bdf_term *terms,
                    const double *mu, int mu_is_matrix, const double *Lambda,
                    uint32_t entity_tag, int shard, int n_shards, double *out, const double *prior_pack);
int bdf_sample_block(bdf_ctx *ctx, int D, int64_t nu, int64_t nv, const int32_t *vx_dev, const double *Yma,
                     const double *factor, double alpha, const double *mu, const double *Lambda, uint32_t entity_tag,
                     double *out);
int bdf_prior_pack_doubles(int D);
int bdf_row_system(bdf_ctx *ctx, int D, int64_t N, int n_terms, const bdf_term *terms,
                   const double *mu, int mu_is_matrix, const double *Lambda,
                   double *P_out, double *b_out);
int bdf_rows_unfinished(bdf_ctx *ctx, int64_t *count);
int bdf_normals(bdf_ctx *ctx, uint32_t purpose, uint32_t entity_tag, int64_t row_begin,
                int64_t n_rows, int n, double *out);
int bdf_philox(bdf_ctx *ctx, uint32_t purpose, uint32_t entity_tag, uint64_t row, uint32_t pair,
               uint32_t out_host[4]);

int bdf_sample_rows_spike(bdf_ctx *ctx, int D, int64_t N, int n_terms, const bdf_term *terms, const double *spike_state,
                          const double *u_current, uint32_t entity_tag, int shard, int n_shards, double *out);
int bdf_spike_hyper(bdf_ctx *ctx, int D, int64_t N, const double *sample, double incl_a, double incl_b, double shape, double rate,
                    uint32_t entity_tag, double *spike_state);
int bdf_spike_accumulate(bdf_ctx *ctx, int D, int64_t N, const double *sample, const double *spike_state, double *row_sum,
                         double *hyper_sum);

int bdf_hyper_sums(bdf_ctx *ctx, int D, int64_t N, const double *sample, const double *uhat,
                   double *sumU, double *UUt);
int bdf_hyper_sums_ranks(bdf_ctx *ctx, bdf_comm *comm, int D, int64_t N, int chunks, const double *sample, const double *uhat,
                         double *sumU, double *UUt);
int bdf_hyper_sample(bdf_ctx *ctx, int D, int64_t N, const double *sumU, const double *UUt,
                     const double *mu0, double b0, const double *Tinv, double nu,
                     uint32_t entity_tag, double *mu_out, double *Lambda_out, double *params_out, double *prior_pack_out,
                     const double *draws);
int bdf_hyper_draws(bdf_ctx *ctx, int D, int64_t N, double nu, uint32_t entity_tag, double *draws_out);

int bdf_pairs_sort(bdf_pairs *pairs, int mode);
int bdf_pairs_order(const bdf_pairs *pairs, int64_t *orig_host);
int bdf_pairs_set_baseline(bdf_pairs *pairs, const double *baseline);
int bdf_pairs_set_link(bdf_pairs *pairs, int link);
int bdf_pairs_set_logistic_link(bdf_pairs *pairs);
int bdf_pairs_set_count_link(bdf_pairs *pairs, double r);
int bdf_feat_linear(bdf_ctx *ctx, const bdf_feat *F, const double *beta, double mean_value, double *out);
int bdf_predict_sse(bdf_ctx *ctx, const bdf_pairs *pairs, int D, const double *const *factors, double mean_value,
                    const double *linear_values, double *stats_out);

int bdf_sample_alpha(bdf_ctx *ctx, double alpha_lambda0, double alpha_nu0, int64_t n, const double *sumsq_err,
                     uint32_t rel_tag, double *alpha_out);
int bdf_sample_beta_rel(bdf_ctx *ctx, const bdf_feat *F, const bdf_pairs *train, int D, const double *const *factors,
                        double mean_value, double alpha, double lambda_beta, uint32_t rel_tag,
                        double *beta_out, double *linear_out, double *rhs_out);
int bdf_sample_beta_rel_ranks(bdf_ctx *ctx, bdf_comm *comm, const bdf_feat *F, const bdf_pairs *train, int64_t first_obs, int D,
                              const double *const *factors, double mean_value, double alpha, double lambda_beta, uint32_t rel_tag,
                              double *beta_out, double *linear_out, double *rhs_out);
int bdf_sum_ranks(bdf_ctx *ctx, bdf_comm *comm, double *x, int64_t n);
int bdf_probit_draw(bdf_ctx *ctx, const bdf_pairs *train, int D, const double *const *factors, double mean_value,
                    uint32_t rel_tag, double *linear_out, double *z_out);
// ... 126 lines not shown
    int64_t N;
    int64_t n_real;
    uint32_t tag;
    int32_t n_terms;
    struct {
        const bdf_rel *rel;
        int32_t mode;
        int32_t entity_of_mode[BDF_MAX_MODES];
        double alpha, mean_value;
    } terms[BDF_MAX_TERMS];
    double *sample[3];
    double *mu, *Lambda, *mu0, *WI, *sumU, *UUt, *params , *prior_pack, *draws;
    double b0, nu0;
    const bdf_feat *feat;
    double *beta;
    double *uhat, *mu_matrix;
    double *Tinv;
    double *lambda_beta;
    int32_t *cg_iters;
    int32_t use_ff;
    int32_t sample_lambda_beta, full_lambda_u;
    int32_t _pad;
    double tol;
    double lb_nu, lb_mu;
    double *bg_Lambda;
    double *bg_mu;
    double *bg_pack;
    double *bg_alpha_rows;
    int32_t spike;
    int32_t _pad_spike;
    double spike_a, spike_b, spike_shape, spike_rate;
    double *spike_state;
} bdf_gibbs_entity;
int bdf_gibbs_create(bdf_ctx *rows_ctx, int D, int n_entities, const bdf_gibbs_entity *entities, bdf_gibbs **out);
int bdf_gibbs_destroy(bdf_gibbs *g);
int bdf_gibbs_contexts(bdf_gibbs *g, bdf_ctx **hyper, bdf_ctx **pred);
int bdf_ctx_stream(const bdf_ctx *ctx, void **stream);
int bdf_gibbs_set_test(bdf_gibbs *g, bdf_pairs *pairs, const int32_t *entity_of_mode, double mean_value, double clamp_lo,
                       double clamp_hi, double class_cut, double *stats_dev);
typedef struct {
    const bdf_rel *rel;
    int32_t entity_of_mode[BDF_MAX_MODES];
    double mean_value;
    double *alpha_dev;
    int32_t alpha_sample;
    uint32_t rel_tag;
    double alpha_lambda0, alpha_nu0;
    int64_t nnz;
    bdf_pairs *train;
    int64_t first_obs, obs_block;
    const bdf_feat *feat;
    double *beta;
    double *linear;
    double lambda_beta;
    const bdf_feat *feat_test;
    double *test_baseline;
    int32_t probit;
    int32_t _pad;
    const int8_t *censor;
    const double *interval;
    bdf_ordinal *ordinal;
    const int8_t *ordinal_codes;
    double robust_nu;
    double *obs_precision;
    int32_t pg_model;
    int32_t _pad_pg;
    double pg_r;
    double bg_weight, bg_value;
    double *bg_sums;
    const double *bg_weights;
    int32_t noise_mode;
    int32_t _pad_noise;
    double noise_shape, noise_rate;
    double *noise_tau;
} bdf_gibbs_relation;
int bdf_gibbs_set_relations(bdf_gibbs *g, int n_relations, const bdf_gibbs_relation *rels);
int bdf_gibbs_set_comm(bdf_gibbs *g, bdf_comm *comm);
int bdf_gibbs_sweep(bdf_gibbs *g, uint32_t sweep, int predict_phase);
int bdf_gibbs_current(const bdf_gibbs *g, int entity, int *buffer);
int bdf_gibbs_rows_only(bdf_gibbs *g, int entity, uint32_t sweep);
int bdf_gibbs_warm_device(bdf_gibbs *g, double milliseconds);
int bdf_gibbs_recorded(const bdf_gibbs *g, int entity, int *hyper, int *beta);
int bdf_gibbs_set_recorded(bdf_gibbs *g, int entity, int hyper, int beta);
int bdf_gibbs_time_rows(bdf_gibbs *g, int entity, void *start, void *stop);
int bdf_gibbs_span_rows(bdf_gibbs *g, int entity, void *slot_dev);
int bdf_gibbs_sync(bdf_gibbs *g);

int bdf_synth_ratings(uint64_t seed, int64_t n_rows, int64_t n_cols, int64_t k_begin, int64_t k_end,
                      double zipf_offset, double test_fraction, int32_t *rows_out, int32_t *cols_out,
                      double *vals_out, uint8_t *held_out);

typedef struct bdf_vb bdf_vb;
int bdf_vb_create(bdf_ctx *ctx, int D, const int64_t *dims, int64_t nnz, const void *ids, int id_bytes, const double *values,
                  double alpha, const double *mu_init_u, const double *mu_init_v, bdf_vb **out);
int bdf_vb_destroy(bdf_vb *vb);
int bdf_vb_set_test(bdf_vb *vb, bdf_pairs *test, double clamp_lo, double clamp_hi);
int bdf_vb_iterate(bdf_vb *vb, int n);
int bdf_vb_stats(bdf_vb *vb, double *out);
int bdf_vb_model(bdf_vb *vb, int entity, double *mu_host, double *Euu_host, double *prior_host);

typedef struct bdf_hmc bdf_hmc;
int bdf_hmc_create(bdf_ctx *ctx, int D, const int64_t *dims, int64_t nnz, const void *ids, int id_bytes, const double *values,
                   double alpha, bdf_hmc **out);
int bdf_hmc_destroy(bdf_hmc *hmc);
int bdf_hmc_set_test(bdf_hmc *hmc, bdf_pairs *test, double clamp_lo, double clamp_hi);
int bdf_hmc_set_params(bdf_hmc *hmc, int L, int L_inner, int prior_freq, double eps, int burnin);
int bdf_hmc_iterate(bdf_hmc *hmc, int n);
int bdf_hmc_stats(bdf_hmc *hmc, double *out, double *log, int log_cap);
int bdf_hmc_model(bdf_hmc *hmc, int entity, double *sample, double *momentum, double *mu, double *Lambda);

#ifdef __cplusplus
}
#endif
#endif
```

Before: 14090 sweeps/s.

## Gather column-kernel factors from a lane-interleaved image written by the previous sweep

Adds a per-sample "gather image" for D=32 that reorders each factor row so every lane of the column row kernel fetches its two (or four) needed elements with one or two 128-bit buffer loads instead of scattered 64-bit loads. The row kernel writes the image of its output alongside the normal sample, so the next entity's sweep can reuse it without a separate pack pass. A validity cache keyed by sample pointer, with invalidation hooks wherever samples are written externally, decides when a repack is needed. The cost is extra device memory, extra stores per solved row, and a risk of stale images if an invalidation path is missed.

```diff
diff --git a/bayesiandatafusion.jl_amd/_lib.py b/bayesiandatafusion.jl_amd/_lib.py
--- a/bayesiandatafusion.jl_amd/_lib.py
+++ b/bayesiandatafusion.jl_amd/_lib.py
@@ -199,6 +199,11 @@
     "bdf_ctx_set_small_rows": (C.c_int, [C.c_void_p, C.c_int, C.c_int64]),
     "bdf_ctx_set_lowrank": (C.c_int, [C.c_void_p, C.c_int, C.c_int64]),
     "bdf_ctx_set_col_rows": (C.c_int, [C.c_void_p, C.c_int]),
+    "bdf_ctx_set_gather_image": (C.c_int, [C.c_void_p, C.c_int]),
+    "bdf_ctx_gather_image_stats": (C.c_int, [C.c_void_p, C.POINTER(C.c_int64)]),
+    "bdf_ctx_gather_image_read": (C.c_int, [C.c_void_p, C.c_void_p, C.c_int64, C.c_void_p]),
+    "bdf_gather_image_pack": (C.c_int, [C.c_void_p, C.c_void_p, C.c_int64, C.c_void_p]),
+    "bdf_gibbs_sample_written": (C.c_int, [C.c_void_p, C.c_int]),
     "bdf_ctx_rows_dispatch": (C.c_int, [C.c_void_p, C.c_uint32, C.POINTER(C.c_int64)]),
     "bdf_pairs_create": (C.c_int, [C.c_void_p, C.c_int, C.c_int64, C.c_void_p, C.c_int, c_dp, C.POINTER(C.c_void_p)]),
     "bdf_pairs_destroy": (C.c_int, [C.c_void_p]),
diff --git a/bayesiandatafusion.jl_amd/csrc/bdf_api.hip b/bayesiandatafusion.jl_amd/csrc/bdf_api.hip
--- a/bayesiandatafusion.jl_amd/csrc/bdf_api.hip
+++ b/bayesiandatafusion.jl_amd/csrc/bdf_api.hip
@@ -85,6 +85,8 @@
     if (c->col_piece == 1) c->col_piece = 128;
     if (c->col_piece != 0) c->col_piece = std::min(4096, std::max(8, c->col_piece));
     c->col_explicit = false;
+    c->gather_image = 1;
+    c->gimg_trust = false;
     c->lr_T = nullptr; c->lr_vt = nullptr; c->lr_vt_bytes = 0; c->lr_mrows = nullptr; c->lr_mrows_bytes = 0;
     {
         const char *force = getenv("BDF_GATHER");
@@ -230,6 +232,15 @@
     }
     ctx->col_piece = max_piece;
     ctx->col_explicit = true;
+    return BDF_OK;
+}
+
+extern "C" int bdf_ctx_set_gather_image(bdf_ctx *ctx, int on)
+{
+    BDF_REQUIRE(ctx && on >= 0 && on <= 2, BDF_ERR_ARG, "bdf_ctx_set_gather_image: 0 (off), 1 (on) or 2 (the full image)");
+    const int tier = on;
+    if (tier != ctx->gather_image) bdf_gather_image_invalidate(ctx, nullptr);
+    ctx->gather_image = tier;
     return BDF_OK;
 }
 
diff --git a/bayesiandatafusion.jl_amd/csrc/bdf_common.h b/bayesiandatafusion.jl_amd/csrc/bdf_common.h
--- a/bayesiandatafusion.jl_amd/csrc/bdf_common.h
+++ b/bayesiandatafusion.jl_amd/csrc/bdf_common.h
@@ -64,6 +64,8 @@
     int64_t lr_min_rows;
     int col_piece;
     bool col_explicit;
+    int gather_image;
+    bool gimg_trust;
     double *lr_T;
     double *lr_mrows;
     size_t lr_mrows_bytes;
diff --git a/bayesiandatafusion.jl_amd/csrc/bdf_gibbs.hip b/bayesiandatafusion.jl_amd/csrc/bdf_gibbs.hip
--- a/bayesiandatafusion.jl_amd/csrc/bdf_gibbs.hip
+++ b/bayesiandatafusion.jl_amd/csrc/bdf_gibbs.hip
@@ -1,4 +1,5 @@
 #include "bdf_common.h"
+#include "rows.h"
 #include <algorithm>
 #include <chrono>
 #include <cmath>
@@ -75,6 +76,11 @@
     }
 }
 
+void sample_written(bdf_gibbs *g, const bdf_gibbs::Ent &E)
+{
+    for (int b = 0; b < 3; b++) bdf_gather_image_invalidate(g->rows, E.d.sample[b]);
+}
+
 int streams_concurrent(hipStream_t a, hipStream_t b, bool *yes)
 {
     uint32_t *d;
@@ -252,6 +258,7 @@
     for (int j = 0; j < n_entities; j++) {
         auto &E = g->ent[(size_t)j];
         E.d = ents[j]; E.cur = 0;
+        sample_written(g, E);
         BDF_HIP(hipEventCreate(&E.ev_rows));
         BDF_HIP(hipEventCreate(&E.ev_hyper));
         if (E.d.feat) BDF_HIP(hipEventCreateWithFlags(&E.ev_beta, hipEventDisableTiming));
@@ -523,6 +530,7 @@
 {
     BDF_REQUIRE(g, BDF_ERR_ARG, "bdf_gibbs_set_comm: NULL argument");
     g->comm = comm;
+    bdf_gather_image_invalidate(g->rows, nullptr);
     return BDF_OK;
 }
 
@@ -549,8 +557,10 @@
     const double *mu, *Lambda, *pack;
     if ((rc = row_prior(g, E, &mu, &Lambda, &pack))) return rc;
     const int nch = e.terms[0].rel->chunks;
-    for (int c = 0; c < nch; c++)
+    for (int c = 0; c < nch; c++) {
+        R->gimg_trust = !g->comm;
         if ((rc = bdf_sample_rows(R, g->D, e.N, e.n_terms, terms, mu, e.feat ? 1 : 0, Lambda, e.tag, c, nch, e.sample[nxt], pack))) return rc;
+    }
     E.cur = nxt;
     return BDF_OK;
 }
@@ -651,6 +661,7 @@
         off += (pc.bytes + 255) & ~(size_t)255;
     }
     for (int j = 0; j < n; j++) {
+        sample_written(g, g->ent[(size_t)j]);
         g->ent[(size_t)j].hyper_recorded = flags[(size_t)2 * j] != 0;
         g->ent[(size_t)j].beta_recorded = flags[(size_t)2 * j + 1] != 0;
     }
@@ -672,6 +683,14 @@
     BDF_REQUIRE(g && entity >= 0 && entity < (int)g->ent.size(), BDF_ERR_ARG, "bdf_gibbs_set_recorded: bad argument");
     g->ent[(size_t)entity].hyper_recorded = hyper != 0;
     g->ent[(size_t)entity].beta_recorded = beta != 0;
+    sample_written(g, g->ent[(size_t)entity]);
+    return BDF_OK;
+}
+
+extern "C" int bdf_gibbs_sample_written(bdf_gibbs *g, int entity)
+{
+    BDF_REQUIRE(g && entity >= 0 && entity < (int)g->ent.size(), BDF_ERR_ARG, "bdf_gibbs_sample_written: bad argument");
+    sample_written(g, g->ent[(size_t)entity]);
     return BDF_OK;
 }
 
@@ -758,6 +777,7 @@
             R->time_stop = (c == nch - 1 && !g->comm && !counter) ? done : nullptr;
             if (poll) { R->rows_ready = g->ready_dev + j; R->rows_ready_want = E.epoch; }
             if (counter) R->rows_done = E.done_dev;
+            R->gimg_trust = !g->comm;
             if ((rc = e.spike ? bdf_sample_rows_spike(R, D, e.N, e.n_terms, terms, e.spike_state, e.sample[E.cur], e.tag, c, nch, e.sample[nxt])
                               : bdf_sample_rows(R, D, e.N, e.n_terms, terms, mu_rows, e.feat ? 1 : 0, Lambda_rows, e.tag, c, nch, e.sample[nxt], pack_rows)))
                 return rc;
diff --git a/bayesiandatafusion.jl_amd/csrc/dpp_rows32.h b/bayesiandatafusion.jl_amd/csrc/dpp_rows32.h
--- a/bayesiandatafusion.jl_amd/csrc/dpp_rows32.h
+++ b/bayesiandatafusion.jl_amd/csrc/dpp_rows32.h
@@ -58,6 +58,15 @@
         col_star<24, 8, DR - 24>(A1, v1, y);
     }
 }
+__device__ __forceinline__ void col_rank1u(double (&A0)[33], double (&A1)[33], double v0, double v1, double x, double y)
+{
+    fm1<0>(A0[0], v0, v0);
+    col_star<1, 1, 7>(A0, v0, v0);
+    col_star<0, 0, 8>(A1, v0, v1);
+    col_star<16, 0, 8>(A1, v1, v1);
+    col_star<8, 8, 8>(A0, v0, x);
+    col_star<24, 8, 8>(A1, v1, y);
+}
 template <int DR, int S, int K, int I, bool FIRST>
 __device__ __forceinline__ void fin_elim(double (&A0)[33], double (&A1)[33], double nm0, double nm1)
 {
diff --git a/bayesiandatafusion.jl_amd/csrc/k_gather_image.hip b/bayesiandatafusion.jl_amd/csrc/k_gather_image.hip
--- /dev/null
+++ b/bayesiandatafusion.jl_amd/csrc/k_gather_image.hip
@@ -0,0 +1,36 @@
+#include "rows.h"
+
+namespace {
+
+__global__ __launch_bounds__(256) void k_gather_image(const double *__restrict__ sample, double *__restrict__ image, int64_t M, int tier)
+{
+    const int64_t t = (int64_t)blockIdx.x * 256 + threadIdx.x;
+    if (t >= M * 16) return;
+    const int64_t i = t >> 4;
+    const int j = (int)(t & 15);
+    const double *r = sample + i * 32;
+    const double v0 = r[31 - j], v1 = r[15 - j];
+    if (tier == 2) {
+        const bool h = j >= 8;
+        double *d = image + i * 64 + j * 4;
+        d[0] = v0; d[1] = v1;
+        d[2] = h ? v0 : v1;
+        d[3] = h ? v1 : r[31 - (j ^ 8)];
+    } else {
+        double *d = image + i * 32 + j * 2;
+        d[0] = v0; d[1] = v1;
+    }
+}
+
+}
+
+int bdf_gather_image_pack_launch(bdf_ctx *ctx, const double *sample, int64_t M, int tier, double *image)
+{
+    BDF_REQUIRE(ctx && sample && image && M >= 0 && (tier == 1 || tier == 2), BDF_ERR_ARG, "bdf_gather_image_pack: bad argument");
+    if (M == 0) return BDF_OK;
+    BDF_REQUIRE(M <= bdf_col_image_max_rows(), BDF_ERR_ARG, "bdf_gather_image_pack: %lld rows (at most %lld)", (long long)M, (long long)bdf_col_image_max_rows());
+    const unsigned blocks = (unsigned)((M * 16 + 255) / 256);
+    hipLaunchKernelGGL(k_gather_image, dim3(blocks), dim3(256), 0, ctx->stream, sample, image, M, tier);
+    BDF_HIP(hipGetLastError());
+    return BDF_OK;
+}
diff --git a/bayesiandatafusion.jl_amd/csrc/k_rows_col.hip b/bayesiandatafusion.jl_amd/csrc/k_rows_col.hip
--- a/bayesiandatafusion.jl_amd/csrc/k_rows_col.hip
+++ b/bayesiandatafusion.jl_amd/csrc/k_rows_col.hip
@@ -30,6 +30,14 @@
     fm1_run<K>(A1[32], r, v1);
 }
 
+template <int K>
+__device__ __forceinline__ void col_obs_img(double (&A0)[33], double (&A1)[33], double v0, double v1, double x, double y, double r)
+{
+    col_rank1u(A0, A1, v0, v1, x, y);
+    fm1_run<K>(A0[32], r, v0);
+    fm1_run<K>(A1[32], r, v1);
+}
+
 __device__ __forceinline__ double col_ld(__amdgpu_buffer_rsrc_t rs, uint32_t off)
 {
     typedef unsigned u2v __attribute__((ext_vector_type(2)));
@@ -37,15 +45,32 @@
     return __hiloint2double((int)x.y, (int)x.x);
 }
 
-template <bool FULL, int K0>
-__device__ __forceinline__ void col_gather4(double (&b)[4][2], __amdgpu_buffer_rsrc_t rs, uint32_t idw, uint32_t rowb, uint32_t eo, bool ok1)
+__device__ __forceinline__ void col_ld2(__amdgpu_buffer_rsrc_t rs, uint32_t off, double &p, double &q)
+{
+    typedef unsigned u4v __attribute__((ext_vector_type(4)));
+    const u4v x = __builtin_amdgcn_raw_buffer_load_b128(rs, (int)off, 0, 0);
+    p = __hiloint2double((int)x.y, (int)x.x);
+    q = __hiloint2double((int)x.w, (int)x.z);
+}
+
+#define COL_IMG_LANE(IMG) ((IMG) == 2 ? 4 : 2)
+#define COL_IMG_PAD_ID 0x7ffff8u
+
+template <int IMG, bool FULL, int K0>
+__device__ __forceinline__ void col_gather4(double (&b)[4][COL_IMG_LANE(IMG)], __amdgpu_buffer_rsrc_t rs, uint32_t idw, uint32_t rowb, uint32_t eo, bool ok1)
 {
 #pragma unroll
     for (int q = 0; q < 4; q++) {
         uint32_t id;
         if (q == 0) id = row_bcast_u32<K0>(idw); else if (q == 1) id = row_bcast_u32<K0 + 1>(idw);
         else if (q == 2) id = row_bcast_u32<K0 + 2>(idw); else id = row_bcast_u32<K0 + 3>(idw);
-        if constexpr (FULL) {
+        if constexpr (IMG == 2) {
+            const uint32_t base = id + eo;
+            col_ld2(rs, base, b[q][0], b[q][1]);
+            col_ld2(rs, base + 16u, b[q][2], b[q][3]);
+        } else if constexpr (IMG == 1) {
+            col_ld2(rs, id + eo, b[q][0], b[q][1]);
+        } else if constexpr (FULL) {
             const uint32_t base = id + eo;
             b[q][1] = col_ld(rs, base);
             b[q][0] = col_ld(rs, base + 128u);
@@ -56,9 +81,16 @@
         }
     }
 }
-template <int DR, int K0>
-__device__ __forceinline__ void col_compute4(double (&A0)[33], double (&A1)[33], const double (&b)[4][2], double r, bool h, uint64_t hmask)
-{
+template <int DR, int IMG, int K0>
+__device__ __forceinline__ void col_compute4(double (&A0)[33], double (&A1)[33], const double (&b)[4][COL_IMG_LANE(IMG)], double r, bool h, uint64_t hmask)
+{
+    if constexpr (IMG == 2) {
+        col_obs_img<K0>(A0, A1, b[0][0], b[0][1], b[0][2], b[0][3], r);
+        col_obs_img<K0 + 1>(A0, A1, b[1][0], b[1][1], b[1][2], b[1][3], r);
+        col_obs_img<K0 + 2>(A0, A1, b[2][0], b[2][1], b[2][2], b[2][3], r);
+        col_obs_img<K0 + 3>(A0, A1, b[3][0], b[3][1], b[3][2], b[3][3], r);
+        return;
+    }
     col_obs<DR, K0>(A0, A1, b[0][0], b[0][1], r, h, hmask);
     col_obs<DR, K0 + 1>(A0, A1, b[1][0], b[1][1], r, h, hmask);
     col_obs<DR, K0 + 2>(A0, A1, b[2][0], b[2][1], r, h, hmask);
@@ -108,9 +140,10 @@
     }
 }
 
-template <int DR, bool FULL>
-__global__ __launch_bounds__(64, BDF_COL_WAVES) __attribute__((amdgpu_num_vgpr(COL_VGPR_HALF))) void k_rows_col(SampleArgs a_in, ColPlanDev p_in, uint32_t fac_bytes)
-{
+template <int DR, bool FULL, int IMG>
+__device__ __forceinline__ void rows_col_body(const SampleArgs &a_in, const ColPlanDev &p_in, uint32_t fac_bytes)
+{
+    static_assert(IMG == 0 || (FULL && DR == 32), "the gather image is D = 32's");
     __shared__ __attribute__((aligned(16))) double lds[4 * COL_TL + 768];
     const int w = blockIdx.x;
     if (w >= p_in.n_waves) return;
@@ -131,9 +164,9 @@
     const int ec0 = D - 1 - j, ec1 = D - 17 - j;
     const int n0 = ec0, n1 = ec1 >= 0 ? ec1 : 0;
     const bool ok1 = ec1 >= 0;
-    const uint32_t rowb = (uint32_t)D * 8u;
-    const uint32_t eo = FULL ? (uint32_t)ec1 * 8u : (uint32_t)ec0 * 8u;
-    const __amdgpu_buffer_rsrc_t rs = __builtin_amdgcn_make_buffer_rsrc((void *)T.fac[0], 0, (int)fac_bytes, 0x00020000);
+    const uint32_t rowb = IMG ? (uint32_t)COL_IMG_LANE(IMG) * 128u : (uint32_t)D * 8u;
+    const uint32_t eo = IMG ? (uint32_t)j * (uint32_t)COL_IMG_LANE(IMG) * 8u : (FULL ? (uint32_t)ec1 * 8u : (uint32_t)ec0 * 8u);
+    const __amdgpu_buffer_rsrc_t rs = __builtin_amdgcn_make_buffer_rsrc((void *)(IMG ? a.img_in : T.fac[0]), 0, (int)fac_bytes, 0x00020000);
     const bool coded = T.packed != nullptr;
     const double mean = T.mean;
     {
@@ -159,7 +192,7 @@
 #define COL_CHUNK(c0, IDW, R)                                                                     \
             {                                                                                     \
                 const int o_ = (c0) + j;                                                          \
-                IDW = 0xffffffu; R = 0.0;                                                         \
+                IDW = IMG ? COL_IMG_PAD_ID : 0xffffffu; R = 0.0;                                                         \
                 if (o_ < n) {                                                                     \
                     if (coded) { const uint32_t pw_ = packed[o_]; IDW = pw_; R = table[pw_ >> 24] - mean; } \
                     else { IDW = (uint32_t)colidx[o_]; R = vals[o_] - mean; }                     \
@@ -169,25 +202,25 @@
             uint32_t idw_c, idw_n;
             double r_c, r_n;
             COL_CHUNK(0, idw_c, r_c)
-            double ba[4][2], bb[4][2];
-            col_gather4<FULL, 0>(ba, rs, idw_c, rowb, eo, ok1);
+            double ba[4][COL_IMG_LANE(IMG)], bb[4][COL_IMG_LANE(IMG)];
+            col_gather4<IMG, FULL, 0>(ba, rs, idw_c, rowb, eo, ok1);
             for (int c0 = 0;; c0 += 16) {
                 COL_CHUNK(c0 + 16, idw_n, r_n)
-                col_gather4<FULL, 4>(bb, rs, idw_c, rowb, eo, ok1);
+                col_gather4<IMG, FULL, 4>(bb, rs, idw_c, rowb, eo, ok1);
                 __builtin_amdgcn_sched_barrier(0);
-                col_compute4<DR, 0>(A0, A1, ba, r_c, hh, hmask);
+                col_compute4<DR, IMG, 0>(A0, A1, ba, r_c, hh, hmask);
                 if (c0 + 4 >= nmax) break;
-                col_gather4<FULL, 8>(ba, rs, idw_c, rowb, eo, ok1);
+                col_gather4<IMG, FULL, 8>(ba, rs, idw_c, rowb, eo, ok1);
                 __builtin_amdgcn_sched_barrier(0);
-                col_compute4<DR, 4>(A0, A1, bb, r_c, hh, hmask);
+                col_compute4<DR, IMG, 4>(A0, A1, bb, r_c, hh, hmask);
                 if (c0 + 8 >= nmax) break;
-                col_gather4<FULL, 12>(bb, rs, idw_c, rowb, eo, ok1);
+                col_gather4<IMG, FULL, 12>(bb, rs, idw_c, rowb, eo, ok1);
                 __builtin_amdgcn_sched_barrier(0);
-                col_compute4<DR, 8>(A0, A1, ba, r_c, hh, hmask);
+                col_compute4<DR, IMG, 8>(A0, A1, ba, r_c, hh, hmask);
                 if (c0 + 12 >= nmax) break;
-                col_gather4<FULL, 0>(ba, rs, idw_n, rowb, eo, ok1);
+                col_gather4<IMG, FULL, 0>(ba, rs, idw_n, rowb, eo, ok1);
                 __builtin_amdgcn_sched_barrier(0);
-                col_compute4<DR, 12>(A0, A1, bb, r_c, hh, hmask);
+                col_compute4<DR, IMG, 12>(A0, A1, bb, r_c, hh, hmask);
                 if (c0 + 16 >= nmax) break;
                 idw_c = idw_n; r_c = r_n;
             }
@@ -337,6 +370,18 @@
         fin_backward<DR - 1>(A0, A1, y0, y1, rd0, rd1, j);
         if (lead) __hip_atomic_store(a.out + ((int64_t)jb.row * D + ec0), y0, __ATOMIC_RELAXED, __HIP_MEMORY_SCOPE_AGENT);
         if (lead && ok1) __hip_atomic_store(a.out + ((int64_t)jb.row * D + ec1), y1, __ATOMIC_RELAXED, __HIP_MEMORY_SCOPE_AGENT);
+        if constexpr (IMG != 0) {
+            const double yo = __shfl_xor(y0, 8);
+            if (lead && a.img_out) {
+                double *ip = a.img_out + ((int64_t)jb.row * 16 + j) * COL_IMG_LANE(IMG);
+                __hip_atomic_store(ip, y0, __ATOMIC_RELAXED, __HIP_MEMORY_SCOPE_AGENT);
+                __hip_atomic_store(ip + 1, y1, __ATOMIC_RELAXED, __HIP_MEMORY_SCOPE_AGENT);
+                if constexpr (IMG == 2) {
+                    __hip_atomic_store(ip + 2, hh ? y0 : y1, __ATOMIC_RELAXED, __HIP_MEMORY_SCOPE_AGENT);
+                    __hip_atomic_store(ip + 3, hh ? y1 : yo, __ATOMIC_RELAXED, __HIP_MEMORY_SCOPE_AGENT);
+                }
+            }
+        }
         CSTAMP(st_fin);
     }
     }
@@ -357,7 +402,18 @@
 #endif
 }
 
-#define COL_C_OBS 52.0
+template <int DR, bool FULL>
+__global__ __launch_bounds__(64, BDF_COL_WAVES) __attribute__((amdgpu_num_vgpr(COL_VGPR_HALF))) void k_rows_col(SampleArgs a_in, ColPlanDev p_in, uint32_t fac_bytes)
+{
+    rows_col_body<DR, FULL, 0>(a_in, p_in, fac_bytes);
+}
+template <int IMG>
+__global__ __launch_bounds__(64, BDF_COL_WAVES) __attribute__((amdgpu_num_vgpr(COL_VGPR_HALF))) void k_rows_col_img(SampleArgs a_in, ColPlanDev p_in, uint32_t fac_bytes)
+{
+    rows_col_body<32, true, IMG>(a_in, p_in, fac_bytes);
+}
+
+#define COL_C_OBS 51.0
 #define COL_C_FIN 1460.0
 #define COL_C_FOLD 180.0
 #define COL_C_PART 700.0
@@ -495,17 +551,27 @@
     plan = bdf_col_plan{};
 }
 
-int bdf_col_launch(bdf_ctx *ctx, const SampleArgs &a, const bdf_col_plan &plan, int64_t M_other, hipEvent_t e0, hipEvent_t e1)
+int64_t bdf_col_image_max_rows() { return (int64_t)COL_IMG_PAD_ID; }
+
+int bdf_col_launch(bdf_ctx *ctx, const SampleArgs &a, const bdf_col_plan &plan, int64_t M_other, int img_tier, hipEvent_t e0, hipEvent_t e1)
 {
     if (plan.n_waves <= 0) return BDF_OK;
     ColPlanDev p;
     p.jobs = plan.jobs_dev; p.wave_round = plan.wave_round_dev; p.n_waves = plan.n_waves; p._pad = 0;
     p.rows = plan.rows_dev; p.partials = plan.partials_dev; p.arrived = plan.arrived_dev;
-    const int64_t bytes = M_other * (int64_t)a.D * 8;
+    BDF_REQUIRE(!a.img_in || ((img_tier == 1 || img_tier == 2) && a.D == 32 && M_other <= bdf_col_image_max_rows()), BDF_ERR_ARG,
+                "bdf_sample_rows: a gather image of %lld rows at D = %d", (long long)M_other, a.D);
+    const int64_t bytes = a.img_in ? M_other * bdf_gather_image_row_doubles(img_tier) * 8 : M_other * (int64_t)a.D * 8;
     BDF_REQUIRE(bytes < ((int64_t)1 << 32), BDF_ERR_ARG, "bdf_sample_rows: the column kernel needs a factor matrix below 4 GiB");
     const uint32_t fb = (uint32_t)bytes;
     const dim3 grid((unsigned)plan.n_waves), block(64);
     const int DR = (a.D + 3) / 4 * 4;
+    if (a.img_in) {
+        if (img_tier == 2) hipExtLaunchKernelGGL((k_rows_col_img<2>), grid, block, 0, ctx->stream, e0, e1, 0, a, p, fb);
+        else hipExtLaunchKernelGGL((k_rows_col_img<1>), grid, block, 0, ctx->stream, e0, e1, 0, a, p, fb);
+        BDF_HIP(hipGetLastError());
+        return BDF_OK;
+    }
 #define COL_LAUNCH(DRV, FULLV) hipExtLaunchKernelGGL((k_rows_col<DRV, FULLV>), grid, block, 0, ctx->stream, e0, e1, 0, a, p, fb)
     if (a.D == 32) COL_LAUNCH(32, true);
     else if (DR <= 20) COL_LAUNCH(20, false);
diff --git a/bayesiandatafusion.jl_amd/csrc/rows.h b/bayesiandatafusion.jl_amd/csrc/rows.h
--- a/bayesiandatafusion.jl_amd/csrc/rows.h
+++ b/bayesiandatafusion.jl_amd/csrc/rows.h
@@ -42,6 +42,8 @@
     uint32_t *done;
     const double *spike_state;
     const double *u_current;
+    const double *img_in;
+    double *img_out;
 };
 
 inline int bdf_rows_dp(int D) { return D <= 16 ? 16 : (D <= 32 ? 32 : 64); }
@@ -132,4 +134,9 @@
 };
 int bdf_col_plan_build(bdf_ctx *ctx, const std::vector<bdf_row_ref> &rows, int T, int64_t slots, bdf_col_plan &plan);
 void bdf_col_plan_free(bdf_col_plan &plan);
-int bdf_col_launch(bdf_ctx *ctx, const SampleArgs &a, const bdf_col_plan &plan, int64_t M_other, hipEvent_t e0, hipEvent_t e1);
+int bdf_col_launch(bdf_ctx *ctx, const SampleArgs &a, const bdf_col_plan &plan, int64_t M_other, int img_tier, hipEvent_t e0, hipEvent_t e1);
+
+inline int64_t bdf_gather_image_row_doubles(int tier) { return tier == 2 ? 64 : 32; }
+int64_t bdf_col_image_max_rows();
+int bdf_gather_image_pack_launch(bdf_ctx *ctx, const double *sample, int64_t M, int tier, double *image);
+void bdf_gather_image_invalidate(bdf_ctx *ctx, const double *sample);
diff --git a/bayesiandatafusion.jl_amd/csrc/rows_plan.hip b/bayesiandatafusion.jl_amd/csrc/rows_plan.hip
--- a/bayesiandatafusion.jl_amd/csrc/rows_plan.hip
+++ b/bayesiandatafusion.jl_amd/csrc/rows_plan.hip
@@ -46,12 +46,16 @@
 
 std::mutex g_plans_mutex;
 
+struct GatherImage { double *dev = nullptr; int64_t rows = 0; int tier = 0; bool valid = false; };
+
 }
 
 struct bdf_rows_state {
     std::map<PlanKey, Plan> plans;
     std::map<uint32_t, std::array<int64_t, 7>> dispatch;
     LrKey lr_key{nullptr, nullptr, nullptr, 0, 0, 0, 0};
+    std::map<const double *, GatherImage> images;
+    int64_t image_stats[3] = {0, 0, 0};
 };
 
 namespace {
@@ -252,14 +256,58 @@
     return rc;
 }
 
-int launch_column(bdf_ctx *ctx, const SampleArgs &a, const Plan &plan, int64_t M_other, bool more, hipEvent_t e0, hipEvent_t e1)
+void images_free(bdf_rows_state *st)
+{
+    for (auto &kv : st->images) (void)hipFree(kv.second.dev);
+    st->images.clear();
+}
+
+int image_of(bdf_ctx *ctx, const double *sample, int64_t rows, int tier, GatherImage **out)
+{
+    auto &m = ctx->rows->images;
+    auto it = m.find(sample);
+    if (it != m.end() && (it->second.rows != rows || it->second.tier != tier)) { (void)hipFree(it->second.dev); m.erase(it); it = m.end(); }
+    if (it == m.end()) {
+        GatherImage g;
+        g.rows = rows; g.tier = tier;
+        BDF_HIP(hipMalloc((void **)&g.dev, (size_t)std::max<int64_t>(rows, 1) * (size_t)bdf_gather_image_row_doubles(tier) * sizeof(double)));
+        it = m.emplace(sample, g).first;
+    }
+    *out = &it->second;
+    return BDF_OK;
+}
+
+int launch_column(bdf_ctx *ctx, const SampleArgs &a, const Plan &plan, int64_t M_other, int64_t n_rows, bool more, bool whole, bool trust,
+                  hipEvent_t e0, hipEvent_t e1)
 {
     static const bool no_coded = getenv("BDF_K1_NO_CODED") != nullptr;
     SampleArgs ac = a;
     if (no_coded) ac.t[0].packed = nullptr;
+    const int tier = ctx->gather_image;
+    if (tier != 0 && a.D == 32 && whole && M_other > 0 && M_other <= bdf_col_image_max_rows()) {
+        int rc;
+        bdf_rows_state *st = ctx->rows;
+        if (st->images.size() >= 48) images_free(st);
+        GatherImage *src;
+        if ((rc = image_of(ctx, a.t[0].fac[0], M_other, tier, &src))) return rc;
+        if (!(trust && src->valid)) {
+            if ((rc = bdf_gather_image_pack_launch(ctx, a.t[0].fac[0], M_other, tier, src->dev))) return rc;
+            src->valid = true;
+            st->image_stats[1]++;
+        }
+        ac.img_in = src->dev;
+        st->image_stats[0]++;
+        if (!more && plan.n_lr == 0 && plan.n_small == 0 && plan.rows_col == n_rows && n_rows <= bdf_col_image_max_rows()) {
+            GatherImage *dst;
+            if ((rc = image_of(ctx, a.out, n_rows, tier, &dst))) return rc;
+            ac.img_out = dst->dev;
+            dst->valid = true;
+            st->image_stats[2]++;
+        }
+    }
     if (more || plan.n_lr > 0 || plan.n_small > 0) ac.done = nullptr;
     if (ac.done) ctx->rows_done_added = plan.col.n_waves;
-    return bdf_col_launch(ctx, ac, plan.col, M_other, e0, e1);
+    return bdf_col_launch(ctx, ac, plan.col, M_other, tier, e0, e1);
 }
 
 }
@@ -270,6 +318,7 @@
 {
     if (!ctx->rows) return;
     bdf_plans_release(ctx, 0);
+    images_free(ctx->rows);
     delete ctx->rows;
     ctx->rows = nullptr;
 }
@@ -278,6 +327,36 @@
 {
     auto it = ctx->rows->dispatch.find(entity_tag);
     return it == ctx->rows->dispatch.end() ? nullptr : &it->second;
+}
+
+void bdf_gather_image_invalidate(bdf_ctx *ctx, const double *sample)
+{
+    for (auto &kv : ctx->rows->images)
+        if (!sample || kv.first == sample) kv.second.valid = false;
+}
+
+extern "C" int bdf_ctx_gather_image_stats(const bdf_ctx *ctx, int64_t out[3])
+{
+    BDF_REQUIRE(ctx && out, BDF_ERR_ARG, "bdf_ctx_gather_image_stats: NULL argument");
+    for (int k = 0; k < 3; k++) out[k] = ctx->rows->image_stats[k];
+    return BDF_OK;
+}
+
+extern "C" int bdf_ctx_gather_image_read(bdf_ctx *ctx, const double *sample, int64_t rows, double *host_out)
+{
+    BDF_REQUIRE(ctx && sample && host_out, BDF_ERR_ARG, "bdf_ctx_gather_image_read: NULL argument");
+    auto it = ctx->rows->images.find(sample);
+    BDF_REQUIRE(it != ctx->rows->images.end() && it->second.valid && it->second.rows == rows, BDF_ERR_ARG,
+                "bdf_ctx_gather_image_read: no current gather image of %lld rows at this address", (long long)rows);
+    BDF_HIP(hipStreamSynchronize(ctx->stream));
+    BDF_HIP(hipMemcpy(host_out, it->second.dev, (size_t)rows * (size_t)bdf_gather_image_row_doubles(it->second.tier) * sizeof(double), hipMemcpyDeviceToHost));
+    return BDF_OK;
+}
+
+extern "C" int bdf_gather_image_pack(bdf_ctx *ctx, const double *sample, int64_t rows, double *image_dev)
+{
+    BDF_REQUIRE(ctx && ctx->gather_image != 0, BDF_ERR_ARG, "bdf_gather_image_pack: the gather image is off on this context");
+    return bdf_gather_image_pack_launch(ctx, sample, rows, ctx->gather_image, image_dev);
 }
 
 extern "C" int bdf_rows_unfinished(bdf_ctx *ctx, int64_t *count)
@@ -326,6 +405,9 @@
 {
     SampleArgs a = a_in;
     int rc;
+    const bool image_trust = ctx->gimg_trust;
+    ctx->gimg_trust = false;
+    bdf_gather_image_invalidate(ctx, a.out);
     const bool spike = a.spike_state != nullptr;
     if (spike) {
         const size_t nlm = (size_t)a.D * a.D + a.D, npk = (size_t)a.D + (size_t)bdf_prior_image_doubles(a.D);
@@ -373,7 +455,7 @@
         const hipEvent_t e0 = dump ? nullptr : ctx->time_start, e1 = (dump || more) ? nullptr : ctx->time_stop;
         if (s == 0) rc = launch_lowrank(ctx, a, *plan, M_other, rels[0]->nint[modes[0]], shard, e0, e1);
         else if (s == 1) rc = bdf_small_launch(ctx, a, plan->small_dev, plan->n_small, e0, e1);
-        else if (s == 2) rc = launch_column(ctx, a, *plan, M_other, more, e0, e1);
+        else if (s == 2) rc = launch_column(ctx, a, *plan, M_other, rels[0]->nint[modes[0]], more, n_shards == 1 && !rels[0]->sharded, image_trust, e0, e1);
         else rc = spike ? bdf_ss_launch(ctx, a, plan->dev, e0, e1) : bdf_k1_launch(ctx, a, plan->dev, dump, e0, e1);
         if (rc) return rc;
         if (!dump) { ctx->time_start = nullptr; if (!more) ctx->time_stop = nullptr; }
diff --git a/bayesiandatafusion.jl_amd/engine.py b/bayesiandatafusion.jl_amd/engine.py
--- a/bayesiandatafusion.jl_amd/engine.py
+++ b/bayesiandatafusion.jl_amd/engine.py
@@ -134,6 +134,24 @@
         if lib().bdf_ctx_rows_dispatch(self.handle, int(entity_tag), out) != 0:
             return None
         return dict(zip(("lowrank", "small", "col", "k1", "k1_items", "col_waves"), (int(x) for x in out)))
+
+    def set_gather_image(self, on=1):
+        check(lib().bdf_ctx_set_gather_image(self.handle, int(on)))
+
+    def gather_image_stats(self):
+        out = (C.c_int64 * 3)()
+        check(lib().bdf_ctx_gather_image_stats(self.handle, out))
+        return dict(zip(("launches", "packs", "left"), (int(x) for x in out)))
+
+    def gather_image_read(self, sample, tier_doubles=32):
+        out = np.empty((sample.shape[0], 16, tier_doubles // 16), dtype=np.float64)
+        check(lib().bdf_ctx_gather_image_read(self.handle, _ptr(sample), int(sample.shape[0]), out.ctypes.data_as(C.c_void_p)))
+        return out
+
+    def gather_image_pack(self, sample, tier_doubles=32):
+        img = self.zeros(sample.shape[0], 16, tier_doubles // 16)
+        check(lib().bdf_gather_image_pack(self.handle, _ptr(sample), int(sample.shape[0]), _ptr(img)))
+        return img
 
     def set_piece_size(self, observations):
         check(lib().bdf_ctx_set_piece_size(self.handle, int(observations)))
@@ -1115,6 +1133,10 @@
             f += r.data.nnz() * (D * (D + 1) + 2 * D + D * max(len(r.entities) - 2, 0))
         return f
 
+    def sample_written(self, j):
+        if self.gibbs:
+            check(lib().bdf_gibbs_sample_written(self.gibbs, int(j)))
+
     def rows_dispatch(self, j):
         return self.ctx.rows_dispatch(self.ent[j].tag)
 
diff --git a/include/bdf.h b/include/bdf.h
--- a/include/bdf.h
+++ b/include/bdf.h
@@ -71,6 +71,10 @@
 int bdf_ctx_set_small_rows(bdf_ctx *ctx, int max_observations, int64_t min_rows);
 int bdf_ctx_set_lowrank(bdf_ctx *ctx, int max_observations, int64_t min_rows);
 int bdf_ctx_set_col_rows(bdf_ctx *ctx, int max_piece);
+int bdf_ctx_set_gather_image(bdf_ctx *ctx, int on);
+int bdf_ctx_gather_image_stats(const bdf_ctx *ctx, int64_t out[3]);
+int bdf_ctx_gather_image_read(bdf_ctx *ctx, const double *sample, int64_t rows, double *host_out);
+int bdf_gather_image_pack(bdf_ctx *ctx, const double *sample, int64_t rows, double *image_dev);
 int bdf_ctx_rows_dispatch(const bdf_ctx *ctx, uint32_t entity_tag, int64_t out[6]);
 int bdf_ctx_span_next_rows(bdf_ctx *ctx, void *slot_dev);
 int bdf_ctx_set_gather(bdf_ctx *ctx, int mode);
@@ -363,6 +367,7 @@
 int bdf_gibbs_warm_device(bdf_gibbs *g, double milliseconds);
 int bdf_gibbs_recorded(const bdf_gibbs *g, int entity, int *hyper, int *beta);
 int bdf_gibbs_set_recorded(bdf_gibbs *g, int entity, int hyper, int beta);
+int bdf_gibbs_sample_written(bdf_gibbs *g, int entity);
 int bdf_gibbs_time_rows(bdf_gibbs *g, int entity, void *start, void *stop);
 int bdf_gibbs_span_rows(bdf_gibbs *g, int entity, void *slot_dev);
 int bdf_gibbs_sync(bdf_gibbs *g);
```

Result: faster. 14320 sweeps/s (median of 6 runs) (+1.6%).
